# azuxmioy/Render-In-Between

Measured on AMD Instinct MI355X. Metric: rendered frames/sec at 512x512 (generator forward + blend, device-resident), higher is better.
Workload: dtype f32

## Files before the change

render-in-between_amd/csrc/igemm.hip.h:

```cpp
#pragma once
#include <hip/hip_runtime.h>
#include <stdint.h>
#include <type_traits>

namespace rib {

typedef float f32x16 __attribute__((ext_vector_type(16)));
typedef float f32x4 __attribute__((ext_vector_type(4)));
typedef __bf16 bf16x8 __attribute__((ext_vector_type(8)));

__device__ __forceinline__ bf16x8 to_bf16x8(const float4 lo, const float4 hi) {
  bf16x8 r;
  r[0] = (__bf16)lo.x; r[1] = (__bf16)lo.y; r[2] = (__bf16)lo.z; r[3] = (__bf16)lo.w;
  r[4] = (__bf16)hi.x; r[5] = (__bf16)hi.y; r[6] = (__bf16)hi.z; r[7] = (__bf16)hi.w;
  return r;
}

enum { ACT_NONE = 0, ACT_LRELU = 1, ACT_TANH = 2, ACT_SIGMOID = 3 };

__device__ __forceinline__ float blend1(float img, float m, float dain) {
  return __fadd_rn(__fmul_rn(img, m), __fmul_rn(dain, __fsub_rn(1.f, m)));
}

enum { ST_F32 = 0, ST_BF16 = 1, ST_F16 = 2 };
// ... 35 lines not shown
__device__ __forceinline__ float4 lrelu4(float4 v) {
  return make_float4(lrelu(v.x), lrelu(v.y), lrelu(v.z), lrelu(v.w));
}
__device__ __forceinline__ float apply_act(float v, int act) {
  if (act == ACT_LRELU) return lrelu(v);
  if (act == ACT_TANH) return tanhf(v);
  if (act == ACT_SIGMOID) return 1.f / (1.f + __expf(-v));
  return v;
}

struct IgemmParams {
  const float* x;
  int Hin, Win, xC;
  int Cin;
  const float* pro_scale;
  const float* pro_shift;
  int pro_ld;
  int pro_lrelu;
  const float* x2; const float* w2;
  int x2C, Cin2;
  const float* w;
  const float* bias;
  int CoutPad;
  int Hout, Wout;
  int tilesX, tilesY;
  int xcd_chunk;
  float* y;
  int yC, yoff, Cout;
  int y_f32;
  int act;
  const float* res;
  int resC, res_ups;
  float* y_nchw;
  double* stat_part;
  int ksplit;
  float* slab;
  const float* xm;
  int xmC, xm_ups;
  const float* m_scale;
  const float* m_shift;
  int m_ld;
  int C;
  int nsets;
  float* ys0; float* ys1;
  int act0, act1;
  const double* m_part; int m_tiles, m_Cs; float m_inv;
  const float* bl_img; const float* bl_dain; float* bl_fuse; int bl_C;
  int w_mod; unsigned w_stride;
  unsigned b_stride; int pair, pair_yoff;
  const float* zeros;
};

enum { STATS_MAX_PARTIALS = 128 };

__device__ __forceinline__ void stats_from_partials(const double* base, int tiles, int Cs, int c, int t0, int tstep,
                                                    double& a1, double& a2) {
  a1 = 0.0; a2 = 0.0;
  int t = t0;
  for (; t + 3 * tstep < tiles; t += 4 * tstep) {
    const double x0 = base[(size_t)t * 2 * Cs + c], y0 = base[(size_t)t * 2 * Cs + Cs + c];
    const double x1 = base[(size_t)(t + tstep) * 2 * Cs + c], y1 = base[(size_t)(t + tstep) * 2 * Cs + Cs + c];
    const double x2 = base[(size_t)(t + 2 * tstep) * 2 * Cs + c], y2 = base[(size_t)(t + 2 * tstep) * 2 * Cs + Cs + c];
    const double x3 = base[(size_t)(t + 3 * tstep) * 2 * Cs + c], y3 = base[(size_t)(t + 3 * tstep) * 2 * Cs + Cs + c];
    a1 += (x0 + x1) + (x2 + x3);
    a2 += (y0 + y1) + (y2 + y3);
  }
  for (; t < tiles; t += tstep) {
    a1 += base[(size_t)t * 2 * Cs + c];
    a2 += base[(size_t)t * 2 * Cs + Cs + c];
  }
}
__device__ __forceinline__ void scale_shift_of(double s1, double s2, float inv_count, float g, float b, float& sc, float& sh) {
  const double mean = s1 * (double)inv_count;
  double var = s2 * (double)inv_count - mean * mean;
  if (var < 0.0) var = 0.0;
  const float rstd = (float)(1.0 / sqrt(var + 1e-5));
  sc = rstd * g;
  sh = b - (float)mean * sc;
}

enum { PREC_F32 = 0, PREC_BF16 = 1, PREC_F16 = 2 };
template <int FRW, int WM, int WN, int MF, int NF, int BK, int STRIDE, int KS, bool UPS, int KW = 1, int TB = 1, int PREC = 0, int DMA = 0>
struct IgemmGeom {
  static constexpr bool BF16 = PREC != PREC_F32;
  static constexpr int NT = 256 * KW;
  static constexpr int FRH = 32 / FRW;
  static constexpr int TH = FRH * MF * WM;
  static constexpr int TW = FRW;
  static constexpr int PH = UPS ? 4 : 1;
  static constexpr int IH = UPS ? (TH + 2) : ((TH - 1) * STRIDE + KS);
  static constexpr int IW = UPS ? (TW + 2) : ((TW - 1) * STRIDE + KS);
  static constexpr int EPS = BF16 ? 8 : 4;
  static constexpr int KF = BK * 4 / EPS;
  static constexpr int GPR = BK / EPS;
  static constexpr int GPRB = KF / 4;
  static constexpr int CK = KF + 4;
  static constexpr int IWH = (IW + 1) / 2;
  static constexpr int IWP = (STRIDE == 2 && FRW == 8) ? ((IW + 3) / 8 * 8 + 4) : IW;
  static constexpr int BN = NF == 0 ? 16 * WN : 32 * NF * WN;
  static constexpr int AP = (DMA & 2) ? KF : CK;
  static constexpr int BP = (DMA & 1) ? KF : CK;
  static constexpr int SLOTS = KF / 4;
  static constexpr int SWZ_SHIFT = SLOTS >= 16 ? 0 : (SLOTS == 8 ? 1 : (SLOTS == 4 ? 2 : 3));
// ... 193 lines not shown
            const uint32_t w[4] = {__float_as_uint(v.x), __float_as_uint(v.y), __float_as_uint(v.z), __float_as_uint(v.w)};
            float e[8];
#pragma unroll
            for (int k = 0; k < 4; ++k) { e[2 * k] = h16_to_f32<ST>((uint16_t)(w[k] & 0xffffu)); e[2 * k + 1] = h16_to_f32<ST>((uint16_t)(w[k] >> 16)); }
            if (aff) {
              const float sc[8] = {psc[0].x, psc[0].y, psc[0].z, psc[0].w, psc[PV - 1].x, psc[PV - 1].y, psc[PV - 1].z, psc[PV - 1].w};
              const float sh[8] = {psh[0].x, psh[0].y, psh[0].z, psh[0].w, psh[PV - 1].x, psh[PV - 1].y, psh[PV - 1].z, psh[PV - 1].w};
#pragma unroll
              for (int k = 0; k < 8; ++k) e[k] = e[k] * sc[k] + sh[k];
            }
            if (lr) {
#pragma unroll
              for (int k = 0; k < 8; ++k) e[k] = lrelu(e[k]);
            }
            uint32_t o[4];
#pragma unroll
            for (int k = 0; k < 4; ++k) o[k] = (uint32_t)f32_to_h16<ST>(e[2 * k]) | ((uint32_t)f32_to_h16<ST>(e[2 * k + 1]) << 16);
            v = make_float4(__uint_as_float(o[0]), __uint_as_float(o[1]), __uint_as_float(o[2]), __uint_as_float(o[3]));
          }
        } else {
          if (aff) v = make_float4(v.x * psc[0].x + psh[0].x, v.y * psc[0].y + psh[0].y, v.z * psc[0].z + psh[0].z, v.w * psc[0].w + psh[0].w);
          if (lr) v = lrelu4(v);
        }
      }
      if (!inb) v = make_float4(0.f, 0.f, 0.f, 0.f);
      int lpix = pix;
      if constexpr (STRIDE == 2) { const int ly = pix / G::IW, lx = pix % G::IW; lpix = ly * G::IWP + (lx & 1) * G::IWH + (lx >> 1); }
      if (tid + i * NT < total4) *reinterpret_cast<float4*>(sA + lpix * G::CK + ac4 * 4) = v;
    }
  };

  auto consumer_stats = [&]() {
    if constexpr (SPADE) {
      if (p.m_part) {
        constexpr int NCH = G::BN / 2, S = NT / NCH;
        const int j = tid % NCH, sl = tid / NCH;
        const int v = n0 / 2 + j;
        const bool vv = v < p.nsets * p.C;
        const int c = vv ? (v >= p.C ? v - p.C : v) : 0;
        double a1, a2;
        stats_from_partials(p.m_part + (size_t)n * p.m_tiles * 2 * p.m_Cs, p.m_tiles, p.m_Cs, c, sl, S, a1, a2);
        double* red = reinterpret_cast<double*>(smem);
        red[(sl * NCH + j) * 2] = a1; red[(sl * NCH + j) * 2 + 1] = a2;
        __syncthreads();
        if (sl == 0) {
          double t1 = 0.0, t2 = 0.0;
#pragma unroll
          for (int k = 0; k < S; ++k) { t1 += red[(k * NCH + j) * 2]; t2 += red[(k * NCH + j) * 2 + 1]; }
          float sc, sh;
          scale_shift_of(t1, t2, p.m_inv, 1.f, 0.f, sc, sh);
          s_stat[j] = sc; s_stat[NCH + j] = sh;
        }
        __syncthreads();
      }
    }
  };

  auto compute_tap = [&](int dy, int dx, int buf, int ph = 0) {
    if constexpr (N16) {
      const int l15 = lane & 15, lq = lane >> 4;
      const float* sBb = sB + buf * G::SB + l15 * G::CK + lq * 4;
#pragma unroll
      for (int kb = 0; kb < BK / 16; ++kb) {
        float4 a[MF][2];
#pragma unroll
        for (int mf = 0; mf < MF; ++mf)
#pragma unroll
          for (int sub = 0; sub < 2; ++sub) {
            const int r = (wm * MF + mf) * 2 + sub + dy, c = l15 + dx;
            a[mf][sub] = *reinterpret_cast<const float4*>(sA + (r * G::IW + c) * G::CK + lq * 4 + kb * 16);
          }
        const float4 b = *reinterpret_cast<const float4*>(sBb + kb * 16);
#pragma unroll
        for (int t = 0; t < 4; ++t)
#pragma unroll
          for (int mf = 0; mf < MF; ++mf)
#pragma unroll
            for (int sub = 0; sub < 2; ++sub) {
              const float av = t == 0 ? a[mf][sub].x : t == 1 ? a[mf][sub].y : t == 2 ? a[mf][sub].z : a[mf][sub].w;
              const float bw = t == 0 ? b.x : t == 1 ? b.y : t == 2 ? b.z : b.w;
              acc16[mf][sub] = __builtin_amdgcn_mfma_f32_16x16x4f32(av, bw, acc16[mf][sub], 0, 0, 0);
            }
      }
      return;
// ... 340 lines not shown
        for (int mf = 0; mf < MF; ++mf)
#pragma unroll
          for (int nf = 0; nf < NFE; ++nf)
#pragma unroll
            for (int r = 0; r < 16; ++r) acc[mf][nf][r] += rb[((mf * NFE + nf) * 16 + r) * 64];
      }
    }
    if (kw != 0) return;
  }

  if constexpr (N16) {
    const int l15 = lane & 15, lq = lane >> 4;
    const int col = n0 + l15;
    const bool cvalid = col < p.Cout;
    const float bv = p.bias[min(col, p.CoutPad - 1)];
    double s1 = 0.0, s2 = 0.0;
#pragma unroll
    for (int mf = 0; mf < MF; ++mf)
#pragma unroll
      for (int sub = 0; sub < 2; ++sub)
#pragma unroll
        for (int r = 0; r < 4; ++r) {
          const int oy = ty0 + (wm * MF + mf) * 2 + sub;
          const int ox = tx0 + lq * 4 + r;
          const float v = apply_act(acc16[mf][sub][r] + bv, p.act);
          if (cvalid && oy < p.Hout && ox < p.Wout) {
            const size_t pix = ((size_t)n * p.Hout + oy) * p.Wout + ox;
            p.y[pix * p.yC + p.yoff + col] = v;
            if (p.y_nchw) p.y_nchw[(((size_t)n * p.Cout + col) * p.Hout + oy) * p.Wout + ox] = v;
            s1 += (double)v;
            s2 += (double)v * (double)v;
          }
        }
    if (p.stat_part) {
      __syncthreads();
      double* red = reinterpret_cast<double*>(smem);
      double a1 = s1 + __shfl_xor(s1, 16); a1 += __shfl_xor(a1, 32);
      double a2 = s2 + __shfl_xor(s2, 16); a2 += __shfl_xor(a2, 32);
      if (lane < 16) { red[(wm * 16 + l15) * 2] = a1; red[(wm * 16 + l15) * 2 + 1] = a2; }
      __syncthreads();
      if (tid < 16) {
        double b1 = 0.0, b2 = 0.0;
#pragma unroll
        for (int m = 0; m < WM; ++m) { b1 += red[(m * 16 + tid) * 2]; b2 += red[(m * 16 + tid) * 2 + 1]; }
        double* dst = p.stat_part + (((size_t)n * (p.tilesX * p.tilesY) + tile) * 2) * p.CoutPad;
        dst[n0 + tid] = b1;
        dst[p.CoutPad + n0 + tid] = b2;
      }
    }
  } else if (!SPADE && p.slab != nullptr) {
    float* slab = p.slab + ((size_t)split * gridDim.z / p.ksplit + n) * p.Hout * p.Wout * p.CoutPad;
#pragma unroll
    for (int nf = 0; nf < NF; ++nf) {
      const int col = n0 + (wn * NF + nf) * 32 + li;
#pragma unroll
      for (int ph = 0; ph < PH; ++ph)
#pragma unroll
      for (int mf = 0; mf < MF; ++mf) {
#pragma unroll
        for (int r = 0; r < 16; ++r) {
          const int row = (r & 3) + 8 * (r >> 2) + 4 * lh;
          int oy = ty0 + (wm * MF + mf) * G::FRH + row / FRW;
          int ox = tx0 + row % FRW;
          if (UPS) { oy = 2 * oy + (ph >> 1); ox = 2 * ox + (ph & 1); }
          if (col < p.CoutPad && oy < p.Hout && ox < p.Wout)
            slab[((size_t)oy * p.Wout + ox) * p.CoutPad + col] = acc[ph * MF + mf][nf][r];
        }
      }
    }
  } else if (!SPADE) {
    double* red = reinterpret_cast<double*>(smem);
    if (p.stat_part) __syncthreads();
    const float* pbias = p.bias + (p.w_mod ? (size_t)(n % p.w_mod) * p.b_stride : 0);
    const int ny = p.pair ? (n >> 1) : n;
    const int yoff = p.pair ? p.yoff + (n & 1) * p.pair_yoff : p.yoff;
#pragma unroll
    for (int nf = 0; nf < NF; ++nf) {
      float pv = 0.f, d1 = 0.f, d2 = 0.f;
      const int col = n0 + (wn * NF + nf) * 32 + li;
      const bool cvalid = col < p.Cout;
      const float bv = (col < p.CoutPad) ? pbias[col] : 0.f;
#pragma unroll
      for (int ph = 0; ph < PH; ++ph)
#pragma unroll
      for (int mf = 0; mf < MF; ++mf) {
        const int oy0 = ty0 + (__builtin_amdgcn_readfirstlane(wm) * MF + mf) * G::FRH, ox0 = tx0 + 4 * lh;
        const bool full = !UPS && oy0 + G::FRH <= p.Hout && tx0 + FRW <= p.Wout;
        float rv[16];
        if (p.res && full) {
          const int sh = p.res_ups ? 1 : 0;
          const size_t rrow = (size_t)(p.Wout >> sh) * p.resC;
          const size_t rbase = (((size_t)n * (p.Hout >> sh) + (oy0 >> sh)) * (p.Wout >> sh) + (ox0 >> sh)) * p.resC + min(col, p.resC - 1);
#pragma unroll
          for (int r = 0; r < 16; ++r) {
            const int RY = (8 * (r >> 2)) / FRW, RX = (8 * (r >> 2)) % FRW + (r & 3);
            rv[r] = ld_act<ST>(p.res, rbase + (size_t)(RY >> sh) * rrow + (size_t)(RX >> sh) * p.resC);
          }
        } else if (p.res) {
#pragma unroll
          for (int r = 0; r < 16; ++r) {
            const int row = (r & 3) + 8 * (r >> 2) + 4 * lh;
            int oy = ty0 + (wm * MF + mf) * G::FRH + row / FRW;
            int ox = tx0 + row % FRW;
            if (UPS) { oy = 2 * oy + (ph >> 1); ox = 2 * ox + (ph & 1); }
            oy = min(oy, p.Hout - 1); ox = min(ox, p.Wout - 1);
// ... 64 lines not shown
              const size_t nbase = (((size_t)n * p.Cout + col) * p.Hout + oy0) * p.Wout + ox0;
#pragma unroll
              for (int r = 0; r < 16; ++r) {
                const int RY = (8 * (r >> 2)) / FRW, RX = (8 * (r >> 2)) % FRW + (r & 3);
                p.y_nchw[nbase + (size_t)RY * p.Wout + RX] = BF16 ? vf[r] : vv[r];
              }
            }
          }
        } else {
#pragma unroll
        for (int r = 0; r < 16; ++r) {
          const int row = (r & 3) + 8 * (r >> 2) + 4 * lh;
          int oy = ty0 + (wm * MF + mf) * G::FRH + row / FRW;
          int ox = tx0 + row % FRW;
          if (UPS) { oy = 2 * oy + (ph >> 1); ox = 2 * ox + (ph & 1); }
          if (okm & (1u << r)) {
            const size_t yi = (((size_t)ny * p.Hout + oy) * p.Wout + ox) * p.yC + yoff + col;
            if constexpr (BF16) { if (p.y_f32) p.y[yi] = vv[r]; else st_act<ST>(p.y, yi, vv[r]); }
            else p.y[yi] = vv[r];
          }
        }
        if (p.y_nchw) {
#pragma unroll
          for (int r = 0; r < 16; ++r) {
            const int row = (r & 3) + 8 * (r >> 2) + 4 * lh;
            int oy = ty0 + (wm * MF + mf) * G::FRH + row / FRW;
            int ox = tx0 + row % FRW;
            if (UPS) { oy = 2 * oy + (ph >> 1); ox = 2 * ox + (ph & 1); }
            if (okm & (1u << r)) p.y_nchw[(((size_t)n * p.Cout + col) * p.Hout + oy) * p.Wout + ox] = BF16 ? vf[r] : vv[r];
          }
        }
        }
      }
      if (p.stat_part) {
        int cnt = 0;
#pragma unroll
        for (int ph = 0; ph < PH; ++ph)
#pragma unroll
          for (int mf = 0; mf < MF; ++mf) {
            const int oy0 = ty0 + (__builtin_amdgcn_readfirstlane(wm) * MF + mf) * G::FRH;
            if (!UPS && oy0 + G::FRH <= p.Hout && tx0 + FRW <= p.Wout) { cnt += cvalid ? 16 : 0; continue; }
#pragma unroll
            for (int r = 0; r < 16; ++r) {
              const int row = (r & 3) + 8 * (r >> 2) + 4 * lh;
              int oy = ty0 + (wm * MF + mf) * G::FRH + row / FRW;
              int ox = tx0 + row % FRW;
              if (UPS) { oy = 2 * oy + (ph >> 1); ox = 2 * ox + (ph & 1); }
              cnt += (cvalid && oy < p.Hout && ox < p.Wout) ? 1 : 0;
            }
          }
        const double k = (double)cnt, pd = (double)pv;
        const double s1 = k * pd + (double)d1;
        const double s2 = (k * pd + 2.0 * (double)d1) * pd + (double)d2;
        const double a1 = s1 + __shfl_xor(s1, 32);
        const double a2 = s2 + __shfl_xor(s2, 32);
        if (lh == 0) {
          const int c = (wn * NF + nf) * 32 + li;
          red[(wm * G::BN + c) * 2 + 0] = a1;
          red[(wm * G::BN + c) * 2 + 1] = a2;
        }
      }
    }
    if (p.stat_part) {
      __syncthreads();
      for (int c = tid; c < G::BN; c += 256) {
        double a1 = 0.0, a2 = 0.0;
#pragma unroll
        for (int m = 0; m < WM; ++m) { a1 += red[(m * G::BN + c) * 2]; a2 += red[(m * G::BN + c) * 2 + 1]; }
        const int col = n0 + c;
        if (col < p.CoutPad) {
          double* dst = p.stat_part + (((size_t)n * (p.tilesX * p.tilesY) + tile) * 2) * p.CoutPad;
          dst[col] = a1;
          dst[p.CoutPad + col] = a2;
        }
      }
    }
  } else if constexpr (NF == 1) {
    const int hb = li >> 4, c16 = li & 15;
    const int colg = n0 + wn * 32 + c16;
    const int v = (n0 / 2) + wn * 16 + c16;
    const bool vvalid = v < p.nsets * p.C;
    const int set = (vvalid && v >= p.C) ? 1 : 0;
    const int c = v - set * p.C;
    float bg = 0.f, bb = 0.f, sc = 0.f, sh = 0.f;
    if (vvalid) {
      bg = p.bias[colg]; bb = p.bias[colg + 16];
      if (p.m_part) { sc = s_stat[v - n0 / 2]; sh = s_stat[G::BN / 2 + v - n0 / 2]; }
      else { sc = p.m_scale[(size_t)n * p.m_ld + c]; sh = p.m_shift[(size_t)n * p.m_ld + c]; }
    }
    float* yout = set ? p.ys1 : p.ys0;
    const int act = set ? p.act1 : p.act0;
    const int Hm = p.xm_ups ? p.Hout / 2 : p.Hout, Wm = p.xm_ups ? p.Wout / 2 : p.Wout;
#pragma unroll
    for (int mf = 0; mf < MF; ++mf) {
      const int oy0 = ty0 + (__builtin_amdgcn_readfirstlane(wm) * MF + mf) * G::FRH;
      const bool full = oy0 + G::FRH <= p.Hout && tx0 + FRW <= p.Wout;
      const int oyl = oy0 + (16 * hb) / FRW, oxl = tx0 + 4 * lh;
      const int s = p.xm_ups ? 1 : 0;
      const size_t xrow = (size_t)Wm * p.xmC, yrow = (size_t)p.Wout * p.C;
      const size_t xbase = (((size_t)n * Hm + (oyl >> s)) * Wm + (oxl >> s)) * p.xmC + (vvalid ? c : 0);
      const size_t ybase = (((size_t)n * p.Hout + oyl) * p.Wout + oxl) * p.C + c;
      float xr[8];
#pragma unroll
      for (int k = 0; k < 8; ++k) {
        if (full) {
          const int RY = (8 * (k >> 2)) / FRW, RX = (8 * (k >> 2)) % FRW + (k & 3);
          xr[k] = ld_act<ST>(p.xm, xbase + (size_t)(RY >> s) * xrow + (size_t)(RX >> s) * p.xmC);
        } else {
          const int r = hb * 8 + k;
          const int row = (r & 3) + 8 * (r >> 2) + 4 * lh;
          const int oy = min(ty0 + (wm * MF + mf) * G::FRH + row / FRW, p.Hout - 1);
          const int ox = min(tx0 + row % FRW, p.Wout - 1);
          const int sy = p.xm_ups ? (oy >> 1) : oy, sx = p.xm_ups ? (ox >> 1) : ox;
          xr[k] = ld_act<ST>(p.xm, (((size_t)n * Hm + sy) * Wm + sx) * p.xmC + (vvalid ? c : 0));
        }
      }
#pragma unroll
      for (int k = 0; k < 8; ++k) {
        const float lo = acc[mf][0][k], hi = acc[mf][0][8 + k];
        const float olo = __shfl_xor(lo, 16), ohi = __shfl_xor(hi, 16);
        const float gamma = (hb ? ohi : lo) + bg;
        const float beta = (hb ? hi : olo) + bb;
        float o = (xr[k] * sc + sh) * (1.f + gamma) + beta;
        o = apply_act(o, act);
        if (full) {
          const int RY = (8 * (k >> 2)) / FRW, RX = (8 * (k >> 2)) % FRW + (k & 3);
          if (vvalid) st_act<ST>(yout, ybase + (size_t)RY * yrow + (size_t)RX * p.C, o);
        } else {
          const int r = hb * 8 + k;
          const int row = (r & 3) + 8 * (r >> 2) + 4 * lh;
          const int oy = ty0 + (wm * MF + mf) * G::FRH + row / FRW;
          const int ox = tx0 + row % FRW;
          if (vvalid && oy < p.Hout && ox < p.Wout) st_act<ST>(yout, (((size_t)n * p.Hout + oy) * p.Wout + ox) * p.C + c, o);
        }
      }
    }
  } else {
#pragma unroll
    for (int q = 0; q < NF / 2; ++q) {
      const int colg = n0 + (wn * NF + 2 * q) * 32 + li;
      const int v = (n0 / 2) + (wn * NF / 2 + q) * 32 + li;
      const bool vvalid = v < p.nsets * p.C;
      const int set = (vvalid && v >= p.C) ? 1 : 0;
      const int c = v - set * p.C;
      float bg = 0.f, bb = 0.f, sc = 0.f, sh = 0.f;
      if (vvalid) {
        bg = p.bias[colg]; bb = p.bias[colg + 32];
        if (p.m_part) { sc = s_stat[v - n0 / 2]; sh = s_stat[G::BN / 2 + v - n0 / 2]; }
        else { sc = p.m_scale[(size_t)n * p.m_ld + c]; sh = p.m_shift[(size_t)n * p.m_ld + c]; }
      }
      float* yout = set ? p.ys1 : p.ys0;
      const int act = set ? p.act1 : p.act0;
      const int Hm = p.xm_ups ? p.Hout / 2 : p.Hout, Wm = p.xm_ups ? p.Wout / 2 : p.Wout;
#pragma unroll
      for (int mf = 0; mf < MF; ++mf) {
        const int oy0 = ty0 + (__builtin_amdgcn_readfirstlane(wm) * MF + mf) * G::FRH, ox0 = tx0 + 4 * lh;
        const bool full = oy0 + G::FRH <= p.Hout && tx0 + FRW <= p.Wout;
        float xr[16];
        if (full) {
          const int s = p.xm_ups ? 1 : 0;
          const size_t xrow = (size_t)Wm * p.xmC;
          const size_t xbase = (((size_t)n * Hm + (oy0 >> s)) * Wm + (ox0 >> s)) * p.xmC + (vvalid ? c : 0);
#pragma unroll
          for (int r = 0; r < 16; ++r) {
            const int RY = (8 * (r >> 2)) / FRW, RX = (8 * (r >> 2)) % FRW + (r & 3);
            xr[r] = ld_act<ST>(p.xm, xbase + (size_t)(RY >> s) * xrow + (size_t)(RX >> s) * p.xmC);
          }
          if (vvalid) {
            const size_t yrow = (size_t)p.Wout * p.C;
            const size_t ybase = (((size_t)n * p.Hout + oy0) * p.Wout + ox0) * p.C + c;
#pragma unroll
            for (int r = 0; r < 16; ++r) {
              const int RY = (8 * (r >> 2)) / FRW, RX = (8 * (r >> 2)) % FRW + (r & 3);
              const float gamma = acc[mf][2 * q][r] + bg;
              const float beta = acc[mf][2 * q + 1][r] + bb;
              float o = (xr[r] * sc + sh) * (1.f + gamma) + beta;
              o = apply_act(o, act);
              st_act<ST>(yout, ybase + (size_t)RY * yrow + (size_t)RX * p.C, o);
            }
          }
        } else {
// ... 30 lines not shown
```

render-in-between_amd/csrc/kernels.hip.h:

```cpp
#pragma once
#include "igemm.hip.h"

namespace rib {

struct GemmDmaParams {
  const float* A; const float* B; float* C;
  int M, N, K, lda, ldc;
  size_t sA, sB, sC;
  int modB;
};

typedef uint32_t u32x4 __attribute__((ext_vector_type(4)));
__device__ __forceinline__ void split3_bf16(const float4 p, const float4 q, bf16x8& hi, bf16x8& mid, bf16x8& lo) {
  const float x[8] = {p.x, p.y, p.z, p.w, q.x, q.y, q.z, q.w};
  u32x4 h, m, l;
#pragma unroll
  for (int i = 0; i < 4; ++i) {
    const uint32_t u0 = __float_as_uint(x[2 * i]), u1 = __float_as_uint(x[2 * i + 1]);
    h[i] = __builtin_amdgcn_perm(u1, u0, 0x07060302u);
    const float r0 = x[2 * i] - __uint_as_float(u0 & 0xffff0000u), r1 = x[2 * i + 1] - __uint_as_float(u1 & 0xffff0000u);
    const uint32_t v0 = __float_as_uint(r0), v1 = __float_as_uint(r1);
    m[i] = __builtin_amdgcn_perm(v1, v0, 0x07060302u);
    const float s0 = r0 - __uint_as_float(v0 & 0xffff0000u), s1 = r1 - __uint_as_float(v1 & 0xffff0000u);
    l[i] = __builtin_amdgcn_perm(__float_as_uint(s1), __float_as_uint(s0), 0x07060302u);
// ... 85 lines not shown
        const int rb = (wn * NF + nf) * 32 + li;
        b[nf] = *reinterpret_cast<const float4*>(sB + rb * BK + (slot ^ ((rb >> 1) & 7)) * 4);
      }
#pragma unroll
      for (int nf = 0; nf < NF; ++nf) {
        if constexpr (ST == ST_F32) {
          acc[nf] = __builtin_amdgcn_mfma_f32_32x32x2f32(a.x, b[nf].x, acc[nf], 0, 0, 0);
          acc[nf] = __builtin_amdgcn_mfma_f32_32x32x2f32(a.y, b[nf].y, acc[nf], 0, 0, 0);
          acc[nf] = __builtin_amdgcn_mfma_f32_32x32x2f32(a.z, b[nf].z, acc[nf], 0, 0, 0);
          acc[nf] = __builtin_amdgcn_mfma_f32_32x32x2f32(a.w, b[nf].w, acc[nf], 0, 0, 0);
        } else if constexpr (ST == ST_F16) {
          acc[nf] = __builtin_amdgcn_mfma_f32_32x32x16_f16(*reinterpret_cast<const f16x8*>(&a), *reinterpret_cast<const f16x8*>(&b[nf]), acc[nf], 0, 0, 0);
        } else {
          acc[nf] = __builtin_amdgcn_mfma_f32_32x32x16_bf16(*reinterpret_cast<const bf16x8*>(&a), *reinterpret_cast<const bf16x8*>(&b[nf]), acc[nf], 0, 0, 0);
        }
      }
    }
  }
  float* C = p.C + (size_t)z * p.sC;
#pragma unroll
  for (int nf = 0; nf < NF; ++nf) {
    const int col = n0 + (wn * NF + nf) * 32 + li;
#pragma unroll
    for (int r = 0; r < 16; ++r) {
      const int row = m0 + wm * 32 + (r & 3) + 8 * (r >> 2) + 4 * lh;
      float v = acc[nf][r];
      if constexpr (X3 == 2) v += acc_s[nf][r];
      if (row < p.M && col < p.N) C[(size_t)row * p.ldc + col] = v;
    }
  }
}

struct FinalizeParams {
  const double* part;
  int tiles, Cs, C;
  const float* gamma;
  const float* beta;
  float* scale;
  float* shift;
  int ld, off;
  float inv_count;
  float eps;
  int g_stride, pair_merge, pair_off;
};

template <int CH>
__global__ __launch_bounds__(1024) void k_stats_finalize(const FinalizeParams p) {
  static_assert(CH == 16 || CH == 4, "16 channels x 64 slices or 4 channels x 256 slices");
  constexpr int SL = 1024 / CH;
  __shared__ double red[2][16][CH];
  const int cl = threadIdx.x % CH, sl = threadIdx.x / CH;
  const int c = blockIdx.x * CH + cl;
  const int n = blockIdx.y;
  double a1 = 0.0, a2 = 0.0;
  if (c < p.Cs) stats_from_partials(p.part + (size_t)n * p.tiles * 2 * p.Cs, p.tiles, p.Cs, c, sl, SL, a1, a2);
#pragma unroll
  for (int off = CH; off < 64; off <<= 1) { a1 += __shfl_xor(a1, off); a2 += __shfl_xor(a2, off); }
  if ((threadIdx.x & 63) < CH) { red[0][threadIdx.x >> 6][cl] = a1; red[1][threadIdx.x >> 6][cl] = a2; }
  __syncthreads();
  if (sl == 0) {
    double t1 = 0.0, t2 = 0.0;
#pragma unroll
    for (int w = 0; w < 16; ++w) { t1 += red[0][w][cl]; t2 += red[1][w][cl]; }
    red[0][0][cl] = t1; red[1][0][cl] = t2;
  }
  if (sl == 0 && c < p.C) {
    const double s1 = red[0][0][cl], s2 = red[1][0][cl];
    const double mean = s1 * (double)p.inv_count;
    double var = s2 * (double)p.inv_count - mean * mean;
    if (var < 0.0) var = 0.0;
    const float rstd = (float)(1.0 / sqrt(var + (double)p.eps));
    const int gs = (n & 1) * p.g_stride;
    const float g = p.gamma ? p.gamma[gs + c] : 1.f;
    const float b = p.beta ? p.beta[gs + c] : 0.f;
    const float sc = rstd * g;
    const size_t at = p.pair_merge ? (size_t)(n >> 1) * p.ld + p.off + (n & 1) * p.pair_off + c : (size_t)n * p.ld + p.off + c;
    p.scale[at] = sc;
    p.shift[at] = b - (float)mean * sc;
  }
}

struct SplitEpiParams {
  const float* slab; int ksplit; int B;
  const float* bias; int CoutPad;
  float* y; int yC, yoff, Cout;
  int act;
  const float* res; int resC, res_ups;
  double* stat_part; int blocks;
  int Hout, Wout;
};

template <int ST>
__global__ __launch_bounds__(256) void k_splitk_epilogue(const SplitEpiParams p) {
  __shared__ __attribute__((aligned(16))) double red[2][256][4];
  const int c4n = p.CoutPad / 4;
  const int slots = 256 / c4n;
  const int c4 = threadIdx.x % c4n, slot = threadIdx.x / c4n;
  const int n = blockIdx.y;
  const int npix = p.Hout * p.Wout;
  const int ppb = slots * 4;
  const size_t sstride = (size_t)p.B * npix * p.CoutPad;
  const float4 bv = *reinterpret_cast<const float4*>(p.bias + c4 * 4);
  double s1[4] = {0.0, 0.0, 0.0, 0.0}, s2[4] = {0.0, 0.0, 0.0, 0.0};
  float4 acc4[4];
  {
    float4 v[4][4];
#pragma unroll
    for (int k = 0; k < 4; ++k) {
      const int pix = blockIdx.x * ppb + k * slots + slot;
      const float* src = p.slab + ((size_t)n * npix + (pix < npix ? pix : 0)) * p.CoutPad + c4 * 4;
#pragma unroll
      for (int s = 0; s < 4; ++s) v[k][s] = s < p.ksplit ? *reinterpret_cast<const float4*>(src + s * sstride) : make_float4(0.f, 0.f, 0.f, 0.f);
    }
#pragma unroll
    for (int k = 0; k < 4; ++k) {
      float4 a = v[k][0];
#pragma unroll
      for (int s = 1; s < 4; ++s)
        if (s < p.ksplit) { a.x += v[k][s].x; a.y += v[k][s].y; a.z += v[k][s].z; a.w += v[k][s].w; }
      acc4[k] = a;
    }
// ... 20 lines not shown
      const int oy = pix / p.Wout, ox = pix % p.Wout;
      const size_t rpix = p.res_ups ? ((size_t)n * (p.Hout >> 1) + (oy >> 1)) * (p.Wout >> 1) + (ox >> 1) : (size_t)n * npix + pix;
#pragma unroll
      for (int e = 0; e < 4; ++e) rres[k][e] = ld_act<ST>(p.res, rpix * p.resC + min(c4 * 4 + e, p.resC - 1));
    }
  }
  float vals[4][4];
#pragma unroll
  for (int k = 0; k < 4; ++k) {
    const int pix = blockIdx.x * ppb + k * slots + slot;
    const float4 a = acc4[k];
    const float v[4] = {a.x + bv.x, a.y + bv.y, a.z + bv.z, a.w + bv.w};
#pragma unroll
    for (int e = 0; e < 4; ++e) {
      float t = v[e];
      if (p.res) t += rres[k][e];
      t = apply_act(t, p.act);
      if constexpr (ST != ST_F32) t = round16<ST>(t);
      vals[k][e] = (pix < npix && c4 * 4 + e < p.Cout) ? t : 0.f;
    }
#pragma unroll
    for (int e = 0; e < 4; ++e) { s1[e] += (double)vals[k][e]; s2[e] += (double)vals[k][e] * (double)vals[k][e]; }
  }
#pragma unroll
  for (int k = 0; k < 4; ++k) {
    const int pix = blockIdx.x * ppb + k * slots + slot;
    if (pix < npix) {
      const size_t opix = (size_t)n * npix + pix;
#pragma unroll
      for (int e = 0; e < 4; ++e)
        if (c4 * 4 + e < p.Cout) st_act<ST>(p.y, opix * p.yC + p.yoff + c4 * 4 + e, vals[k][e]);
    }
  }
  if (p.stat_part) {
#pragma unroll
    for (int e = 0; e < 4; ++e) { red[0][threadIdx.x][e] = s1[e]; red[1][threadIdx.x][e] = s2[e]; }
    __syncthreads();
    for (int c = threadIdx.x; c < p.CoutPad; c += 256) {
      const int g = c / 4, e = c % 4;
      double a1 = 0.0, a2 = 0.0;
      for (int s = 0; s < slots; ++s) { a1 += red[0][s * c4n + g][e]; a2 += red[1][s * c4n + g][e]; }
      double* dst = p.stat_part + (((size_t)n * p.blocks + blockIdx.x) * 2) * p.CoutPad;
      dst[c] = a1;
      dst[p.CoutPad + c] = a2;
    }
  }
}

struct StatSrc {
  const double* part;
  int tiles, Cs;
  float inv_count;
  const float* gamma;
  const float* beta;
};

__device__ __forceinline__ void block_stats_64(const StatSrc& s, int n, int c0, int nch, double* red ,
                                               float* s_sc, float* s_sh) {
  const int j = threadIdx.x & 63, q = threadIdx.x >> 6;
  double a1 = 0.0, a2 = 0.0;
  if (j < nch) stats_from_partials(s.part + (size_t)n * s.tiles * 2 * s.Cs, s.tiles, s.Cs, c0 + j, q, 4, a1, a2);
  red[(q * 64 + j) * 2] = a1; red[(q * 64 + j) * 2 + 1] = a2;
  __syncthreads();
  if (q == 0 && j < nch) {
    double t1 = 0.0, t2 = 0.0;
#pragma unroll
    for (int k = 0; k < 4; ++k) { t1 += red[(k * 64 + j) * 2]; t2 += red[(k * 64 + j) * 2 + 1]; }
    float sc, sh;
    scale_shift_of(t1, t2, s.inv_count, s.gamma ? s.gamma[c0 + j] : 1.f, s.beta ? s.beta[c0 + j] : 0.f, sc, sh);
    s_sc[j] = sc; s_sh[j] = sh;
  }
  __syncthreads();
}

enum { WSRC_PLAIN = 0, WSRC_SPADE = 1, WSRC_JOIN = 2 };
struct WinoInParams {
  const float* x; int H, W, xC, Cin;
  const float* pro_scale; const float* pro_shift; int pro_ld, pro_lrelu;
  StatSrc st;
  float* v; int tilesY, tilesX;
  int nslices, ublocks;
  int x_ups; const float* slab; int slab_ld, col0; const float* sbias;
  const float* x2; const float* xres; float* o; const float* pro2_scale; const float* pro2_shift; StatSrc st2;
};

__device__ __forceinline__ float spade_mod1(float x, float sc, float sh, float g, float bg, float b, float bb) {
  return fmaf(fmaf(x, sc, sh), 1.f + (g + bg), b + bb);
}

template <int MODE> struct WinoConsts { float4 sc, sh, bg, bb, sc2, sh2; bool aff; };
template <int MODE> struct WinoRaw { float4 a, b, c; };

template <int MODE>
__device__ __forceinline__ void wino_in_consts(const WinoInParams& p, int n, int slice, int c4, bool cok, double* red, float* s_sc,
                                               float* s_sh, WinoConsts<MODE>& k) {
  k.sc = make_float4(1.f, 1.f, 1.f, 1.f); k.sh = make_float4(0.f, 0.f, 0.f, 0.f);
  k.aff = false;
  const int l = (threadIdx.x & 15) * 4;
  if (p.st.part) {
    block_stats_64(p.st, n, slice * 64, min(64, p.Cin - slice * 64), red, s_sc, s_sh);
    k.sc = make_float4(s_sc[l], s_sc[l + 1], s_sc[l + 2], s_sc[l + 3]);
    k.sh = make_float4(s_sh[l], s_sh[l + 1], s_sh[l + 2], s_sh[l + 3]);
    k.aff = true;
  } else if (p.pro_scale && cok) {
    k.sc = *reinterpret_cast<const float4*>(p.pro_scale + (size_t)n * p.pro_ld + c4 * 4);
    k.sh = *reinterpret_cast<const float4*>(p.pro_shift + (size_t)n * p.pro_ld + c4 * 4);
    k.aff = true;
  }
  if constexpr (MODE == WSRC_SPADE) {
    const int v = c4 * 4, colg = (v / 32) * 64 + (v % 32);
    k.bg = cok ? *reinterpret_cast<const float4*>(p.sbias + colg) : k.sh;
    k.bb = cok ? *reinterpret_cast<const float4*>(p.sbias + colg + 32) : k.sh;
  }
  if constexpr (MODE == WSRC_JOIN) {
    k.sc2 = make_float4(1.f, 1.f, 1.f, 1.f); k.sh2 = make_float4(0.f, 0.f, 0.f, 0.f);
    if (p.x2) {
      if (p.st2.part) {
        __syncthreads();
        block_stats_64(p.st2, n, slice * 64, min(64, p.Cin - slice * 64), red, s_sc, s_sh);
        k.sc2 = make_float4(s_sc[l], s_sc[l + 1], s_sc[l + 2], s_sc[l + 3]);
        k.sh2 = make_float4(s_sh[l], s_sh[l + 1], s_sh[l + 2], s_sh[l + 3]);
      } else if (cok) {
        k.sc2 = *reinterpret_cast<const float4*>(p.pro2_scale + (size_t)n * p.pro_ld + c4 * 4);
        k.sh2 = *reinterpret_cast<const float4*>(p.pro2_shift + (size_t)n * p.pro_ld + c4 * 4);
      }
    }
  }
}

template <int MODE>
__device__ __forceinline__ void wino_fetch(const WinoInParams& p, int n, int cy, int cx, int c4, WinoRaw<MODE>& r) {
  if constexpr (MODE == WSRC_SPADE) {
    const int Hs = p.x_ups ? p.H >> 1 : p.H, Ws = p.x_ups ? p.W >> 1 : p.W;
    const int sy = p.x_ups ? cy >> 1 : cy, sx = p.x_ups ? cx >> 1 : cx;
    r.a = *reinterpret_cast<const float4*>(p.x + (((size_t)n * Hs + sy) * Ws + sx) * p.xC + c4 * 4);
    const int v = c4 * 4, colg = (v / 32) * 64 + (v % 32);
    const float* sl = p.slab + (((size_t)n * p.H + cy) * p.W + cx) * p.slab_ld + p.col0 + colg;
    r.b = *reinterpret_cast<const float4*>(sl);
    r.c = *reinterpret_cast<const float4*>(sl + 32);
  } else {
    const size_t e = (((size_t)n * p.H + cy) * p.W + cx) * p.xC + c4 * 4;
    r.a = *reinterpret_cast<const float4*>(p.x + e);
    if constexpr (MODE == WSRC_JOIN) r.b = *reinterpret_cast<const float4*>((p.x2 ? p.x2 : p.xres) + e);
  }
}

template <int MODE>
__device__ __forceinline__ float4 wino_value(const WinoInParams& p, const WinoConsts<MODE>& k, const WinoRaw<MODE>& r) {
  float4 w = r.a;
  if constexpr (MODE == WSRC_SPADE) {
    w = make_float4(spade_mod1(r.a.x, k.sc.x, k.sh.x, r.b.x, k.bg.x, r.c.x, k.bb.x), spade_mod1(r.a.y, k.sc.y, k.sh.y, r.b.y, k.bg.y, r.c.y, k.bb.y),
                    spade_mod1(r.a.z, k.sc.z, k.sh.z, r.b.z, k.bg.z, r.c.z, k.bb.z), spade_mod1(r.a.w, k.sc.w, k.sh.w, r.b.w, k.bg.w, r.c.w, k.bb.w));
// ... 40 lines not shown
      }
    float4 t[4];
#pragma unroll
    for (int q = 0; q < 4; ++q) {
      float4 v[2];
#pragma unroll
      for (int a = 0; a < 2; ++a) {
        const int iy = 2 * ty - 1 + (a ? ib : ia), ix = 2 * tx - 1 + q;
        const bool inb = iy >= 0 && iy < p.H && ix >= 0 && ix < p.W;
        float4 w = wino_value<MODE>(p, kc, d[a][q]);
        if constexpr (MODE == WSRC_JOIN) {
          if (r == 1 && (q == 1 || q == 2) && inb) *reinterpret_cast<float4*>(p.o + (((size_t)n * p.H + iy) * p.W + ix) * p.xC + c4 * 4) = w;
        }
        if (!inb) w = make_float4(0.f, 0.f, 0.f, 0.f);
        v[a] = w;
      }
      t[q] = make_float4(v[0].x + sg * v[1].x, v[0].y + sg * v[1].y, v[0].z + sg * v[1].z, v[0].w + sg * v[1].w);
    }
    const size_t plane = (size_t)ntiles * p.Cin;
    float* vb = p.v + (size_t)n * 16 * plane + (size_t)tile * p.Cin + c4 * 4;
    *reinterpret_cast<float4*>(vb + (size_t)(r * 4 + 0) * plane) = RIB_F4_SUB(t[0], t[2]);
    *reinterpret_cast<float4*>(vb + (size_t)(r * 4 + 1) * plane) = RIB_F4_ADD(t[1], t[2]);
    *reinterpret_cast<float4*>(vb + (size_t)(r * 4 + 2) * plane) = RIB_F4_SUB(t[2], t[1]);
    *reinterpret_cast<float4*>(vb + (size_t)(r * 4 + 3) * plane) = RIB_F4_SUB(t[1], t[3]);
  }
}

struct WinoOutParams {
  const float* m; int tilesY, tilesX, CoutPad;
  const float* bias;
  float* y; int yC, yoff, Cout, Hout, Wout;
  int act;
  const float* res; int resC;
  double* stat_part;
  int nslices, ublocks;
};

__device__ __forceinline__ void wino_out_partials(double (*red)[256][4], const double s1[4], const double s2[4], double* stat_part,
                                                  int n, int ublocks, int ub, int slice, int CoutPad) {
#pragma unroll
  for (int e = 0; e < 4; ++e) { red[0][threadIdx.x][e] = s1[e]; red[1][threadIdx.x][e] = s2[e]; }
  __syncthreads();
  if (threadIdx.x < 64) {
    const int c = slice * 64 + threadIdx.x;
    if (c < CoutPad) {
      const int g = threadIdx.x >> 2, e = threadIdx.x & 3;
      double a1 = 0.0, a2 = 0.0;
#pragma unroll
      for (int s = 0; s < 16; ++s) { a1 += red[0][s * 16 + g][e]; a2 += red[1][s * 16 + g][e]; }
      double* dst = stat_part + (((size_t)n * ublocks + ub) * 2) * CoutPad;
      dst[c] = a1;
      dst[CoutPad + c] = a2;
    }
  }
}

__global__ __launch_bounds__(256) void k_wino_out(const WinoOutParams p) {
  __shared__ __attribute__((aligned(16))) double red[2][256][4];
  const int c4n = p.CoutPad / 4;
  const int slice = blockIdx.x % p.nslices, ub = blockIdx.x / p.nslices;
  const int c4 = slice * 16 + (threadIdx.x & 15);
  const int n = blockIdx.y;
  const int ntiles = p.tilesY * p.tilesX;
  double s1[4] = {0.0, 0.0, 0.0, 0.0}, s2[4] = {0.0, 0.0, 0.0, 0.0};
  if (c4 < c4n) {
    const float4 bv = *reinterpret_cast<const float4*>(p.bias + c4 * 4);
    const size_t plane = (size_t)ntiles * p.CoutPad;
    for (int u = ub * 16 + (threadIdx.x >> 4); u < ntiles * 2; u += p.ublocks * 16) {
      const int r = u & 1, tile = u >> 1;
      const float* mb = p.m + (size_t)n * 16 * plane + (size_t)tile * p.CoutPad + c4 * 4;
      float4 mm[3][4];
#pragma unroll
      for (int a = 0; a < 3; ++a)
#pragma unroll
        for (int q = 0; q < 4; ++q) mm[a][q] = *reinterpret_cast<const float4*>(mb + (size_t)((r + a) * 4 + q) * plane);
      const float sg = r ? -1.f : 1.f;
      float4 uu[4];
#pragma unroll
      for (int q = 0; q < 4; ++q)
        uu[q] = make_float4(mm[0][q].x + sg * (mm[1][q].x + mm[2][q].x), mm[0][q].y + sg * (mm[1][q].y + mm[2][q].y),
                            mm[0][q].z + sg * (mm[1][q].z + mm[2][q].z), mm[0][q].w + sg * (mm[1][q].w + mm[2][q].w));
      float4 yv[2];
      yv[0] = RIB_F4_ADD(RIB_F4_ADD(uu[0], uu[1]), uu[2]);
      yv[1] = RIB_F4_SUB(RIB_F4_SUB(uu[1], uu[2]), uu[3]);
      const int ty = tile / p.tilesX, tx = tile % p.tilesX;
      const int oy = 2 * ty + r;
      float rr[2][4];
#pragma unroll
      for (int q = 0; q < 2; ++q) {
        const int cy = min(oy, p.Hout - 1), cx = min(2 * tx + q, p.Wout - 1);
#pragma unroll
        for (int e = 0; e < 4; ++e)
          rr[q][e] = p.res ? p.res[(((size_t)n * p.Hout + cy) * p.Wout + cx) * p.resC + min(c4 * 4 + e, p.resC - 1)] : 0.f;
      }
#pragma unroll
      for (int q = 0; q < 2; ++q) {
        const int ox = 2 * tx + q;
        const bool inb = oy < p.Hout && ox < p.Wout;
        const float v4[4] = {yv[q].x + bv.x, yv[q].y + bv.y, yv[q].z + bv.z, yv[q].w + bv.w};
#pragma unroll
        for (int e = 0; e < 4; ++e) {
          float t = apply_act(v4[e] + rr[q][e], p.act);
          const bool ok = inb && c4 * 4 + e < p.Cout;
          if (ok) p.y[(((size_t)n * p.Hout + oy) * p.Wout + ox) * p.yC + p.yoff + c4 * 4 + e] = t;
          t = ok ? t : 0.f;
          s1[e] += (double)t; s2[e] += (double)t * (double)t;
        }
      }
    }
  }
  if (p.stat_part) wino_out_partials(red, s1, s2, p.stat_part, n, p.ublocks, ub, slice, p.CoutPad);
}

__device__ __constant__ float kWino4BT[6][6] = {
    {81.f / 64, 0.f, -45.f / 16, 0.f, 1.f, 0.f},        {0.f, -27.f / 16, -9.f / 4, 3.f / 4, 1.f, 0.f},
    {0.f, 27.f / 16, -9.f / 4, -3.f / 4, 1.f, 0.f},     {0.f, -27.f / 32, -9.f / 16, 3.f / 2, 1.f, 0.f},
    {0.f, 27.f / 32, -9.f / 16, -3.f / 2, 1.f, 0.f},    {0.f, 81.f / 64, 0.f, -45.f / 16, 0.f, 1.f}};
__device__ __constant__ float kWino4AT[4][6] = {
    {1.f, 1.f, 1.f, 1.f, 1.f, 0.f},                      {0.f, 3.f / 4, -3.f / 4, 3.f / 2, -3.f / 2, 0.f},
    {0.f, 9.f / 16, 9.f / 16, 9.f / 4, 9.f / 4, 0.f},    {0.f, 27.f / 64, -27.f / 64, 27.f / 8, -27.f / 8, 1.f}};

__device__ __forceinline__ float4 f4_fma(float a, float4 x, float4 acc) {
  return make_float4(fmaf(a, x.x, acc.x), fmaf(a, x.y, acc.y), fmaf(a, x.z, acc.z), fmaf(a, x.w, acc.w));
}
__device__ __forceinline__ float4 f4_scale(float a, float4 x) { return make_float4(a * x.x, a * x.y, a * x.z, a * x.w); }

template <int MODE>
__global__ __launch_bounds__(256) void k_wino4_in(const WinoInParams p) {
  __shared__ double red[4 * 64 * 2];
  __shared__ float s_sc[64], s_sh[64];
  const int c4n = p.Cin / 4;
  const int n = blockIdx.y;
  const int slice = blockIdx.x % p.nslices, ub = blockIdx.x / p.nslices;
  const int c4 = slice * 16 + (threadIdx.x & 15);
  const bool cok = c4 < c4n;
  const int ntiles = p.tilesY * p.tilesX;
  WinoConsts<MODE> kc;
  wino_in_consts<MODE>(p, n, slice, c4, cok, red, s_sc, s_sh, kc);
  if (!cok) return;
  for (int u = ub * 16 + (threadIdx.x >> 4); u < ntiles * 6; u += p.ublocks * 16) {
    const int r = u % 6, tile = u / 6;
    const int ty = tile / p.tilesX, tx = tile % p.tilesX;
    const int a0 = r == 0 ? 0 : 1, da = (r == 0 || r == 5) ? 2 : 1, na = (r == 0 || r == 5) ? 3 : 4;
    float4 t[6];
// ... 93 lines not shown
      const float4 s34 = RIB_F4_ADD(u[3], u[4]);
      const float4 d34 = RIB_F4_SUB(u[3], u[4]);
      float4 yv[4];
      yv[0] = make_float4(u[0].x + s12.x + s34.x, u[0].y + s12.y + s34.y, u[0].z + s12.z + s34.z, u[0].w + s12.w + s34.w);
      yv[1] = f4_fma(3.f / 4, d12, f4_scale(3.f / 2, d34));
      yv[2] = f4_fma(9.f / 16, s12, f4_scale(9.f / 4, s34));
      yv[3] = f4_fma(27.f / 64, d12, f4_fma(27.f / 8, d34, u[5]));
      const int ty = tile / p.tilesX, tx = tile % p.tilesX;
      const int oy = 4 * ty + r;
      float rr[4][4];
#pragma unroll
      for (int q = 0; q < 4; ++q) {
        const int cy = min(oy, p.Hout - 1), cx = min(4 * tx + q, p.Wout - 1);
#pragma unroll
        for (int e = 0; e < 4; ++e)
          rr[q][e] = p.res ? p.res[(((size_t)n * p.Hout + cy) * p.Wout + cx) * p.resC + min(c4 * 4 + e, p.resC - 1)] : 0.f;
      }
#pragma unroll
      for (int q = 0; q < 4; ++q) {
        const int ox = 4 * tx + q;
        const bool inb = oy < p.Hout && ox < p.Wout;
        const float v4[4] = {yv[q].x + bv.x, yv[q].y + bv.y, yv[q].z + bv.z, yv[q].w + bv.w};
#pragma unroll
        for (int e = 0; e < 4; ++e) {
          float t = apply_act(v4[e] + rr[q][e], p.act);
          const bool ok = inb && c4 * 4 + e < p.Cout;
          if (ok) p.y[(((size_t)n * p.Hout + oy) * p.Wout + ox) * p.yC + p.yoff + c4 * 4 + e] = t;
          t = ok ? t : 0.f;
          s1[e] += (double)t; s2[e] += (double)t * (double)t;
        }
      }
    }
  }
  if (p.stat_part) wino_out_partials(red, s1, s2, p.stat_part, n, p.ublocks, ub, slice, p.CoutPad);
}
#undef RIB_F4_SUB
#undef RIB_F4_ADD

struct ModulateParams {
  const float* slab; int ksplit, B, slab_ld, col0;
  const float* bias;
  const float* xm; int xmC, xm_ups;
  const float* m_scale; const float* m_shift; int m_ld;
  StatSrc st;
  int C, nsets;
  float* ys0; float* ys1; int act0, act1;
  int Hout, Wout;
  int nslices, pblocks;
};

template <int ST>
__global__ __launch_bounds__(256) void k_spade_modulate(const ModulateParams p) {
  __shared__ double red[4 * 64 * 2];
  __shared__ float s_sc[64], s_sh[64];
  const int v4n = p.nsets * p.C / 4;
  const int n = blockIdx.y;
  const int slice = blockIdx.x % p.nslices, pb = blockIdx.x / p.nslices;
  const int v4 = slice * 16 + (threadIdx.x & 15);
  const int npix = p.Hout * p.Wout;
  const size_t sstride = (size_t)p.B * npix * p.slab_ld;
  const int Hm = p.xm_ups ? p.Hout / 2 : p.Hout, Wm = p.xm_ups ? p.Wout / 2 : p.Wout;
  const int v = v4 * 4;
  const int set = v >= p.C ? 1 : 0;
  const int c = v - set * p.C;
  float4 sc, sh;
  if (p.st.part) {
    const int v0 = slice * 64, c0 = v0 >= p.C ? v0 - p.C : v0;
    block_stats_64(p.st, n, c0, min(64, p.C - c0), red, s_sc, s_sh);
    const int l = (threadIdx.x & 15) * 4;
    sc = make_float4(s_sc[l], s_sc[l + 1], s_sc[l + 2], s_sc[l + 3]);
    sh = make_float4(s_sh[l], s_sh[l + 1], s_sh[l + 2], s_sh[l + 3]);
  }
  if (v4 >= v4n) return;
  if (!p.st.part) {
    sc = *reinterpret_cast<const float4*>(p.m_scale + (size_t)n * p.m_ld + c);
    sh = *reinterpret_cast<const float4*>(p.m_shift + (size_t)n * p.m_ld + c);
  }
  const int colg = (v / 32) * 64 + (v % 32);
  const float4 bg = *reinterpret_cast<const float4*>(p.bias + colg);
  const float4 bb = *reinterpret_cast<const float4*>(p.bias + colg + 32);
  const int act = set ? p.act1 : p.act0;
  float* yout = set ? p.ys1 : p.ys0;
  const int pstep = p.pblocks * 16;
  for (int pix0 = pb * 16 + (threadIdx.x >> 4); pix0 < npix; pix0 += 4 * pstep) {
    float4 g[4], b[4], x[4];
#pragma unroll
    for (int k = 0; k < 4; ++k) {
      const int pix = min(pix0 + k * pstep, npix - 1);
      const float* src = p.slab + ((size_t)n * npix + pix) * p.slab_ld + p.col0 + colg;
      g[k] = *reinterpret_cast<const float4*>(src);
      b[k] = *reinterpret_cast<const float4*>(src + 32);
      for (int s = 1; s < p.ksplit; ++s) {
        const float4 g2 = *reinterpret_cast<const float4*>(src + s * sstride);
        const float4 b2 = *reinterpret_cast<const float4*>(src + s * sstride + 32);
        g[k].x += g2.x; g[k].y += g2.y; g[k].z += g2.z; g[k].w += g2.w;
        b[k].x += b2.x; b[k].y += b2.y; b[k].z += b2.z; b[k].w += b2.w;
      }
      const int oy = pix / p.Wout, ox = pix % p.Wout;
      const int sy = p.xm_ups ? (oy >> 1) : oy, sx = p.xm_ups ? (ox >> 1) : ox;
      x[k] = ld_act4<ST>(p.xm, (((size_t)n * Hm + sy) * Wm + sx) * p.xmC + c);
    }
#pragma unroll
    for (int k = 0; k < 4; ++k) {
      const int pix = pix0 + k * pstep;
      if (pix >= npix) break;
      float4 o;
      o.x = apply_act(spade_mod1(x[k].x, sc.x, sh.x, g[k].x, bg.x, b[k].x, bb.x), act);
      o.y = apply_act(spade_mod1(x[k].y, sc.y, sh.y, g[k].y, bg.y, b[k].y, bb.y), act);
      o.z = apply_act(spade_mod1(x[k].z, sc.z, sh.z, g[k].z, bg.z, b[k].z, bb.z), act);
      o.w = apply_act(spade_mod1(x[k].w, sc.w, sh.w, g[k].w, bg.w, b[k].w, bb.w), act);
      st_act4<ST>(yout, ((size_t)n * npix + pix) * p.C + c, o);
    }
  }
}

struct PoolParams {
  const float* x; float* y;
  int H, W, C;
  double* stat_part;
  int blocks;
};

template <int ST>
__global__ __launch_bounds__(256) void k_avgpool(const PoolParams p) {
  __shared__ __attribute__((aligned(16))) double red[2][256][4];
  const int c4n = p.C / 4;
  const int slots = 256 / c4n;
  const int c4 = threadIdx.x % c4n, slot = threadIdx.x / c4n;
  const int Ho = p.H / 2, Wo = p.W / 2;
  const int n = blockIdx.y;
  const int npix = Ho * Wo;
  const int ppb = slots * 4;
  double s1[4] = {0.0, 0.0, 0.0, 0.0}, s2[4] = {0.0, 0.0, 0.0, 0.0};
  const size_t xn = (size_t)n * p.H * p.W * p.C;
  for (int k = 0; k < 4; ++k) {
    const int pix = blockIdx.x * ppb + k * slots + slot;
    if (pix < npix && slot < slots) {
      const int oy = pix / Wo, ox = pix % Wo;
      float4 v[9]; float m[9];
#pragma unroll
      for (int t = 0; t < 9; ++t) {
        const int iy = oy * 2 - 1 + t / 3, ix = ox * 2 - 1 + t % 3;
        m[t] = (iy >= 0 && iy < p.H && ix >= 0 && ix < p.W) ? 1.f : 0.f;
        const int cy = min(max(iy, 0), p.H - 1), cx = min(max(ix, 0), p.W - 1);
        v[t] = ld_act4<ST>(p.x, xn + ((size_t)cy * p.W + cx) * p.C + c4 * 4);
      }
      float4 a = make_float4(0.f, 0.f, 0.f, 0.f);
#pragma unroll
      for (int t = 0; t < 9; ++t)
        if (m[t] != 0.f) { a.x += v[t].x; a.y += v[t].y; a.z += v[t].z; a.w += v[t].w; }
      const float inv9 = 1.f / 9.f;
      a.x *= inv9; a.y *= inv9; a.z *= inv9; a.w *= inv9;
      if constexpr (ST != ST_F32) a = make_float4(round16<ST>(a.x), round16<ST>(a.y), round16<ST>(a.z), round16<ST>(a.w));
      st_act4<ST>(p.y, ((size_t)n * npix + pix) * p.C + c4 * 4, a);
      const float av[4] = {a.x, a.y, a.z, a.w};
#pragma unroll
      for (int e = 0; e < 4; ++e) { s1[e] += (double)av[e]; s2[e] += (double)av[e] * (double)av[e]; }
    }
  }
#pragma unroll
  for (int e = 0; e < 4; ++e) { red[0][threadIdx.x][e] = s1[e]; red[1][threadIdx.x][e] = s2[e]; }
  __syncthreads();
  for (int c = threadIdx.x; c < p.C; c += 256) {
    const int g = c / 4, e = c % 4;
    double a1 = 0.0, a2 = 0.0;
    for (int s = 0; s < slots; ++s) { a1 += red[0][s * c4n + g][e]; a2 += red[1][s * c4n + g][e]; }
    double* dst = p.stat_part + (((size_t)n * p.blocks + blockIdx.x) * 2) * p.C;
    dst[c] = a1;
    dst[p.C + c] = a2;
  }
}

struct InAddParams {
  const float* t1; const float* sc1; const float* sh1;
  const float* ts; const float* scs; const float* shs;
  const float* xres;
  float* out;
  int C, HW;
  int ld;
  StatSrc st1, sts;
  int nslices, pblocks;
};

template <int ST>
__global__ __launch_bounds__(256) void k_in_add(const InAddParams p) {
  __shared__ double red[4 * 64 * 2];
  __shared__ float s_sc[2][64], s_sh[2][64];
  const int c4n = p.C / 4;
  const int n = blockIdx.y;
  const int slice = blockIdx.x % p.nslices, pb = blockIdx.x / p.nslices;
  const int c4 = slice * 16 + (threadIdx.x & 15);
  const int nch = min(64, p.C - slice * 64);
  if (p.st1.part) block_stats_64(p.st1, n, slice * 64, nch, red, s_sc[0], s_sh[0]);
  if (p.ts && p.sts.part) block_stats_64(p.sts, n, slice * 64, nch, red, s_sc[1], s_sh[1]);
  if (c4 >= c4n) return;
  const int l = (threadIdx.x & 15) * 4;
  float4 s, t, s2 = make_float4(0.f, 0.f, 0.f, 0.f), t2 = s2;
  if (p.st1.part) { s = make_float4(s_sc[0][l], s_sc[0][l + 1], s_sc[0][l + 2], s_sc[0][l + 3]); t = make_float4(s_sh[0][l], s_sh[0][l + 1], s_sh[0][l + 2], s_sh[0][l + 3]); }
  else { s = *reinterpret_cast<const float4*>(p.sc1 + (size_t)n * p.ld + c4 * 4); t = *reinterpret_cast<const float4*>(p.sh1 + (size_t)n * p.ld + c4 * 4); }
  if (p.ts) {
    if (p.sts.part) { s2 = make_float4(s_sc[1][l], s_sc[1][l + 1], s_sc[1][l + 2], s_sc[1][l + 3]); t2 = make_float4(s_sh[1][l], s_sh[1][l + 1], s_sh[1][l + 2], s_sh[1][l + 3]); }
    else { s2 = *reinterpret_cast<const float4*>(p.scs + (size_t)n * p.ld + c4 * 4); t2 = *reinterpret_cast<const float4*>(p.shs + (size_t)n * p.ld + c4 * 4); }
  }
  const float* second = p.ts ? p.ts : p.xres;
  if (!p.ts) { s2 = make_float4(1.f, 1.f, 1.f, 1.f); t2 = make_float4(0.f, 0.f, 0.f, 0.f); }
  const int pstep = p.pblocks * 16;
  for (int pix0 = pb * 16 + (threadIdx.x >> 4); pix0 < p.HW; pix0 += 4 * pstep) {
    float4 a[4], b[4];
#pragma unroll
    for (int k = 0; k < 4; ++k) {
      const size_t e = ((size_t)n * p.HW + min(pix0 + k * pstep, p.HW - 1)) * p.C + c4 * 4;
      a[k] = ld_act4<ST>(p.t1, e);
      b[k] = ld_act4<ST>(second, e);
    }
#pragma unroll
    for (int k = 0; k < 4; ++k) {
      const int pix = pix0 + k * pstep;
      if (pix >= p.HW) break;
      float4 o = make_float4(a[k].x * s.x + t.x, a[k].y * s.y + t.y, a[k].z * s.z + t.z, a[k].w * s.w + t.w);
      if (p.ts) { o.x += b[k].x * s2.x + t2.x; o.y += b[k].y * s2.y + t2.y; o.z += b[k].z * s2.z + t2.z; o.w += b[k].w * s2.w + t2.w; }
      else { o.x += b[k].x; o.y += b[k].y; o.z += b[k].z; o.w += b[k].w; }
      st_act4<ST>(p.out, ((size_t)n * p.HW + pix) * p.C + c4 * 4, o);
    }
  }
}

template <int CO, int ST = 0>
__global__ __launch_bounds__(256) void k_conv_small(const IgemmParams p) {
  extern __shared__ __attribute__((aligned(16))) float smem_dyn[];
  const int Cin = p.Cin, CK = Cin + 4, C4 = Cin / 4;
  float* sA = smem_dyn;
  float* sW = smem_dyn + 18 * 18 * CK;
  const int tid = threadIdx.x;
  const int n = blockIdx.z;
// ... 169 lines not shown
  }
  for (int co = CO; co < p.Cout && p.y; ++co) {
    if (ST != ST_F32 && !p.y_f32) st_act<ST>(p.y, pix * p.yC + p.yoff + co, apply_act(0.f, p.act)); else p.y[pix * p.yC + p.yoff + co] = apply_act(0.f, p.act);
  }
  if constexpr (CO == 1) {
    if (p.bl_fuse) {
      const float m = o[0];
      const size_t hw = (size_t)p.Hout * p.Wout, at = (size_t)oy * p.Wout + ox;
      for (int c = 0; c < p.bl_C; ++c) {
        const size_t i = ((size_t)n * p.bl_C + c) * hw + at;
        p.bl_fuse[i] = blend1(p.bl_img[i], m, p.bl_dain[i]);
      }
    }
  }
}

struct Gather6Params { const float4* src[6]; float4* dst[6]; unsigned n4[6]; };

__global__ __launch_bounds__(256) void k_gather6(const Gather6Params p) {
  const int r = blockIdx.y;
  const float4* s = p.src[r];
  float4* d = p.dst[r];
  const unsigned n = p.n4[r];
  for (unsigned i = blockIdx.x * 256 + threadIdx.x; i < n; i += gridDim.x * 256) d[i] = s[i];
}

struct LowcParams {
  const float* s0; const float* s1; const float* s2; int c0, c1, c2;
  int H, W;
  const float* w;
  const float* bias;
  float* y; int yC, yoff, Cout;
  int act;
  double* stat_part; int CoutPad;
  int tilesX, tilesY;
};

template <int CE, int NCOL, int ST, int TW = 32>
__global__ __launch_bounds__(256) void k_conv_lowc(const LowcParams p) {
  constexpr bool N16 = NCOL == 16;
  static_assert(NCOL == 16 || NCOL == 32 || NCOL == 64, "16-, 32- or 64-column layers");
  static_assert(CE % (N16 ? 4 : 2) == 0, "channel count rounded up to the k-group of one MFMA");
  static_assert(TW == 32 || TW == 16, "8x32 or 8x16 pixel tiles");
  constexpr int TH = 8, IH = TH + 2, IW = TW + 2;
  constexpr int MF = TW / 16;
  constexpr int CP = CE + 1;
  constexpr int KG = N16 ? 4 : 2;
  constexpr int S = 9 * CE / KG;
  constexpr int NF = N16 ? 1 : NCOL / 32;
  __shared__ __attribute__((aligned(16))) float sA[IH * IW * CP];
  __shared__ __attribute__((aligned(16))) double red[4][NCOL][2];
  const int tid = threadIdx.x, lane = tid & 63, wave = tid >> 6;
  const int n = blockIdx.y;
  const int tile = blockIdx.x;
  const int ty0 = (tile / p.tilesX) * TH, tx0 = (tile % p.tilesX) * TW;
  const int ctot = p.c0 + p.c1 + p.c2;
  const size_t HW = (size_t)p.H * p.W;
  {
    constexpr int TOT = CE * IH * IW, NIT = (TOT + 255) / 256;
    float v[NIT];
#pragma unroll
    for (int it = 0; it < NIT; ++it) {
      const int i = tid + it * 256;
      const int c = i / (IH * IW), rem = i - c * (IH * IW);
      const int y = rem / IW, x = rem - y * IW;
      const int gy = ty0 - 1 + y, gx = tx0 - 1 + x;
      v[it] = 0.f;
      if (i < TOT && c < ctot && gy >= 0 && gy < p.H && gx >= 0 && gx < p.W) {
        const float* src; int cc, cn;
        if (c < p.c0) { src = p.s0; cc = c; cn = p.c0; }
        else if (c < p.c0 + p.c1) { src = p.s1; cc = c - p.c0; cn = p.c1; }
        else { src = p.s2; cc = c - p.c0 - p.c1; cn = p.c2; }
        v[it] = src[((size_t)n * cn + cc) * HW + (size_t)gy * p.W + gx];
      }
    }
#pragma unroll
    for (int it = 0; it < NIT; ++it) {
      const int i = tid + it * 256;
      const int c = i / (IH * IW), rem = i - c * (IH * IW);
      const int y = rem / IW, x = rem - y * IW;
      if (i < TOT) sA[(y * IW + x) * CP + c] = v[it];
    }
  }
  constexpr int HV = (!N16 && S * NF > 64) ? 2 : 1;
  constexpr int SH = (S + HV - 1) / HV;
  float bw[SH][NF];
  const float* pw = N16 ? p.w + (lane >> 4) * 16 + (lane & 15) : p.w + (lane >> 5) * NCOL + (lane & 31);
  auto load_b = [&](int h) {
#pragma unroll
// ... 26 lines not shown
          const int off = ((tap / 3) * IW + (tap % 3)) * CP + c;
#pragma unroll
          for (int mf = 0; mf < MF; ++mf) {
            const float a = pa[off + mf * IW * CP];
#pragma unroll
            for (int nf = 0; nf < NF; ++nf) {
              acc[mf][nf] = __builtin_amdgcn_mfma_f32_32x32x2f32(a, bw[sl][nf], acc[mf][nf], 0, 0, 0);
            }
          }
        }
      }
    }
#pragma unroll
    for (int nf = 0; nf < NF; ++nf) {
      const int col = nf * 32 + li;
      const float bv = p.bias[col];
      const bool cok = col < p.Cout;
      double c1 = 0.0, c2 = 0.0;
#pragma unroll
      for (int mf = 0; mf < MF; ++mf) {
#pragma unroll
        for (int r = 0; r < 16; ++r) {
          const int m = (r & 3) + 8 * (r >> 2) + 4 * lh;
          const int oy = ty0 + wave * 2 + (TW == 32 ? mf : (m >> 4));
          const int ox = tx0 + (TW == 32 ? m : (m & 15));
          float v = apply_act(acc[mf][nf][r] + bv, p.act);
          if (ST != ST_F32) v = round16<ST>(v);
          const bool ok = cok && oy < p.H && ox < p.W;
          if (ok) st_act<ST>(p.y, ((size_t)n * HW + (size_t)oy * p.W + ox) * p.yC + p.yoff + col, v);
          v = ok ? v : 0.f;
          c1 += (double)v; c2 += (double)v * (double)v;
        }
      }
      if (p.stat_part) {
        c1 += __shfl_xor(c1, 32); c2 += __shfl_xor(c2, 32);
        if (lh == 0) { red[wave][col][0] = c1; red[wave][col][1] = c2; }
      }
    }
  } else {
    const int l15 = lane & 15, lq = lane >> 4;
    constexpr int NFR = TW / 8;
    f32x4 acc[NFR];
#pragma unroll
    for (int f = 0; f < NFR; ++f)
#pragma unroll
      for (int r = 0; r < 4; ++r) acc[f][r] = 0.f;
    const float* pa = sA + ((wave * 2) * IW + l15) * CP + lq;
#pragma unroll
    for (int s = 0; s < S; ++s) {
      const int tap = (4 * s) / CE, c = (4 * s) % CE;
      const int off = ((tap / 3) * IW + (tap % 3)) * CP + c;
#pragma unroll
      for (int f = 0; f < NFR; ++f) {
        const float a = pa[off + (TW == 32 ? ((f >> 1) * IW + (f & 1) * 16) : f * IW) * CP];
        acc[f] = __builtin_amdgcn_mfma_f32_16x16x4f32(a, bw[s][0], acc[f], 0, 0, 0);
      }
    }
    const int col = l15;
    const float bv = p.bias[col];
    const bool cok = col < p.Cout;
#pragma unroll
    for (int f = 0; f < NFR; ++f) {
      const int oy = ty0 + wave * 2 + (TW == 32 ? (f >> 1) : f);
#pragma unroll
      for (int r = 0; r < 4; ++r) {
        const int ox = tx0 + (TW == 32 ? (f & 1) * 16 : 0) + lq * 4 + r;
        float v = apply_act(acc[f][r] + bv, p.act);
        if (ST != ST_F32) v = round16<ST>(v);
        const bool ok = cok && oy < p.H && ox < p.W;
        if (ok) st_act<ST>(p.y, ((size_t)n * HW + (size_t)oy * p.W + ox) * p.yC + p.yoff + col, v);
        v = ok ? v : 0.f;
        s1 += (double)v; s2 += (double)v * (double)v;
      }
    }
    if (p.stat_part) {
      s1 += __shfl_xor(s1, 16); s2 += __shfl_xor(s2, 16);
      s1 += __shfl_xor(s1, 32); s2 += __shfl_xor(s2, 32);
      if (lq == 0) { red[wave][col][0] = s1; red[wave][col][1] = s2; }
    }
  }
  if (p.stat_part) {
    __syncthreads();
    for (int c = tid; c < p.CoutPad; c += 256) {
      double a1 = 0.0, a2 = 0.0;
      if (c < NCOL) {
#pragma unroll
        for (int w = 0; w < 4; ++w) { a1 += red[w][c][0]; a2 += red[w][c][1]; }
      }
      {
        double* dst = p.stat_part + (((size_t)n * (p.tilesX * p.tilesY) + tile) * 2) * p.CoutPad;
        dst[c] = a1;
        dst[p.CoutPad + c] = a2;
      }
    }
  }
}

struct PackParams {
  const float* s0; const float* s1; const float* s2;
  int c0, c1, c2;
  float* dst; int dC;
  int HW;
};

template <int ST>
__global__ __launch_bounds__(256) void k_pack(const PackParams p) {
  __shared__ float tile[64][33];
  const int n = blockIdx.y;
  const int pix0 = blockIdx.x * 64;
  const int lp = threadIdx.x & 63, slice = threadIdx.x >> 6;
  const int ctot = p.c0 + p.c1 + p.c2;
  const int pix = pix0 + lp;
  for (int j = slice; j < p.dC; j += 4) {
    float t = 0.f;
    if (pix < p.HW && j < ctot) {
      if (j < p.c0) t = p.s0[((size_t)n * p.c0 + j) * p.HW + pix];
      else if (j < p.c0 + p.c1) t = p.s1[((size_t)n * p.c1 + (j - p.c0)) * p.HW + pix];
      else t = p.s2[((size_t)n * p.c2 + (j - p.c0 - p.c1)) * p.HW + pix];
    }
    tile[lp][j] = t;
  }
  __syncthreads();
  const int c4n = p.dC / 4;
  for (int idx = threadIdx.x; idx < 64 * c4n; idx += 256) {
    const int q = idx / c4n, g = idx % c4n;
    if (pix0 + q < p.HW)
// ... 133 lines not shown
```

render-in-between_amd/csrc/rib.hip:

```cpp
#include "kernels.hip.h"
#include "raster.hip.h"
#include "quality.hip.h"
#include <hip/hip_ext.h>
#include "../../include/rib.h"

#include <algorithm>
#include <array>
#include <climits>
#include <cmath>
#include <cstdarg>
#include <cstdio>
#include <cstdlib>
#include <cstring>
#include <map>
#include <memory>
#include <string>
#include <vector>


#include "variants.hip.h"
#define RIB_V(sec, ...) RIB_I_V(RIB_F_EXTERN, __VA_ARGS__)
#define RIB_VK(sec, ...) RIB_I_VK(RIB_F_EXTERN, __VA_ARGS__)
#define RIB_VT(sec, ...) RIB_I_VT(RIB_F_EXTERN, __VA_ARGS__)
#define RIB_VTK(sec, ...) RIB_I_VTK(RIB_F_EXTERN, __VA_ARGS__)
// ... 345 lines not shown
      if (S > nchunks || (S > 1 && (!allow_split || v.NF == 0))) break;
      const long wgs = tiles * ntiles * B * S;
      const int chunks = (nchunks + S - 1) / S;
      const int taps = ups ? 16 : ks * ks;
      const double mfma_tap = v.NF == 0 ? (BK / 16) * v.MF * 8 * 32.0
                                        : (v.BF16 != PREC_F32 ? (BK / 16) * v.MF * v.NF * 32.0 : (BK / 8) * v.MF * v.NF * 4 * 64.0);
      const double ovh_wg = (chunks * (std::max(1, taps / v.TB) * 350.0 + (ks == 1 && v.TB == 2 ? 300.0 : 600.0)) + 7000.0) / v.KW + (v.KW - 1) * 1500.0;
      const double mfma_wg = (double)chunks * taps * mfma_tap;
      const double t_lat = std::ceil((double)wgs / (256.0 * occ)) * (mfma_wg + ovh_wg);
      const double t_cu = std::ceil((double)wgs / 256.0) * (mfma_wg + ovh_wg / occ);
      double t = std::max(t_lat, t_cu);
      if (S > 1) t += 6000.0 + (double)(S + 1) * B * Hout * Wout * pad32(ncols) * 4.0 / 1667.0;
      if (t < best.cycles) { best.cycles = t; best.v = &v; best.ksplit = S; }
    }
  }
  return best;
}

const Variant* pick_gemm_dma(int prec, long Z, int M, int N, int K) {
  static const bool off = getenv("RIB_NO_DMA") != nullptr;
  if (off || K % (prec == PREC_F32 ? 32 : 64) != 0) return nullptr;
  const Variant* best = nullptr; long best_area = 0, best_wgs = 0;
  for (int i = 0; i < kNumVariants; ++i) {
    const Variant& v = kVariants[i];
    if (!v.dma() || v.BF16 != prec) continue;
    const long wgs = Z * ((M + v.BM() - 1) / v.BM()) * ((N + v.BN() - 1) / v.BN());
    const long area = (long)v.BM() * v.BN();
    const bool full = wgs >= 512, bfull = best_wgs >= 512;
    if (!best || (full && (!bfull || area > best_area)) || (!full && !bfull && wgs > best_wgs)) { best = &v; best_area = area; best_wgs = wgs; }
  }
  return best;
}

enum OpKind { OP_PACK, OP_IGEMM, OP_FINALIZE, OP_POOL, OP_INADD, OP_SPLITEPI, OP_MODULATE, OP_WINO_IN, OP_WINO_OUT, OP_LOWC, OP_GEMM };

enum PtrSpace { PS_NULL = 0, PS_WS, PS_WEIGHT, PS_USER, PS_WINO };
enum UserSlot { U_LABEL = 0, U_FAKE, U_PREV, U_IMG, U_MASK, U_FUSE, U_COUNT };
struct PRef {
  PtrSpace sp = PS_NULL;
  size_t off = 0;
};


struct Op {
  OpKind kind;
  int kclass;
  std::string name;
  const Variant* var = nullptr;
  std::string for_op;
  bool label_only = false;
  int small_co = 0;
  bool head = false;
  bool fuse_blend = false;
  IgemmParams ip;
  PRef x, pro_scale, pro_shift, w, bias, y, res, y_nchw, stat, xm, m_scale, m_shift, ys0, ys1, slab, x2, w2;
  PRef m_part;
  PRef st_part[2], st_gamma[2], st_beta[2];
  SplitEpiParams sp; PRef s_slab, s_bias, s_y, s_res, s_stat;
  ModulateParams mp; PRef m_slab, m_bias, m_xm, m_sc, m_sh, m_ys0, m_ys1;
  dim3 grid;
  double flops = 0;
  FinalizeParams fp; PRef f_part, f_gamma, f_beta, f_scale, f_shift;
  PoolParams pp; PRef p_x, p_y, p_stat;
  InAddParams ap; PRef a_t1, a_sc1, a_sh1, a_ts, a_scs, a_shs, a_x, a_out;
  PackParams kp; PRef k_s0, k_s1, k_s2, k_dst;
  LowcParams lc; PRef lc_s0, lc_s1, lc_s2, lc_w, lc_bias, lc_y, lc_stat; int lowc_ce = 0, lowc_ncol = 0, lowc_tw = 32;
  WinoInParams wi; PRef wi_x, wi_sc, wi_sh, wi_v, wi_slab, wi_sbias, wi_x2, wi_xres, wi_o, wi_sc2, wi_sh2; int wi_mode = 0;
  WinoOutParams wo; PRef wo_m, wo_bias, wo_y, wo_res, wo_stat;
  GemmDmaParams gp; PRef g_a, g_b, g_c;
  bool wino = false;
  int wino_m = 0;
};

struct PendingStats {
  Op fin;
  bool pushed = false;
  size_t part_off = 0; int tiles = 0, Cs = 0; float inv_count = 0.f;
  bool affine = false; size_t g_off = 0, be_off = 0;
};

struct Tap { std::string name; size_t off; int Cp, C, H, W; };

struct LazySrc;
struct Act {
  size_t off = 0;
  int Cp = 0, C = 0, H = 0, W = 0;
  bool virt = false; int usrc[3] = {0, 0, 0}, uc[3] = {0, 0, 0};
  std::shared_ptr<LazySrc> lazy;
};
struct PendingStats;
struct Norm {
  size_t sc = 0, sh = 0; int ld = 0;
  bool valid = false;
  std::shared_ptr<PendingStats> pend;
};

struct LazySrc {
  int mode = 0;
  std::string name;
  Act x; Norm nx;
  bool x_ups = false, lrelu = false;
  size_t slab_off = 0; int slab_ld = 0, col0 = 0; size_t sbias_off = 0;
  bool has2 = false; Act x2; Norm n2; Act xres; Act o;
};

struct LabelSlots { size_t x0 = 0, x0_b = 0, nx_sc = 0, nx_sh = 0, nx_b = 0, cat = 0, cat_b = 0, ncat_sc = 0, ncat_sh = 0, ncat_b = 0; };

struct Plan {
  bool labels_only = false;
  LabelSlots ls;
// ... 312 lines not shown
}

struct FusionPolicy {
  bool consumer_stats = !getenv("RIB_NO_CONSUMER_STATS");
  bool head_conv = !getenv("RIB_NO_HEADCONV");
  bool small_conv = !getenv("RIB_NO_SMALLCONV");
  long wino_max_px = getenv("RIB_WINO_MAX_PX") ? atol(getenv("RIB_WINO_MAX_PX")) : 16384;
  int wino_force = getenv("RIB_WINO_M") ? atoi(getenv("RIB_WINO_M")) : 0;
  bool split_k = !getenv("RIB_NO_SPLITK");
  bool n16 = !getenv("RIB_NO_N16");
  int lowc_tw = getenv("RIB_LOWC_TW") ? (atoi(getenv("RIB_LOWC_TW")) == 16 ? 16 : 32) : 0;
  long cond_gemm_max_px = getenv("RIB_COND_GEMM_MAX_PX") ? atol(getenv("RIB_COND_GEMM_MAX_PX")) : 4096;
  bool unfused_spade = !getenv("RIB_NO_UNFUSED_SPADE");
  bool lazy_sources = !getenv("RIB_NO_LAZY");
  bool fuse_shortcut = !getenv("RIB_NO_FUSE_SHORTCUT");
  bool ws_reuse = !getenv("RIB_NO_WS_REUSE");
  bool pair_mask_encoders = !getenv("RIB_NO_PAIR");
};

struct Builder {
  rib_handle* h;
  Plan* P;
  int B;
  const FusionPolicy pol;
  size_t ws = 0;
  std::string error;
  bool mark_label = false;
  bool pair_mask = false;
  bool defer_stats = true;
  void materialize(const Norm& n, const std::string& consumer = std::string()) {
    if (n.pend && !n.pend->pushed) { n.pend->pushed = true; n.pend->fin.for_op = consumer; push(n.pend->fin); }
  }
  static bool has_partials(const Norm& n) { return n.pend && !n.pend->pushed; }
  void finalize_or_defer(Op& f, Norm* out, bool now, size_t part_off, int tiles, int Cs, float inv_count, bool affine, size_t g_off, size_t be_off) {
    if (now || !pol.consumer_stats || !defer_stats || mark_label || tiles > STATS_MAX_PARTIALS) { push(f); return; }
    auto ps = std::make_shared<PendingStats>();
    ps->fin = f; ps->part_off = part_off; ps->tiles = tiles; ps->Cs = Cs; ps->inv_count = inv_count;
    ps->affine = affine; ps->g_off = g_off; ps->be_off = be_off;
    out->pend = ps;
  }
  bool take_partials(const Norm& n, StatSrc& st, Op& op, int slot) {
    if (!has_partials(n) || n.pend->tiles > STATS_MAX_PARTIALS) return false;
    const PendingStats& ps = *n.pend;
    memset(&st, 0, sizeof st);
    st.tiles = ps.tiles; st.Cs = ps.Cs; st.inv_count = ps.inv_count;
    op.st_part[slot] = WS(ps.part_off);
    if (ps.affine) { op.st_gamma[slot] = WT(ps.g_off); op.st_beta[slot] = WT(ps.be_off); }
    return true;
  }
  struct LevelSlab { size_t off = 0; int ld = 0; };
  std::map<int, LevelSlab> level_slab;
  int tuneB = 0;
  int TB_() const { return tuneB > 0 ? tuneB : B; }
  void push(Op op) {
    op.label_only = mark_label;
    P->ops.push_back(op);
  }

  struct AllocRec { size_t voff, bytes, phys; int first, last; };
  std::vector<AllocRec> allocs;
  size_t alloc(size_t bytes) {
    size_t o = ws; ws += align256(bytes);
    allocs.push_back(AllocRec{o, align256(bytes), o, INT_MAX, -1});
    return o;
  }
  Act act(int C, int H, int W) {
    Act a; a.C = C; a.Cp = h->padc(C); a.H = H; a.W = W;
    a.off = alloc((size_t)B * H * W * a.Cp * h->esz());
    return a;
  }
  Norm norm(int Cp, int images = 0) {
    Norm n; n.ld = Cp; n.valid = true;
    n.sc = alloc((size_t)(images ? images : B) * Cp * sizeof(float));
    n.sh = alloc((size_t)(images ? images : B) * Cp * sizeof(float));
    return n;
  }
  Act act_n(int images, int C, int H, int W) {
    Act a; a.C = C; a.Cp = h->padc(C); a.H = H; a.W = W;
    a.off = alloc((size_t)images * H * W * a.Cp * h->esz());
    return a;
  }
  Act virt(int C, int H, int W, int s0, int c0, int s1 = 0, int c1 = 0, int s2 = 0, int c2 = 0) {
    Act a; a.virt = true; a.C = C; a.Cp = 0; a.H = H; a.W = W;
    a.usrc[0] = s0; a.uc[0] = c0; a.usrc[1] = s1; a.uc[1] = c1; a.usrc[2] = s2; a.uc[2] = c2;
    return a;
  }
  bool lowc_serves(std::initializer_list<const char*> names) {
    for (const char* nm : names) {
      auto it = h->conv_index.find(nm);
      if (it == h->conv_index.end() || !h->convs[it->second].wl_off) return false;
    }
    return true;
  }
  bool head_without_nhwc(const ConvDef& c) {
    return c.cout <= 3 && c.ks == 3 && c.stride == 1 && (c.cinp == 16 || c.cinp == 32) && pol.small_conv && pol.head_conv;
  }
  static PRef WS(size_t off) { PRef r; r.sp = PS_WS; r.off = off; return r; }
// ... 105 lines not shown
    } else if (a.y_none) {
      op.y = PRef(); p.yC = 0; p.yoff = 0; p.Cout = a.cout_store >= 0 ? a.cout_store : c.cout;
    } else {
      op.y = WS(a.out.off); p.yC = a.out.Cp; p.yoff = a.yoff;
      p.Cout = a.cout_store >= 0 ? a.cout_store : h->padc(c.cout);
      if (a.out.H != Hout || a.out.W != Wout) { error = fmt("%s: output size mismatch", opname.c_str()); return false; }
    }
    if (a.pair) {
      const bool w16p = h->mc16();
      p.w_mod = 2;
      p.w_stride = (unsigned)(w16p ? 2 * (a.pair->w16_off - c.w16_off) : a.pair->w_off - c.w_off);
      p.b_stride = (unsigned)(a.pair->b_off - c.b_off);
      p.pair = a.pair_merge ? 1 : 0; p.pair_yoff = a.pair_yoff;
    }
    if (a.res) { op.res = WS(a.res->off); p.resC = a.res->Cp; p.res_ups = a.res_ups ? 1 : 0; }
    op.y_nchw = a.y_nchw;
    if (a.y_none && !(small && c.cout <= 3 && (c.cinp == 16 || c.cinp == 32) && pol.head_conv && a.y_nchw.sp != PS_NULL)) {
      error = opname + ": only the head kernel can run without an NHWC destination"; return false;
    }
    if (small) {
      op.small_co = c.cout;
      op.head = c.cout <= 3 && (c.cinp == 16 || c.cinp == 32) && pol.head_conv;
      op.fuse_blend = op.head && c.cout == 1 && a.y_user.sp == PS_USER && a.y_user.off == (size_t)U_MASK;
      p.bl_C = h->g.c.image_nc;
      p.ksplit = 1;
      p.tilesX = (Wout + 15) / 16; p.tilesY = (Hout + 15) / 16; p.xcd_chunk = xcd_chunk_of(p.tilesX * p.tilesY);
      op.grid = dim3(p.tilesX * p.tilesY, 1, B);
      op.flops = 2.0 * c.cin * c.ks * c.ks * c.cout * (double)Hout * Wout * B;
      P->flops[RIB_KC_IGEMM] += op.flops;
      push(op);
      return true;
    }
    int tiles = p.tilesX * p.tilesY;
    size_t part_off = 0;
    op.grid = dim3(tiles, v->NF == 0 ? 1 : (c.coutp + v->BN() - 1) / v->BN(), nB * S);
    op.flops = 2.0 * c.cin * c.ks * c.ks * c.cout * (double)Hout * Wout * nB + aux_flops;
    P->flops[RIB_KC_IGEMM] += op.flops;
    if (a.pair && (S != 1 || v->NF == 0)) { error = opname + ": a paired launch cannot split K or use the 16-column path"; return false; }
    if (S == 1) {
      if (a.want_stats) { part_off = alloc((size_t)nB * tiles * 2 * c.coutp * sizeof(double)); op.stat = WS(part_off); }
      push(op);
    } else {
      const size_t slab_off = alloc((size_t)S * B * Hout * Wout * c.coutp * sizeof(float));
      op.slab = WS(slab_off);
      Op e; e.kind = OP_SPLITEPI; e.kclass = RIB_KC_CONVAUX; e.name = opname + ".splitk_sum";
      memset(&e.sp, 0, sizeof e.sp);
      e.sp.ksplit = S; e.sp.B = B; e.sp.CoutPad = c.coutp; e.sp.yC = p.yC; e.sp.yoff = p.yoff; e.sp.Cout = p.Cout;
      e.sp.act = p.act; e.sp.resC = p.resC; e.sp.res_ups = p.res_ups; e.sp.Hout = Hout; e.sp.Wout = Wout;
      const int slots = 256 / (c.coutp / 4), ppb = slots * 4;
      const int blocks = (Hout * Wout + ppb - 1) / ppb;
      e.sp.blocks = blocks;
      e.s_slab = WS(slab_off); e.s_bias = op.bias; e.s_y = op.y; e.s_res = op.res;
      if (a.want_stats) { part_off = alloc((size_t)B * blocks * 2 * c.coutp * sizeof(double)); e.s_stat = WS(part_off); }
      e.grid = dim3(blocks, B, 1);
      tiles = blocks;
      op.y = PRef(); op.res = PRef();
      push(op);
      push(e);
    }
    if (a.want_stats) {
      Op f; f.kind = OP_FINALIZE; f.kclass = RIB_KC_STATS; f.name = opname + ".stats";
      memset(&f.fp, 0, sizeof f.fp);
      f.fp.tiles = tiles; f.fp.Cs = c.coutp; f.fp.C = h->padc(c.cout);
      f.fp.ld = a.stats_out->ld; f.fp.off = (int)a.stats_choff;
      f.fp.inv_count = 1.0f / ((float)Hout * (float)Wout); f.fp.eps = 1e-5f;
      f.f_part = WS(part_off);
      if (a.affine) { f.f_gamma = WT(c.g_off); f.f_beta = WT(c.be_off); }
      f.f_scale = WS(a.stats_out->sc); f.f_shift = WS(a.stats_out->sh);
      f.grid = dim3(c.coutp / 16, nB, 1);
      if (a.pair) { f.fp.g_stride = a.affine ? (int)(a.pair->g_off - c.g_off) : 0; f.fp.pair_merge = a.pair_merge ? 1 : 0; f.fp.pair_off = a.pair_yoff; }
      finalize_or_defer(f, a.stats_out, a.stats_choff != 0 || a.stats_now || a.pair != nullptr, part_off, tiles, c.coutp, f.fp.inv_count, a.affine, c.g_off, c.be_off);
    }
    return true;
  }

  bool conv_lowc(const ConvArgs& a, const std::string& opname) {
    const ConvDef& c = *a.cd;
    const int H = a.in.H, W = a.in.W;
    if (!c.wl_off || c.ks != 3 || c.stride != 1 || a.ups || a.pro || a.res || a.aux || a.y_nchw.sp != PS_NULL || a.y_user.sp != PS_NULL ||
        a.in.uc[0] + a.in.uc[1] + a.in.uc[2] != c.cin) { error = opname + ": not a layer k_conv_lowc can run"; return false; }
    if (a.out.H != H || a.out.W != W) { error = fmt("%s: output size mismatch", opname.c_str()); return false; }
    Op op; op.kind = OP_LOWC; op.kclass = RIB_KC_IGEMM; op.name = opname; op.lowc_ce = c.lowc_ce; op.lowc_ncol = c.lowc_ncol;
    memset(&op.lc, 0, sizeof op.lc);
    LowcParams& p = op.lc;
    p.c0 = a.in.uc[0]; p.c1 = a.in.uc[1]; p.c2 = a.in.uc[2];
    p.H = H; p.W = W; p.yC = a.out.Cp; p.yoff = a.yoff; p.Cout = a.cout_store >= 0 ? a.cout_store : h->padc(c.cout);
    p.act = a.act; p.CoutPad = c.coutp;
    const int tw = pol.lowc_tw ? pol.lowc_tw : ((c.lowc_ncol == 64 && !a.want_stats) ? 16 : 32);
    op.lowc_tw = tw;
    p.tilesX = (W + tw - 1) / tw; p.tilesY = (H + 7) / 8;
    if (p.Cout > c.lowc_ncol || c.cout > c.lowc_ncol) { error = opname + ": more output columns than the k_conv_lowc instantiation has"; return false; }
    op.lc_s0 = US(a.in.usrc[0]); if (p.c1) op.lc_s1 = US(a.in.usrc[1]); if (p.c2) op.lc_s2 = US(a.in.usrc[2]);
    op.lc_w = WT(c.wl_off); op.lc_bias = WT(c.b_off); op.lc_y = WS(a.out.off);
    const int tiles = p.tilesX * p.tilesY;
    size_t part_off = 0;
    if (a.want_stats) { part_off = alloc((size_t)B * tiles * 2 * c.coutp * sizeof(double)); op.lc_stat = WS(part_off); }
    op.grid = dim3(tiles, B, 1);
    op.flops = 2.0 * c.cin * 9.0 * c.cout * (double)H * W * B;
    P->flops[RIB_KC_IGEMM] += op.flops;
    push(op);
    if (a.want_stats) {
      Op f; f.kind = OP_FINALIZE; f.kclass = RIB_KC_STATS; f.name = opname + ".stats";
      memset(&f.fp, 0, sizeof f.fp);
      f.fp.tiles = tiles; f.fp.Cs = c.coutp; f.fp.C = h->padc(c.cout);
      f.fp.ld = a.stats_out->ld; f.fp.off = (int)a.stats_choff;
      f.fp.inv_count = 1.0f / ((float)H * (float)W); f.fp.eps = 1e-5f;
      f.f_part = WS(part_off);
      if (a.affine) { f.f_gamma = WT(c.g_off); f.f_beta = WT(c.be_off); }
      f.f_scale = WS(a.stats_out->sc); f.f_shift = WS(a.stats_out->sh);
      f.grid = dim3(c.coutp / 16, B, 1);
      finalize_or_defer(f, a.stats_out, a.stats_choff != 0 || a.stats_now, part_off, tiles, c.coutp, f.fp.inv_count, a.affine, c.g_off, c.be_off);
    }
    return true;
  }

  bool conv_wino(const ConvArgs& a, const std::string& opname, int Hout, int Wout) {
    const ConvDef& c = *a.cd;
    const int wino_force = pol.wino_force;
    const int wm = wino_force == 2 || wino_force == 4 ? wino_force : ((long)TB_() * ((Hout + 3) / 4) * ((Wout + 3) / 4) >= 256 ? 4 : 2);
    const int NP = (wm + 2) * (wm + 2);
    const int tilesY = (Hout + wm - 1) / wm, tilesX = (Wout + wm - 1) / wm, ntiles = tilesY * tilesX;
    const std::string gname = opname + (wm == 2 ? ".wino" : ".wino4");
    const size_t v_off = alloc((size_t)B * NP * ntiles * c.cinp * sizeof(float));
    const size_t m_off = alloc((size_t)B * NP * ntiles * c.coutp * sizeof(float));
    {
      Op op; op.kind = OP_WINO_IN; op.kclass = RIB_KC_CONVAUX; op.name = opname + ".wino_in"; op.for_op = gname; op.wino_m = wm;
      memset(&op.wi, 0, sizeof op.wi);
      op.wi.H = a.in.H; op.wi.W = a.in.W; op.wi.xC = a.in.Cp; op.wi.Cin = c.cinp; op.wi.tilesY = tilesY; op.wi.tilesX = tilesX;
      op.wi.pro_lrelu = a.pro_lrelu ? 1 : 0;
      op.wi_x = WS(a.in.off); op.wi_v = WS(v_off);
      if (a.in.lazy) {
        const LazySrc& L = *a.in.lazy;
        if (a.pro || a.pro_lrelu) { error = gname + ": a lazy input carries its own prologue"; return false; }
        op.wi_mode = L.mode;
        op.wi_x = WS(L.x.off); op.wi.xC = L.x.Cp;
        op.wi.pro_ld = L.nx.ld;
        if (!take_partials(L.nx, op.wi.st, op, 0)) { materialize(L.nx, gname); op.wi_sc = WS(L.nx.sc); op.wi_sh = WS(L.nx.sh); }
        if (L.mode == WSRC_SPADE) {
          op.wi.x_ups = L.x_ups ? 1 : 0; op.wi.pro_lrelu = L.lrelu ? 1 : 0;
          op.wi_slab = WS(L.slab_off); op.wi.slab_ld = L.slab_ld; op.wi.col0 = L.col0; op.wi_sbias = WT(L.sbias_off);
        } else {
          if (L.has2) {
            op.wi_x2 = WS(L.x2.off);
            if (L.n2.ld != L.nx.ld) { error = gname + ": join operands with different statistics rows"; return false; }
            if (!take_partials(L.n2, op.wi.st2, op, 1)) { materialize(L.n2, gname); op.wi_sc2 = WS(L.n2.sc); op.wi_sh2 = WS(L.n2.sh); }
          } else op.wi_xres = WS(L.xres.off);
          op.wi_o = WS(L.o.off);
        }
      } else if (a.pro && !(a.pro_choff == 0 && take_partials(*a.pro, op.wi.st, op, 0))) {
        materialize(*a.pro, gname);
        op.wi.pro_ld = a.pro->ld;
        op.wi_sc = WS(a.pro->sc + a.pro_choff * sizeof(float)); op.wi_sh = WS(a.pro->sh + a.pro_choff * sizeof(float));
      }
      const int nsl = (c.cinp + 63) / 64, units = ntiles * (wm + 2);
      op.wi.nslices = nsl; op.wi.ublocks = std::max(1, std::min((units + 15) / 16, (op.wi.st.tiles > 0 ? 512 : 4096) / nsl));
      op.grid = dim3(op.wi.ublocks * nsl, B, 1);
      push(op);
    }
    {
      Choice ch;
      ch.v = pick_gemm_dma(h->prec(), (long)TB_() * NP, ntiles, c.coutp, c.cinp);
      if (!ch.v) ch = choose_variant(h->prec(), 1, 1, false, false, c.coutp, TB_() * NP, tilesY, tilesX, c.cinp, false, 0, false);
      auto it = h->choices.find(fmt("%d,%d,%d|%s", TB_(), P->H, P->W, gname.c_str()));
      if (it != h->choices.end()) {
        const Variant& tv = kVariants[it->second.first];
        if (tv.BF16 != h->prec() || tv.KS != 1 || tv.STRIDE != 1 || tv.UPS || tv.SPADE || tv.NF == 0 || c.cinp % tv.BK != 0 || it->second.second != 1) {
          error = fmt("%s: tuned choice (variant %d, ksplit %d) does not fit this layer", gname.c_str(), it->second.first, it->second.second); return false;
        }
        ch.v = &tv; ch.ksplit = 1;
      }
      const Variant* v = ch.v;
      if (!v) { error = gname + ": no 1x1 kernel variant"; return false; }
      const int set = ensure_wino_set(h, (int)(&c - h->convs.data()), wm);
      if (set < 0) { error = gname + ": " + h->err; return false; }
      Op op; op.kind = OP_IGEMM; op.kclass = RIB_KC_IGEMM; op.name = gname; op.var = v; op.wino = true; op.wino_m = wm;
      op.flops = 2.0 * c.cin * 9.0 * c.cout * (double)Hout * Wout * B;
      if (v->dma()) {
        op.kind = OP_GEMM;
        GemmDmaParams& g = op.gp;
        memset(&g, 0, sizeof g);
        g.M = ntiles; g.N = c.coutp; g.K = c.cinp; g.lda = c.cinp; g.ldc = c.coutp;
        g.sA = (size_t)ntiles * c.cinp; g.sB = (size_t)c.coutp * c.cinp; g.sC = (size_t)ntiles * c.coutp; g.modB = NP;
        op.g_a = WS(v_off); op.g_b = PRef(); op.g_b.sp = PS_WINO; op.g_b.off = (size_t)set; op.g_c = WS(m_off);
        op.grid = dim3((ntiles + v->BM() - 1) / v->BM(), (c.coutp + v->BN() - 1) / v->BN(), B * NP);
        P->flops[RIB_KC_IGEMM] += op.flops;
        push(op);
      } else {
      IgemmParams& p = op.ip;
      memset(&p, 0, sizeof p);
      p.Hin = tilesY; p.Win = tilesX; p.xC = c.cinp; p.Cin = c.cinp; p.CoutPad = c.coutp; p.Hout = tilesY; p.Wout = tilesX;
      p.tilesX = (tilesX + v->TW() - 1) / v->TW(); p.tilesY = (tilesY + v->TH() - 1) / v->TH(); p.xcd_chunk = xcd_chunk_of(p.tilesX * p.tilesY);
      p.act = ACT_NONE; p.ksplit = 1; p.yC = c.coutp; p.yoff = 0; p.Cout = c.coutp;
      p.w_mod = NP; p.w_stride = (unsigned)((size_t)c.coutp * c.cinp);
      op.x = WS(v_off); op.w = PRef(); op.w.sp = PS_WINO; op.w.off = (size_t)set; op.bias = WT(c.zero_off); op.y = WS(m_off);
      op.grid = dim3(p.tilesX * p.tilesY, (c.coutp + v->BN() - 1) / v->BN(), B * NP);
      P->flops[RIB_KC_IGEMM] += op.flops;
      push(op);
      }
    }
    {
      Op op; op.kind = OP_WINO_OUT; op.kclass = RIB_KC_CONVAUX; op.name = opname + ".wino_out"; op.for_op = gname; op.wino_m = wm;
      memset(&op.wo, 0, sizeof op.wo);
      const int nsl = (c.coutp + 63) / 64, units = ntiles * wm;
      const int blocks = std::max(1, std::min((units + 15) / 16, (int)STATS_MAX_PARTIALS));
      op.wo.tilesY = tilesY; op.wo.tilesX = tilesX; op.wo.CoutPad = c.coutp; op.wo.ublocks = blocks; op.wo.nslices = nsl;
      op.wo.yC = a.out.Cp; op.wo.yoff = a.yoff; op.wo.Cout = a.cout_store >= 0 ? a.cout_store : h->padc(c.cout);
      op.wo.Hout = Hout; op.wo.Wout = Wout; op.wo.act = a.act;
      if (a.out.H != Hout || a.out.W != Wout) { error = fmt("%s: output size mismatch", opname.c_str()); return false; }
      op.wo_m = WS(m_off); op.wo_bias = WT(c.b_off); op.wo_y = WS(a.out.off);
      if (a.res) { op.wo_res = WS(a.res->off); op.wo.resC = a.res->Cp; }
      size_t part_off = 0;
      if (a.want_stats) { part_off = alloc((size_t)B * blocks * 2 * c.coutp * sizeof(double)); op.wo_stat = WS(part_off); }
      op.grid = dim3(blocks * nsl, B, 1);
      push(op);
      if (a.want_stats) {
        Op f; f.kind = OP_FINALIZE; f.kclass = RIB_KC_STATS; f.name = opname + ".stats";
        memset(&f.fp, 0, sizeof f.fp);
        f.fp.tiles = blocks; f.fp.Cs = c.coutp; f.fp.C = h->padc(c.cout);
        f.fp.ld = a.stats_out->ld; f.fp.off = (int)a.stats_choff;
        f.fp.inv_count = 1.0f / ((float)Hout * (float)Wout); f.fp.eps = 1e-5f;
        f.f_part = WS(part_off);
        if (a.affine) { f.f_gamma = WT(c.g_off); f.f_beta = WT(c.be_off); }
        f.f_scale = WS(a.stats_out->sc); f.f_shift = WS(a.stats_out->sh);
        f.grid = dim3(c.coutp / 16, B, 1);
        finalize_or_defer(f, a.stats_out, a.stats_choff != 0 || a.stats_now, part_off, blocks, c.coutp, f.fp.inv_count, a.affine, c.g_off, c.be_off);
      }
    }
    return true;
  }

  bool cond_level_gemm(int level, const Act& cond) {
    const long max_px = pol.cond_gemm_max_px;
    const auto it = h->level_groups.find(level);
    if (it == h->level_groups.end() || it->second.size() < 2 || (long)TB_() * cond.H * cond.W > max_px) return true;
    int N = 0; double fl = 0.0;
    for (int gi : it->second) {
      const SpadeGroup& sg = h->spades[gi];
      if (sg.col0 != N || h->padc(sg.cond) != cond.Cp) { error = fmt("cond level %d: SPADE group %s does not continue the level's filter matrix", level, sg.key.c_str()); return false; }
      N += sg.npad;
      fl += 2.0 * sg.cond * 2.0 * sg.nsets * sg.C * (double)cond.H * cond.W * B;
    }
    const SpadeGroup& first = h->spades[it->second[0]];
    const std::string name = fmt("cond_%d.gammabeta", level);
    Choice ch;
    ch.v = pick_gemm_dma(h->prec(), TB_(), cond.H * cond.W, N, cond.Cp);
    if (!ch.v) ch = choose_variant(h->prec(), 1, 1, false, false, N, TB_(), cond.H, cond.W, cond.Cp, false);
    {
      auto ct = h->choices.find(fmt("%d,%d,%d|%s", TB_(), P->H, P->W, name.c_str()));
      if (ct != h->choices.end()) {
        const Variant& tv = kVariants[ct->second.first];
        if (tv.BF16 != h->prec() || tv.KS != 1 || tv.STRIDE != 1 || tv.UPS || tv.SPADE || tv.NF == 0 || cond.Cp % tv.BK != 0 || ct->second.second != 1) {
          error = fmt("%s: tuned choice (variant %d, ksplit %d) does not fit this launch", name.c_str(), ct->second.first, ct->second.second); return false;
        }
        ch.v = &tv; ch.ksplit = 1;
      }
    }
    const Variant* v = ch.v;
    if (!v) { error = name + ": no 1x1 kernel variant"; return false; }
// ... 76 lines not shown
      *ys0 = act(sg.C, Hout, Wout);
      if (sg.nsets == 2) *ys1 = act(sg.C, Hout, Wout);
      int S = 1, slab_ld = 0, col0 = 0;
      size_t slab_off = 0;
      if (from_level) {
        slab_off = lvl->second.off; slab_ld = lvl->second.ld; col0 = sg.col0;
      } else {
        const Variant* cv = uf.v; S = uf.ksplit;
        slab_off = alloc((size_t)S * B * Hout * Wout * sg.npad * sizeof(float)); slab_ld = sg.npad;
        Op op; op.kind = OP_IGEMM; op.kclass = RIB_KC_SPADE; op.name = key + ".spade"; op.var = cv;
        IgemmParams& p = op.ip;
        memset(&p, 0, sizeof p);
        p.Hin = cond.H; p.Win = cond.W; p.xC = cond.Cp; p.Cin = cond.Cp;
        p.CoutPad = sg.npad; p.Hout = Hout; p.Wout = Wout; p.ksplit = S;
        p.tilesX = (Wout + cv->TW() - 1) / cv->TW(); p.tilesY = (Hout + cv->TH() - 1) / cv->TH(); p.xcd_chunk = xcd_chunk_of(p.tilesX * p.tilesY);
        op.x = WS(cond.off); op.w = WT(h->mc16() ? sg.w16_off : sg.w_off); op.bias = WT(sg.b_off); op.slab = WS(slab_off);
        op.grid = dim3(p.tilesX * p.tilesY, (sg.npad + cv->BN() - 1) / cv->BN(), B * S);
        op.flops = 2.0 * sg.cond * 2.0 * sg.nsets * sg.C * (double)Hout * Wout * B;
        P->flops[RIB_KC_SPADE] += op.flops;
        push(op);
      }
      Op mo; mo.kind = OP_MODULATE; mo.kclass = RIB_KC_ELTWISE; mo.name = key + ".spade.modulate";
      memset(&mo.mp, 0, sizeof mo.mp);
      mo.mp.ksplit = S; mo.mp.B = B; mo.mp.slab_ld = slab_ld; mo.mp.col0 = col0; mo.mp.xmC = x.Cp; mo.mp.xm_ups = x_ups ? 1 : 0;
      mo.mp.m_ld = nx.ld; mo.mp.C = sg.Cp; mo.mp.nsets = sg.nsets; mo.mp.act0 = act0 ? ACT_LRELU : ACT_NONE; mo.mp.act1 = ACT_NONE;
      mo.mp.Hout = Hout; mo.mp.Wout = Wout;
      mo.m_slab = WS(slab_off); mo.m_bias = WT(sg.b_off); mo.m_xm = WS(x.off);
      if (!(sg.Cp % 64 == 0 && nx.pend && !nx.pend->affine && sg.Cp <= nx.pend->Cs && take_partials(nx, mo.mp.st, mo, 0))) {
        materialize(nx, key + ".spade");
        mo.m_sc = WS(nx.sc); mo.m_sh = WS(nx.sh);
      }
      mo.m_ys0 = WS(ys0->off); if (sg.nsets == 2) mo.m_ys1 = WS(ys1->off);
      const int nsl = (sg.nsets * sg.Cp + 63) / 64;
      mo.mp.nslices = nsl; mo.mp.pblocks = std::max(1, std::min((Hout * Wout + 15) / 16, (mo.mp.st.tiles > 0 ? 384 : 2048) / nsl));
      mo.grid = dim3(mo.mp.pblocks * nsl, B, 1);
      push(mo);
      return true;
    }
    *ys0 = act(sg.C, Hout, Wout);
    if (sg.nsets == 2) *ys1 = act(sg.C, Hout, Wout);
    Op op; op.kind = OP_IGEMM; op.kclass = RIB_KC_SPADE; op.name = key + ".spade"; op.var = v;
    IgemmParams& p = op.ip;
    memset(&p, 0, sizeof p);
    p.Hin = cond.H; p.Win = cond.W; p.xC = cond.Cp; p.Cin = cond.Cp;
    const bool one_frag = v->NF == 1;
    const int ncols = one_frag ? 32 : sg.npad;
    p.CoutPad = ncols; p.Hout = Hout; p.Wout = Wout;
    p.tilesX = (Wout + v->TW() - 1) / v->TW(); p.tilesY = (Hout + v->TH() - 1) / v->TH(); p.xcd_chunk = xcd_chunk_of(p.tilesX * p.tilesY);
    p.ksplit = 1;
    p.xmC = x.Cp; p.xm_ups = x_ups ? 1 : 0; p.m_ld = nx.ld; p.C = sg.Cp; p.nsets = sg.nsets;
    p.act0 = act0 ? ACT_LRELU : ACT_NONE; p.act1 = ACT_NONE;
    op.x = WS(cond.off); op.w = WT(h->mc16() ? sg.w16_off : sg.w_off); op.bias = WT(sg.b_off);
    if (one_frag) { op.w = WT(sg.w1_off); op.bias = WT(sg.b1_off); }
    op.xm = WS(x.off);
    if (has_partials(nx) && !nx.pend->affine && sg.Cp <= nx.pend->Cs) {
      const PendingStats& ps = *nx.pend;
      op.m_part = WS(ps.part_off); p.m_tiles = ps.tiles; p.m_Cs = ps.Cs; p.m_inv = ps.inv_count;
    } else {
      materialize(nx, key + ".spade");
      op.m_scale = WS(nx.sc); op.m_shift = WS(nx.sh);
    }
    op.ys0 = WS(ys0->off); if (sg.nsets == 2) op.ys1 = WS(ys1->off);
    op.grid = dim3(p.tilesX * p.tilesY, (ncols + v->BN() - 1) / v->BN(), B);
    op.flops = 2.0 * sg.cond * 2.0 * sg.nsets * sg.C * (double)Hout * Wout * B;
    P->flops[RIB_KC_SPADE] += op.flops;
    push(op);
    return true;
  }

  bool spade_block(const std::string& name, const Act& x, bool x_ups, const Norm& nx, const Act& cond,
                   Act* out, Norm* nout) {
    const ConvDef& c0 = conv_of(h, name + ".conv_block_0");
    const ConvDef& c1 = conv_of(h, name + ".conv_block_1");
    const bool learned = h->conv_index.count(name + ".conv_block_s") > 0;
    const int Hout = x_ups ? x.H * 2 : x.H, Wout = x_ups ? x.W * 2 : x.W;
    Act ys0, ys1;
    Act hbuf = act(c0.cout, Hout, Wout);
    Norm nh = norm(hbuf.Cp);
    { ConvArgs a; a.cd = &c0; a.out = hbuf; a.want_stats = true; a.stats_out = &nh;
      if (!spade(name + ".0", cond, x, x_ups, nx, &ys0, &ys1, true, runs_wino(a, Hout, Wout))) return false;
      if (!ys0.lazy) tap(name + ".ys0", ys0);
      a.in = ys0;
      if (!conv(a, name + ".conv_block_0")) return false; }
    tap(name + ".h", hbuf);
    Act y1, dummy;
    {
      ConvArgs t; t.cd = &c1; t.res = &x; t.res_ups = !learned && x_ups;
      const bool lazy1 = !learned && runs_wino(t, Hout, Wout);
      if (!spade(name + ".1", cond, hbuf, false, nh, &y1, &dummy, true, lazy1)) return false;
    }
// ... 53 lines not shown
      cur = act_n(2, c0.cout, L.H, L.W); ncur = norm(h->padc(c0.cout), 2);
      const size_t img_bytes = (size_t)L.H * L.W * cur.Cp * h->esz();
      for (int b = 0; b < 2; ++b) {
        const ConvDef& cd = conv_of(h, m + "." + branches[b] + ".0");
        Act o = cur; o.off += b * img_bytes;
        Norm no = ncur; no.sc += (size_t)b * ncur.ld * sizeof(float); no.sh += (size_t)b * ncur.ld * sizeof(float);
        ConvArgs a; a.cd = &cd; a.in = *inputs[b]; a.out = o; a.want_stats = true; a.stats_out = &no; a.affine = true; a.stats_now = true;
        if (!conv(a, cd.name)) return false;
        tap(std::string("mask.") + (b == 0 ? "lbl_0" : "img_0") + ".raw", o);
      }
    }
    for (int i = 1; i <= c.mask_down; ++i) {
      const ConvDef& cl = conv_of(h, m + ".down_lbl." + std::to_string(i));
      const ConvDef& ci = conv_of(h, m + ".down_img." + std::to_string(i));
      const bool lastl = (i == c.mask_down);
      Act o = lastl ? CAT : act_n(2, cl.cout, cur.H / 2, cur.W / 2);
      Norm no = lastl ? ncat : norm(h->padc(cl.cout), 2);
      ConvArgs a; a.cd = &cl; a.pair = &ci; a.in = cur; a.out = o; a.pro = &ncur; a.pro_lrelu = true;
      if (lastl) { a.pair_merge = true; a.pair_yoff = chm; }
      a.want_stats = true; a.stats_out = &no; a.affine = true; a.no_split = true;
      a.choice_names = {m + ".down_pair." + std::to_string(i), m + ".down_img." + std::to_string(i)};
      if (!conv(a, m + ".down_pair." + std::to_string(i))) return false;
      if (!lastl) {
        const size_t img_bytes = (size_t)o.H * o.W * o.Cp * h->esz();
        Act ol = o, oi = o; oi.off += img_bytes;
        tap("mask.lbl_" + std::to_string(i) + ".raw", ol);
        tap("mask.img_" + std::to_string(i) + ".raw", oi);
      }
      cur = o; ncur = no;
    }
    return true;
  }

  template <typename F> static void for_each_pref(Op& op, F f) {
    PRef* all[] = {&op.x, &op.pro_scale, &op.pro_shift, &op.w, &op.bias, &op.y, &op.res, &op.y_nchw, &op.stat, &op.xm, &op.m_scale,
                   &op.m_shift, &op.ys0, &op.ys1, &op.slab, &op.x2, &op.w2, &op.m_part,
                   &op.s_slab, &op.s_bias, &op.s_y, &op.s_res, &op.s_stat, &op.m_slab, &op.m_bias, &op.m_xm, &op.m_sc, &op.m_sh,
                   &op.m_ys0, &op.m_ys1, &op.f_part, &op.f_gamma, &op.f_beta, &op.f_scale, &op.f_shift, &op.p_x, &op.p_y, &op.p_stat,
                   &op.a_t1, &op.a_sc1, &op.a_sh1, &op.a_ts, &op.a_scs, &op.a_shs, &op.a_x, &op.a_out, &op.k_s0, &op.k_s1, &op.k_s2, &op.k_dst,
                   &op.wi_x, &op.wi_sc, &op.wi_sh, &op.wi_v, &op.wi_slab, &op.wi_x2, &op.wi_xres, &op.wi_o, &op.wi_sc2, &op.wi_sh2, &op.wo_m, &op.wo_bias, &op.wo_y, &op.wo_res, &op.wo_stat,
                   &op.lc_s0, &op.lc_s1, &op.lc_s2, &op.lc_w, &op.lc_bias, &op.lc_y, &op.lc_stat, &op.st_part[0], &op.st_part[1], &op.g_a, &op.g_c};
    for (PRef* r : all) if (r->sp == PS_WS) f(*r);
  }
  AllocRec* alloc_of(size_t voff) {
    size_t lo = 0, hi = allocs.size();
    while (lo + 1 < hi) { const size_t mid = (lo + hi) / 2; if (allocs[mid].voff <= voff) lo = mid; else hi = mid; }
    return (!allocs.empty() && voff >= allocs[lo].voff && voff < allocs[lo].voff + allocs[lo].bytes) ? &allocs[lo] : nullptr;
  }
  bool assign_physical() {
    const bool reuse = pol.ws_reuse && !P->labels_only;
    if (!reuse) { P->ws_bytes = ws; return true; }
    bool bad = false;
    for (size_t i = 0; i < P->ops.size(); ++i)
      for_each_pref(P->ops[i], [&](PRef& r) {
        AllocRec* a = alloc_of(r.off);
        if (!a) { bad = true; return; }
        a->first = std::min(a->first, (int)i); a->last = std::max(a->last, (int)i);
      });
    if (bad) { error = "workspace reference outside every allocation"; return false; }
    const LabelSlots& l = P->ls;
    for (size_t off : {l.x0, l.nx_sc, l.nx_sh, l.cat, l.ncat_sc, l.ncat_sh})
      if (AllocRec* a = alloc_of(off)) a->first = -1;
    if (h->keep_taps)
      for (const Tap& t : P->taps)
        if (AllocRec* a = alloc_of(t.off)) a->last = INT_MAX;
    std::vector<int> order;
    for (size_t i = 0; i < allocs.size(); ++i) if (allocs[i].last >= 0 || allocs[i].first == -1) order.push_back((int)i);
    std::sort(order.begin(), order.end(), [&](int a, int b) { return allocs[a].bytes != allocs[b].bytes ? allocs[a].bytes > allocs[b].bytes : a < b; });
    std::vector<int> placed;
    size_t top = 0;
    for (int i : order) {
      AllocRec& a = allocs[i];
      std::vector<std::pair<size_t, size_t>> busy;
      for (int j : placed) {
        const AllocRec& b = allocs[j];
// ... 21 lines not shown
    l.x0 = x.off; l.x0_b = (size_t)B * x.H * x.W * x.Cp * h->esz();
    l.nx_sc = nx.sc; l.nx_sh = nx.sh; l.nx_b = (size_t)B * nx.ld * sizeof(float);
    l.cat = CAT.off; l.cat_b = (size_t)B * CAT.H * CAT.W * CAT.Cp * h->esz();
    l.ncat_sc = ncat.sc; l.ncat_sh = ncat.sh; l.ncat_b = (size_t)B * ncat.ld * sizeof(float);
  }

  bool build_labels() {
    const Cfg& g = h->g;
    const rib_config& c = g.c;
    const int H = P->H, W = P->W;
    P->labels_only = true;
    defer_stats = false;
    const bool vL = lowc_serves({"down_first", "flow_network_temp.down_lbl.0"});
    Act L = vL ? virt(c.label_nc, H, W, U_LABEL, c.label_nc) : act(c.label_nc, H, W);
    if (!vL && L.Cp > 32) { error = "input channel counts above 32 are not supported by the pack kernel"; return false; }
    if (!vL) {
      Op op; op.kind = OP_PACK; op.kclass = RIB_KC_PACK; op.name = "pack.label";
      memset(&op.kp, 0, sizeof op.kp);
      op.kp.c0 = c.label_nc; op.kp.c1 = 0; op.kp.c2 = 0; op.kp.dC = L.Cp; op.kp.HW = H * W;
      op.k_s0 = US(U_LABEL); op.k_dst = WS(L.off);
      op.grid = dim3((H * W + 63) / 64, B, 1);
      push(op);
    }
    const int chm = g.mask_nf(c.mask_down);
    if (h->padc(chm) != chm) { error = "mask network width must be a multiple of 8 (16 with bf16 storage)"; return false; }
    Act CAT = act(2 * chm, H >> c.mask_down, W >> c.mask_down);
    Norm ncat = norm(CAT.Cp);
    if (!mask_branch(0, L, CAT, ncat, chm)) return false;
    const ConvDef& df = conv_of(h, "down_first");
    Act x = act(df.cout, H, W); Norm nx = norm(x.Cp);
    ConvArgs a; a.cd = &df; a.in = L; a.out = x; a.want_stats = true; a.stats_out = &nx;
    if (!conv(a, "down_first")) return false;
    record_label_slots(x, nx, CAT, ncat);
    return assign_physical();
  }

  struct Frame {
    Act L;
    Act Ein;
    Act I9;
    std::vector<Act> cond;
    Act CAT; Norm ncat;
    int chm = 0, Hm = 0, Wm = 0;
  };

  bool plan_boundary(Frame& F) {
    const Cfg& g = h->g;
    const rib_config& c = g.c;
    const int H = P->H, W = P->W;
    const bool vL = lowc_serves({"down_first", "flow_network_temp.down_lbl.0"});
    const bool vE = lowc_serves({"ref_embedding.conv_first"});
    const bool vI = lowc_serves({"flow_network_temp.down_img.0"}) && head_without_nhwc(conv_of(h, "conv_img"));
    F.L = vL ? virt(c.label_nc, H, W, U_LABEL, c.label_nc) : act(c.label_nc, H, W);
    F.Ein = vE ? virt(c.image_nc * 2, H, W, U_FAKE, c.image_nc, U_PREV, c.image_nc) : act(c.image_nc * 2, H, W);
    F.I9 = vI ? virt(c.image_nc * 3, H, W, U_PREV, c.image_nc, U_FAKE, c.image_nc, U_IMG, c.image_nc) : act(c.image_nc * 3, H, W);
    auto pack = [&](const std::string& nm, const Act& dst, int s0, int c0, int s1, int c1) {
      Op op; op.kind = OP_PACK; op.kclass = RIB_KC_PACK; op.name = nm;
      memset(&op.kp, 0, sizeof op.kp);
      op.kp.c0 = c0; op.kp.c1 = c1; op.kp.c2 = 0; op.kp.dC = dst.Cp; op.kp.HW = H * W;
      op.k_s0 = US(s0); if (c1) op.k_s1 = US(s1);
      op.k_dst = WS(dst.off);
      op.grid = dim3((H * W + 63) / 64, B, 1);
      push(op);
    };
    if (F.L.Cp > 32 || F.Ein.Cp > 32 || F.I9.Cp > 32) { error = "input channel counts above 32 are not supported by the pack kernel"; return false; }
    mark_label = true;
    if (!vL) pack("pack.label", F.L, U_LABEL, c.label_nc, 0, 0);
// ... 46 lines not shown
      mark_label = false;
    }

    return true;
  }

  bool plan_trunk(Frame& F) {
    const Cfg& g = h->g;
    const rib_config& c = g.c;
    const int H = P->H, W = P->W;
    const int D = c.num_down_img;
    const std::vector<Act>& cond = F.cond;
    Act x; Norm nx;
    {
      const ConvDef& df = conv_of(h, "down_first");
      x = act(df.cout, H, W); nx = norm(x.Cp);
      ConvArgs a; a.cd = &df; a.in = F.L; a.out = x; a.want_stats = true; a.stats_out = &nx;
      mark_label = true;
      if (!conv(a, "down_first")) return false;
      mark_label = false;
      tap("down_first", x);
    }
    record_label_slots(x, nx, F.CAT, F.ncat);
    for (int i = 0; i <= D; ++i) {
      Act out; Norm nout;
      const bool last = (i == D);
      if (!spade_block("down_" + std::to_string(i), x, false, nx, cond[std::min(c.emb_down, i)], &out, last ? &nout : nullptr)) return false;
      if (!last) {
        if (out.Cp % 4 != 0 || 256 % (out.Cp / 4) != 0) { error = "avgpool: unsupported channel count"; return false; }
        Act pooled = act(out.C, out.H / 2, out.W / 2);
        Norm np = norm(pooled.Cp);
        const int slots = 256 / (out.Cp / 4), ppb = slots * 4;
        const int blocks = (pooled.H * pooled.W + ppb - 1) / ppb;
        const size_t part = alloc((size_t)B * blocks * 2 * out.Cp * sizeof(double));
        Op op; op.kind = OP_POOL; op.kclass = RIB_KC_POOL; op.name = "down_" + std::to_string(i) + ".pool";
        memset(&op.pp, 0, sizeof op.pp);
        op.pp.H = out.H; op.pp.W = out.W; op.pp.C = out.Cp; op.pp.blocks = blocks;
        op.p_x = WS(out.off); op.p_y = WS(pooled.off); op.p_stat = WS(part);
        op.grid = dim3(blocks, B, 1);
        push(op);
        Op f; f.kind = OP_FINALIZE; f.kclass = RIB_KC_STATS; f.name = op.name + ".stats";
        memset(&f.fp, 0, sizeof f.fp);
        f.fp.tiles = blocks; f.fp.Cs = out.Cp; f.fp.C = out.Cp; f.fp.ld = np.ld; f.fp.off = 0;
        f.fp.inv_count = 1.0f / ((float)pooled.H * (float)pooled.W); f.fp.eps = 1e-5f;
        f.f_part = WS(part); f.f_scale = WS(np.sc); f.f_shift = WS(np.sh);
        f.grid = dim3((out.Cp + 15) / 16, B, 1);
        finalize_or_defer(f, &np, false, part, blocks, out.Cp, f.fp.inv_count, false, 0, 0);
        x = pooled; nx = np;
      } else { x = out; nx = nout; }
    }
    const int jres = std::min(c.emb_down, D + 1);
    for (int i = 0; i < g.num_res_blocks(); ++i) {
      Act out; Norm nout;
      if (!spade_block("res_" + std::to_string(i), x, false, nx, cond[jres], &out, &nout)) return false;
      x = out; nx = nout;
    }
    bool ups = false;
    for (int i = D; i >= 0; --i) {
      Act out; Norm nout;
      if (!spade_block("up_" + std::to_string(i), x, ups, nx, cond[std::min(i, c.emb_down)], &out, i != 0 ? &nout : nullptr)) return false;
      x = out; nx = nout; ups = true;
    }
    {
      const ConvDef& ci = conv_of(h, "conv_img");
      ConvArgs a; a.cd = &ci; a.in = x; a.pro_lrelu = true; a.out = F.I9; a.yoff = c.image_nc * 2;
      a.cout_store = c.image_nc; a.act = ACT_TANH; a.y_nchw = US(U_IMG);
      a.y_none = F.I9.virt;
      if (!conv(a, "conv_img")) return false;
    }

    return true;
  }

  bool plan_mask_net(Frame& F) {
    const Cfg& g = h->g;
    const rib_config& c = g.c;
    const int H = P->H, W = P->W;
    const std::string m = "flow_network_temp";
    const int chm = F.chm, Hm = F.Hm, Wm = F.Wm;
    const Act& CAT = F.CAT; const Norm& ncat = F.ncat;
// ... 19 lines not shown
      if (learned) {
        const ConvDef& cs = conv_of(h, bn + ".conv_block_s");
        ts = act(cs.cout, Hm, Wm); ns = norm(ts.Cp);
        ConvArgs a; a.cd = &cs; a.in = xin; a.out = ts; if (first) { a.pro = &ncat; a.pro_lrelu = true; }
        a.want_stats = true; a.stats_out = &ns; a.affine = true;
        if (!conv(a, cs.name)) return false;
      } else if (first) { error = "mask res block 0 must have a learned shortcut"; return false; }
      Act o = act(c1.cout, Hm, Wm);
      {
        const bool no_lazy = !pol.lazy_sources;
        ConvArgs t;
        if (i + 1 < c.mask_res_blocks) t.cd = &conv_of(h, m + ".res_flow." + std::to_string(i + 1) + ".conv_block_0");
        if (t.cd && !no_lazy && h->prec() == PREC_F32 && runs_wino(t, Hm, Wm) && t.cd->cinp == o.Cp && n1.ld == o.Cp) {
          auto L = std::make_shared<LazySrc>();
          L->mode = WSRC_JOIN; L->name = bn + ".join"; L->x = t1; L->nx = n1; L->o = o;
          if (learned) { L->has2 = true; L->x2 = ts; L->n2 = ns; } else L->xres = xin_stored;
          Act y = o; y.lazy = L;
          tap("mask.res_" + std::to_string(i), o);
          r = y; first = false;
          continue;
        }
      }
      Op op; op.kind = OP_INADD; op.kclass = RIB_KC_ELTWISE; op.name = bn + ".join";
      memset(&op.ap, 0, sizeof op.ap);
      op.ap.C = o.Cp; op.ap.HW = Hm * Wm; op.ap.ld = n1.ld;
      op.a_t1 = WS(t1.off);
      if (!take_partials(n1, op.ap.st1, op, 0)) { materialize(n1); op.a_sc1 = WS(n1.sc); op.a_sh1 = WS(n1.sh); }
      if (learned) {
        op.a_ts = WS(ts.off);
        if (!take_partials(ns, op.ap.sts, op, 1)) { materialize(ns); op.a_scs = WS(ns.sc); op.a_shs = WS(ns.sh); }
      } else op.a_x = WS(xin_stored.off);
      op.a_out = WS(o.off);
      const int nsl = (o.Cp + 63) / 64;
      op.ap.nslices = nsl; op.ap.pblocks = std::max(1, std::min((Hm * Wm + 15) / 16, ((op.ap.st1.tiles > 0 || op.ap.sts.tiles > 0) ? 384 : 2048) / nsl));
      op.grid = dim3(op.ap.pblocks * nsl, B, 1);
      push(op);
      tap("mask.res_" + std::to_string(i), o);
      r = o; first = false;
    }
    Act cur = r; Norm ncur; bool have = false;
    for (int j = 0; j < c.mask_down; ++j) {
      const ConvDef& cd = conv_of(h, m + ".up_flow." + std::to_string(2 * j + 1));
      Act o = act(cd.cout, cur.H * 2, cur.W * 2); Norm no = norm(o.Cp);
      ConvArgs a; a.cd = &cd; a.in = cur; a.ups = true; a.out = o;
      if (have) { a.pro = &ncur; a.pro_lrelu = true; }
      a.want_stats = true; a.stats_out = &no; a.affine = true;
      if (!conv(a, cd.name)) return false;
      tap("mask.up_" + std::to_string(j) + ".raw", o);
      cur = o; ncur = no; have = true;
    }
    {
      const ConvDef& cm = conv_of(h, m + ".conv_mask.0");
      ConvArgs a; a.cd = &cm; a.in = cur; if (have) { a.pro = &ncur; a.pro_lrelu = true; }
      a.act = ACT_SIGMOID; a.y_user = US(U_MASK);
      if (!conv(a, cm.name)) return false;
    }
    return true;
  }

  bool build() {
    Frame F;
    return plan_boundary(F) && plan_embedder(F) && plan_mask_label_branch(F) && plan_trunk(F) && plan_mask_net(F) && assign_physical();
  }
};

enum { PLAN_LABELS = 1, PLAN_UNPAIRED = 2 };
inline bool plan_pairs(int B, int flags) {
  return FusionPolicy().pair_mask_encoders && B == 1 && !(flags & (PLAN_LABELS | PLAN_UNPAIRED));
}
Plan* get_plan(rib_handle* h, int B, int H, int W, int flags = 0, int tuneB = 0) {
  const bool labels_only = (flags & PLAN_LABELS) != 0;
  if (!labels_only && !plan_pairs(B, 0)) flags &= ~PLAN_UNPAIRED;
  if (h->plan_batch > 0) tuneB = h->plan_batch;
  if (tuneB == B) tuneB = 0;
  const std::array<int, 5> key = {flags & 3, tuneB, B, H, W};
  auto it = h->plans.find(key);
  if (it != h->plans.end()) return it->second.get();
  const int mult = 1 << std::max(h->g.c.num_down_img, h->g.c.mask_down);
  if (B < 1 || H < mult || W < mult || H % mult || W % mult) {
    h->err = fmt("unsupported shape B=%d H=%d W=%d: H and W must be positive multiples of %d (SURVEY F5)", B, H, W, mult);
    return nullptr;
  }
  {
    const rib_config& c = h->g.c;
    const size_t widest = (size_t)std::max(std::max(c.emb_filters, c.mask_filters * 2), std::max(c.num_filters * 2, 32));
    if ((size_t)H * W * widest >= (1ull << 31)) {
      h->err = fmt("unsupported shape H=%d W=%d: a full-resolution activation exceeds 2^31 elements", H, W);
      return nullptr;
    }
  }
  std::unique_ptr<Plan> P(new Plan());
  P->B = B; P->H = H; P->W = W;
  Builder b; b.h = h; b.P = P.get(); b.B = B; b.tuneB = tuneB; b.pair_mask = plan_pairs(B, flags);
  if (!(labels_only ? b.build_labels() : b.build())) { h->err = "plan: " + b.error; return nullptr; }
  Plan* raw = P.get();
// ... 30 lines not shown
template <int CO> void launch_small_t(int bf16, dim3 grid, size_t lds, hipStream_t st, const IgemmParams& p) {
  if (bf16 == PREC_BF16) RIB_KLAUNCH((k_conv_small<CO, ST_BF16>), grid, dim3(256), lds, st, p);
  else if (bf16 == PREC_F16) RIB_KLAUNCH((k_conv_small<CO, ST_F16>), grid, dim3(256), lds, st, p);
  else RIB_KLAUNCH((k_conv_small<CO, ST_F32>), grid, dim3(256), lds, st, p);
}
void launch_head(int co, int cin, int bf16, dim3 grid, hipStream_t st, const IgemmParams& p) {
  if (cin == 16) { if (co == 1) launch_head_t<1, 16>(bf16, grid, st, p); else if (co == 2) launch_head_t<2, 16>(bf16, grid, st, p); else launch_head_t<3, 16>(bf16, grid, st, p); }
  else { if (co == 1) launch_head_t<1, 32>(bf16, grid, st, p); else if (co == 2) launch_head_t<2, 32>(bf16, grid, st, p); else launch_head_t<3, 32>(bf16, grid, st, p); }
}

int run_plan(rib_handle* h, Plan* P, const Resolver& R, hipStream_t st, bool skip_label_ops = false) {
  const int bf16 = h->prec();
  for (Op& op : P->ops) {
    if (skip_label_ops && op.label_only) continue;
    g_prof_pair = ProfPair();
    if (h->profiling && h->prof_kernels) {
      ProfPair pp;
      HIP_TRY(h, hipEventCreate(&pp.start));
      HIP_TRY(h, hipEventCreate(&pp.stop));
      h->prof_kernel_events.push_back({op.kclass, pp.start, pp.stop});
      g_prof_pair = pp;
    } else if (h->profiling) {
      hipEvent_t e0 = nullptr;
      HIP_TRY(h, hipEventCreate(&e0));
      HIP_TRY(h, hipEventRecord(e0, st));
      h->prof_events.push_back({op.kclass, e0});
    }
    switch (op.kind) {
      case OP_IGEMM: {
        IgemmParams p = op.ip;
        p.x = R.get<const float>(op.x); p.pro_scale = R.get<const float>(op.pro_scale); p.pro_shift = R.get<const float>(op.pro_shift);
        p.w = R.get<const float>(op.w); p.bias = R.get<const float>(op.bias);
        p.y = R.get<float>(op.y); p.res = R.get<const float>(op.res); p.y_nchw = R.get<float>(op.y_nchw);
        p.stat_part = R.get<double>(op.stat); p.slab = R.get<float>(op.slab);
        p.x2 = R.get<const float>(op.x2); p.w2 = R.get<const float>(op.w2);
        p.xm = R.get<const float>(op.xm); p.m_scale = R.get<const float>(op.m_scale); p.m_shift = R.get<const float>(op.m_shift);
        p.ys0 = R.get<float>(op.ys0); p.ys1 = R.get<float>(op.ys1);
        p.m_part = R.get<const double>(op.m_part);
        p.zeros = R.blob + h->zero_off;
        if (op.small_co > 0 && op.head) {
          if (op.fuse_blend && R.user[U_FUSE]) {
            p.bl_img = reinterpret_cast<const float*>(R.user[U_IMG]); p.bl_dain = reinterpret_cast<const float*>(R.user[U_FAKE]);
            p.bl_fuse = reinterpret_cast<float*>(const_cast<void*>(R.user[U_FUSE]));
          }
          launch_head(op.small_co, p.Cin, bf16, op.grid, st, p);
        } else if (op.small_co > 0) {
          const size_t lds = ((size_t)18 * 18 * (p.Cin + 4) + (size_t)op.small_co * 9 * p.Cin) * sizeof(float);
          switch (op.small_co) {
            case 1: launch_small_t<1>(bf16, op.grid, lds, st, p); break;
            case 2: launch_small_t<2>(bf16, op.grid, lds, st, p); break;
            case 3: launch_small_t<3>(bf16, op.grid, lds, st, p); break;
            default: launch_small_t<4>(bf16, op.grid, lds, st, p); break;
          }
        } else
        RIB_KLAUNCH(pick_igemm_fn(op.var, p), op.grid, dim3(256 * op.var->KW), 0, st, p);
      } break;
      case OP_GEMM: {
        GemmDmaParams p = op.gp;
        p.A = R.get<const float>(op.g_a); p.B = R.get<const float>(op.g_b); p.C = R.get<float>(op.g_c);
        RIB_KLAUNCH(h->products == RIB_PRODUCTS_BF16X3 && op.var->gfn_x3 ? op.var->gfn_x3 : op.var->gfn, op.grid, dim3(256), 0, st, p);
      } break;
      case OP_FINALIZE: {
        FinalizeParams p = op.fp;
        p.part = R.get<const double>(op.f_part); p.gamma = R.get<const float>(op.f_gamma); p.beta = R.get<const float>(op.f_beta);
        p.scale = R.get<float>(op.f_scale); p.shift = R.get<float>(op.f_shift);
        if (p.tiles > 512) RIB_KLAUNCH(k_stats_finalize<4>, dim3((p.Cs + 3) / 4, op.grid.y, op.grid.z), dim3(1024), 0, st, p);
        else RIB_KLAUNCH(k_stats_finalize<16>, op.grid, dim3(1024), 0, st, p);
      } break;
      case OP_MODULATE: {
        ModulateParams p = op.mp;
        p.slab = R.get<const float>(op.m_slab); p.bias = R.get<const float>(op.m_bias); p.xm = R.get<const float>(op.m_xm);
        p.m_scale = R.get<const float>(op.m_sc); p.m_shift = R.get<const float>(op.m_sh);
        p.st.part = R.get<const double>(op.st_part[0]); p.st.gamma = R.get<const float>(op.st_gamma[0]); p.st.beta = R.get<const float>(op.st_beta[0]);
        p.ys0 = R.get<float>(op.m_ys0); p.ys1 = R.get<float>(op.m_ys1);
        RIB_LAUNCH_ST(bf16, k_spade_modulate, op.grid, dim3(256), 0, st, p);
      } break;
      case OP_SPLITEPI: {
        SplitEpiParams p = op.sp;
        p.slab = R.get<const float>(op.s_slab); p.bias = R.get<const float>(op.s_bias); p.y = R.get<float>(op.s_y);
        p.res = R.get<const float>(op.s_res); p.stat_part = R.get<double>(op.s_stat);
        RIB_LAUNCH_ST(bf16, k_splitk_epilogue, op.grid, dim3(256), 0, st, p);
      } break;
      case OP_POOL: {
        PoolParams p = op.pp;
        p.x = R.get<const float>(op.p_x); p.y = R.get<float>(op.p_y); p.stat_part = R.get<double>(op.p_stat);
        RIB_LAUNCH_ST(bf16, k_avgpool, op.grid, dim3(256), 0, st, p);
      } break;
      case OP_INADD: {
        InAddParams p = op.ap;
        p.t1 = R.get<const float>(op.a_t1); p.sc1 = R.get<const float>(op.a_sc1); p.sh1 = R.get<const float>(op.a_sh1);
        p.ts = R.get<const float>(op.a_ts); p.scs = R.get<const float>(op.a_scs); p.shs = R.get<const float>(op.a_shs);
        p.xres = R.get<const float>(op.a_x); p.out = R.get<float>(op.a_out);
        p.st1.part = R.get<const double>(op.st_part[0]); p.st1.gamma = R.get<const float>(op.st_gamma[0]); p.st1.beta = R.get<const float>(op.st_beta[0]);
        p.sts.part = R.get<const double>(op.st_part[1]); p.sts.gamma = R.get<const float>(op.st_gamma[1]); p.sts.beta = R.get<const float>(op.st_beta[1]);
        RIB_LAUNCH_ST(bf16, k_in_add, op.grid, dim3(256), 0, st, p);
      } break;
      case OP_WINO_IN: {
        WinoInParams p = op.wi;
        p.x = R.get<const float>(op.wi_x); p.pro_scale = R.get<const float>(op.wi_sc); p.pro_shift = R.get<const float>(op.wi_sh);
        p.v = R.get<float>(op.wi_v);
        p.st.part = R.get<const double>(op.st_part[0]); p.st.gamma = R.get<const float>(op.st_gamma[0]); p.st.beta = R.get<const float>(op.st_beta[0]);
        p.slab = R.get<const float>(op.wi_slab); p.sbias = R.get<const float>(op.wi_sbias);
        p.x2 = R.get<const float>(op.wi_x2); p.xres = R.get<const float>(op.wi_xres); p.o = R.get<float>(op.wi_o);
        p.pro2_scale = R.get<const float>(op.wi_sc2); p.pro2_shift = R.get<const float>(op.wi_sh2);
        p.st2.part = R.get<const double>(op.st_part[1]); p.st2.gamma = R.get<const float>(op.st_gamma[1]); p.st2.beta = R.get<const float>(op.st_beta[1]);
        if (op.wino_m == 4) {
          if (op.wi_mode == WSRC_SPADE) RIB_KLAUNCH(k_wino4_in<WSRC_SPADE>, op.grid, dim3(256), 0, st, p);
          else if (op.wi_mode == WSRC_JOIN) RIB_KLAUNCH(k_wino4_in<WSRC_JOIN>, op.grid, dim3(256), 0, st, p);
          else RIB_KLAUNCH(k_wino4_in<WSRC_PLAIN>, op.grid, dim3(256), 0, st, p);
        } else {
          if (op.wi_mode == WSRC_SPADE) RIB_KLAUNCH(k_wino_in<WSRC_SPADE>, op.grid, dim3(256), 0, st, p);
          else if (op.wi_mode == WSRC_JOIN) RIB_KLAUNCH(k_wino_in<WSRC_JOIN>, op.grid, dim3(256), 0, st, p);
          else RIB_KLAUNCH(k_wino_in<WSRC_PLAIN>, op.grid, dim3(256), 0, st, p);
        }
      } break;
      case OP_WINO_OUT: {
        WinoOutParams p = op.wo;
        p.m = R.get<const float>(op.wo_m); p.bias = R.get<const float>(op.wo_bias); p.y = R.get<float>(op.wo_y);
        p.res = R.get<const float>(op.wo_res); p.stat_part = R.get<double>(op.wo_stat);
        if (op.wino_m == 4) RIB_KLAUNCH(k_wino4_out, op.grid, dim3(256), 0, st, p);
        else RIB_KLAUNCH(k_wino_out, op.grid, dim3(256), 0, st, p);
      } break;
      case OP_LOWC: {
        LowcParams p = op.lc;
        p.s0 = R.get<const float>(op.lc_s0); p.s1 = R.get<const float>(op.lc_s1); p.s2 = R.get<const float>(op.lc_s2);
        p.w = R.get<const float>(op.lc_w); p.bias = R.get<const float>(op.lc_bias); p.y = R.get<float>(op.lc_y);
        p.stat_part = R.get<double>(op.lc_stat);
        launch_lowc(op.lowc_ce, op.lowc_ncol, op.lowc_tw, op.grid, st, p);
      } break;
      case OP_PACK: {
        PackParams p = op.kp;
        p.s0 = R.get<const float>(op.k_s0); p.s1 = R.get<const float>(op.k_s1); p.s2 = R.get<const float>(op.k_s2);
        p.dst = R.get<float>(op.k_dst);
        RIB_LAUNCH_ST(bf16, k_pack, op.grid, dim3(256), 0, st, p);
      } break;
    }
  }
  g_prof_pair = ProfPair();
  if (h->profiling && !h->prof_kernels) {
    hipEvent_t e1 = nullptr;
    HIP_TRY(h, hipEventCreate(&e1));
    HIP_TRY(h, hipEventRecord(e1, st));
    h->prof_events.push_back({-1, e1});
  }
  HIP_TRY(h, hipGetLastError());
  return RIB_OK;
}

int check_ready(rib_handle* h) {
  if (!h) return RIB_ERR_INVALID;
  if (!h->weights_ready) return fail(h, RIB_ERR_STATE, "weights not loaded: call rib_finalize_weights() or rib_import_weights() first");
  return RIB_OK;
}

}

extern "C" {

int rib_create(const rib_config* cfg, int device, rib_handle** out) {
  if (!cfg || !out) { g_create_error = "rib_create: null argument"; return RIB_ERR_INVALID; }
// ... 762 lines not shown
    case OP_GEMM: {
      const GemmDmaParams& g = op.gp;
      const double Z = op.grid.z;
      return Z * g.M * (double)g.K * e + (g.modB ? (double)g.modB : 1.0) * g.N * (double)g.K * e + Z * g.M * (double)g.N * 4.0;
    }
    case OP_LOWC: {
      const LowcParams& l = op.lc;
      return Bn * l.H * l.W * (double)(l.c0 + l.c1 + l.c2) * 4.0 + Bn * l.H * l.W * (double)l.Cout * e + 9.0 * (l.c0 + l.c1 + l.c2) * l.Cout * 4.0;
    }
    case OP_POOL: return Bn * op.pp.H * op.pp.W * (double)op.pp.C * e * 1.25;
    case OP_INADD: return Bn * op.ap.HW * (double)op.ap.C * e * 3.0;
    case OP_SPLITEPI: {
      const SplitEpiParams& q = op.sp;
      return (double)q.ksplit * q.B * q.Hout * q.Wout * q.CoutPad * 4.0 + (double)q.B * q.Hout * q.Wout * q.Cout * e * (q.res ? 2.0 : 1.0);
    }
    case OP_MODULATE: {
      const ModulateParams& m = op.mp;
      const double px = (double)m.B * m.Hout * m.Wout;
      return px * 2.0 * m.C * m.nsets * 4.0 * m.ksplit + px * m.C * e / (m.xm_ups ? 4.0 : 1.0) + px * m.C * e * m.nsets;
    }
    case OP_WINO_IN: {
      const WinoInParams& w = op.wi;
      const int T = op.wino_m + 2;
      double b = Bn * w.H * w.W * (double)w.Cin * e / (w.x_ups ? 4.0 : 1.0) + Bn * w.tilesY * w.tilesX * (double)T * T * w.Cin * e;
      if (op.wi_mode != 0 && w.slab) b += Bn * w.H * w.W * 2.0 * w.Cin * 4.0;
      if (w.x2 || w.xres) b += Bn * w.H * w.W * (double)w.Cin * e * 2.0;
      return b;
    }
    case OP_WINO_OUT: {
      const WinoOutParams& w = op.wo;
      const int T = op.wino_m + 2;
      return Bn * w.tilesY * w.tilesX * (double)T * T * w.CoutPad * 4.0 + Bn * w.Hout * w.Wout * (double)w.Cout * e * (w.res ? 2.0 : 1.0);
    }
    case OP_FINALIZE: return Bn * op.fp.tiles * 2.0 * op.fp.Cs * 8.0;
    default: return 0.0;
  }
}

int rib_debug_launch_info(rib_handle* h, int B, int H, int W, int idx, char* buf, size_t buflen) {
  if (!h || !buf) return RIB_ERR_INVALID;
  Plan* P = get_plan(h, B, H, W);
  if (!P || idx < 0 || idx >= (int)P->ops.size()) return RIB_ERR_INVALID;
  const Op& op = P->ops[idx];
  const int rc = launch_info_head(op, buf, buflen);
  const size_t n = strlen(buf);
  if (n + 24 < buflen) snprintf(buf + n, buflen - n, "|%.0f", op_algorithmic_bytes(h, P, op));
  return rc;
}

const char* rib_build_info(void) {
  static const std::string info = [] {
#define RIB_X(s) rib_stamp_section_##s,
    const char* sh[RIB_NSECTIONS] = {RIB_FOR_SECTIONS(RIB_X)};
#undef RIB_X
    std::string s = std::string("librib stamp=") + (kLibStamp + sizeof("rib-stamp lib ") - 1) + " shards=";
    bool ok = true;
    for (int i = 0; i < RIB_NSECTIONS; ++i) {
      const char* hash = strrchr(sh[i], ' ');
      hash = hash ? hash + 1 : "?";
      ok = ok && strcmp(hash, RIB_SHARD_STAMP) == 0;
      s += std::string(i ? "," : "") + hash;
    }
    s += fmt(" consistent=%d variants=%d compiler=%s", ok ? 1 : 0, kNumVariants, __VERSION__);
    return s;
  }();
  return info.c_str();
}
// ... 127 lines not shown
```

Measured before the change: 393.7.

## Replace per-tile stats partials with deterministic fixed-point atomic accumulators

Normalization statistics are now accumulated in a per-channel arena of multi-limb 64-bit integers via atomic adds, instead of per-tile double partials reduced later. Because integer addition is order-independent, the sums stay deterministic. Finalize and the consumer kernels then decode the sums directly rather than reducing over all tiles, which shrinks the finalize kernels and cuts partial-buffer traffic. In exchange it adds zeroing ops, 14 atomics per channel per block, and encode/decode arithmetic.

```diff
diff --git a/render-in-between_amd/csrc/igemm.hip.h b/render-in-between_amd/csrc/igemm.hip.h
--- a/render-in-between_amd/csrc/igemm.hip.h
+++ b/render-in-between_amd/csrc/igemm.hip.h
@@ -91,7 +91,7 @@
   const float* res;
   int resC, res_ups;
   float* y_nchw;
-  double* stat_part;
+  long long* stat_acc;
   int ksplit;
   float* slab;
   const float* xm;
@@ -103,7 +103,7 @@
   int nsets;
   float* ys0; float* ys1;
   int act0, act1;
-  const double* m_part; int m_tiles, m_Cs; float m_inv;
+  const long long* m_acc; int m_Cs; float m_inv;
   const float* bl_img; const float* bl_dain; float* bl_fuse; int bl_C;
   int w_mod; unsigned w_stride;
   unsigned b_stride; int pair, pair_yoff;
@@ -112,22 +112,44 @@
 
 enum { STATS_MAX_PARTIALS = 128 };
 
-__device__ __forceinline__ void stats_from_partials(const double* base, int tiles, int Cs, int c, int t0, int tstep,
-                                                    double& a1, double& a2) {
-  a1 = 0.0; a2 = 0.0;
-  int t = t0;
-  for (; t + 3 * tstep < tiles; t += 4 * tstep) {
-    const double x0 = base[(size_t)t * 2 * Cs + c], y0 = base[(size_t)t * 2 * Cs + Cs + c];
-    const double x1 = base[(size_t)(t + tstep) * 2 * Cs + c], y1 = base[(size_t)(t + tstep) * 2 * Cs + Cs + c];
-    const double x2 = base[(size_t)(t + 2 * tstep) * 2 * Cs + c], y2 = base[(size_t)(t + 2 * tstep) * 2 * Cs + Cs + c];
-    const double x3 = base[(size_t)(t + 3 * tstep) * 2 * Cs + c], y3 = base[(size_t)(t + 3 * tstep) * 2 * Cs + Cs + c];
-    a1 += (x0 + x1) + (x2 + x3);
-    a2 += (y0 + y1) + (y2 + y3);
+enum { STATS_LIMBS = 7, STATS_ROWS = 2 * STATS_LIMBS };
+enum { STATS_MAX_TILES = 1 << 14 };
+constexpr double STATS_MAX_ABS = 0x1p302;
+__host__ __device__ __forceinline__ void stats_encode(double v, long long limb[STATS_LIMBS]) {
+  double a = fabs(v);
+  a = a < STATS_MAX_ABS ? a : STATS_MAX_ABS;
+#pragma unroll
+  for (int k = STATS_LIMBS - 1; k > 0; --k) {
+    const double u = ldexp(1.0, 48 * k - 32);
+    const double q = floor(a / u);
+    limb[k] = (long long)q;
+    a -= q * u;
   }
-  for (; t < tiles; t += tstep) {
-    a1 += base[(size_t)t * 2 * Cs + c];
-    a2 += base[(size_t)t * 2 * Cs + Cs + c];
-  }
+  limb[0] = (long long)rint(a * 0x1p32);
+  if (v < 0.0)
+    for (int k = 0; k < STATS_LIMBS; ++k) limb[k] = -limb[k];
+}
+__host__ __device__ __forceinline__ double stats_decode(const long long limb[STATS_LIMBS]) {
+  double d = (double)limb[STATS_LIMBS - 1];
+#pragma unroll
+  for (int k = STATS_LIMBS - 2; k >= 0; --k) d = d * 0x1p48 + (double)limb[k];
+  return d * 0x1p-32;
+}
+__device__ __forceinline__ void stats_acc_add(long long* acc, int ld, int c, double s1, double s2) {
+  long long l[2][STATS_LIMBS];
+  stats_encode(s1, l[0]);
+  stats_encode(s2, l[1]);
+  unsigned long long* a = reinterpret_cast<unsigned long long*>(acc) + c;
+#pragma unroll
+  for (int r = 0; r < STATS_ROWS; ++r)
+    __hip_atomic_fetch_add(a + (size_t)r * ld, (unsigned long long)l[r / STATS_LIMBS][r % STATS_LIMBS], __ATOMIC_RELAXED, __HIP_MEMORY_SCOPE_AGENT);
+}
+__device__ __forceinline__ void stats_of_acc(const long long* acc, int ld, int c, double& s1, double& s2) {
+  long long l[2][STATS_LIMBS];
+#pragma unroll
+  for (int r = 0; r < STATS_ROWS; ++r) l[r / STATS_LIMBS][r % STATS_LIMBS] = acc[(size_t)r * ld + c];
+  s1 = stats_decode(l[0]);
+  s2 = stats_decode(l[1]);
 }
 __device__ __forceinline__ void scale_shift_of(double s1, double s2, float inv_count, float g, float b, float& sc, float& sh) {
   const double mean = s1 * (double)inv_count;
@@ -387,24 +409,16 @@
 
   auto consumer_stats = [&]() {
     if constexpr (SPADE) {
-      if (p.m_part) {
-        constexpr int NCH = G::BN / 2, S = NT / NCH;
-        const int j = tid % NCH, sl = tid / NCH;
-        const int v = n0 / 2 + j;
-        const bool vv = v < p.nsets * p.C;
-        const int c = vv ? (v >= p.C ? v - p.C : v) : 0;
-        double a1, a2;
-        stats_from_partials(p.m_part + (size_t)n * p.m_tiles * 2 * p.m_Cs, p.m_tiles, p.m_Cs, c, sl, S, a1, a2);
-        double* red = reinterpret_cast<double*>(smem);
-        red[(sl * NCH + j) * 2] = a1; red[(sl * NCH + j) * 2 + 1] = a2;
-        __syncthreads();
-        if (sl == 0) {
-          double t1 = 0.0, t2 = 0.0;
-#pragma unroll
-          for (int k = 0; k < S; ++k) { t1 += red[(k * NCH + j) * 2]; t2 += red[(k * NCH + j) * 2 + 1]; }
+      if (p.m_acc) {
+        constexpr int NCH = G::BN / 2;
+        if (tid < NCH) {
+          const int v = n0 / 2 + tid;
+          const int c = v < p.nsets * p.C ? (v >= p.C ? v - p.C : v) : 0;
+          double t1, t2;
+          stats_of_acc(p.m_acc + (size_t)n * STATS_ROWS * p.m_Cs, p.m_Cs, c, t1, t2);
           float sc, sh;
           scale_shift_of(t1, t2, p.m_inv, 1.f, 0.f, sc, sh);
-          s_stat[j] = sc; s_stat[NCH + j] = sh;
+          s_stat[tid] = sc; s_stat[NCH + tid] = sh;
         }
         __syncthreads();
       }
@@ -811,7 +825,7 @@
             s2 += (double)v * (double)v;
           }
         }
-    if (p.stat_part) {
+    if (p.stat_acc) {
       __syncthreads();
       double* red = reinterpret_cast<double*>(smem);
       double a1 = s1 + __shfl_xor(s1, 16); a1 += __shfl_xor(a1, 32);
@@ -822,9 +836,7 @@
         double b1 = 0.0, b2 = 0.0;
 #pragma unroll
         for (int m = 0; m < WM; ++m) { b1 += red[(m * 16 + tid) * 2]; b2 += red[(m * 16 + tid) * 2 + 1]; }
-        double* dst = p.stat_part + (((size_t)n * (p.tilesX * p.tilesY) + tile) * 2) * p.CoutPad;
-        dst[n0 + tid] = b1;
-        dst[p.CoutPad + n0 + tid] = b2;
+        stats_acc_add(p.stat_acc + (size_t)n * STATS_ROWS * p.CoutPad, p.CoutPad, n0 + tid, b1, b2);
       }
     }
   } else if (!SPADE && p.slab != nullptr) {
@@ -849,7 +861,7 @@
     }
   } else if (!SPADE) {
     double* red = reinterpret_cast<double*>(smem);
-    if (p.stat_part) __syncthreads();
+    if (p.stat_acc) __syncthreads();
     const float* pbias = p.bias + (p.w_mod ? (size_t)(n % p.w_mod) * p.b_stride : 0);
     const int ny = p.pair ? (n >> 1) : n;
     const int yoff = p.pair ? p.yoff + (n & 1) * p.pair_yoff : p.yoff;
@@ -980,7 +992,7 @@
         }
         }
       }
-      if (p.stat_part) {
+      if (p.stat_acc) {
         int cnt = 0;
 #pragma unroll
         for (int ph = 0; ph < PH; ++ph)
@@ -1009,7 +1021,7 @@
         }
       }
     }
-    if (p.stat_part) {
+    if (p.stat_acc) {
       __syncthreads();
       for (int c = tid; c < G::BN; c += 256) {
         double a1 = 0.0, a2 = 0.0;
@@ -1017,9 +1029,7 @@
         for (int m = 0; m < WM; ++m) { a1 += red[(m * G::BN + c) * 2]; a2 += red[(m * G::BN + c) * 2 + 1]; }
         const int col = n0 + c;
         if (col < p.CoutPad) {
-          double* dst = p.stat_part + (((size_t)n * (p.tilesX * p.tilesY) + tile) * 2) * p.CoutPad;
-          dst[col] = a1;
-          dst[p.CoutPad + col] = a2;
+          stats_acc_add(p.stat_acc + (size_t)n * STATS_ROWS * p.CoutPad, p.CoutPad, col, a1, a2);
         }
       }
     }
@@ -1033,7 +1043,7 @@
     float bg = 0.f, bb = 0.f, sc = 0.f, sh = 0.f;
     if (vvalid) {
       bg = p.bias[colg]; bb = p.bias[colg + 16];
-      if (p.m_part) { sc = s_stat[v - n0 / 2]; sh = s_stat[G::BN / 2 + v - n0 / 2]; }
+      if (p.m_acc) { sc = s_stat[v - n0 / 2]; sh = s_stat[G::BN / 2 + v - n0 / 2]; }
       else { sc = p.m_scale[(size_t)n * p.m_ld + c]; sh = p.m_shift[(size_t)n * p.m_ld + c]; }
     }
     float* yout = set ? p.ys1 : p.ys0;
@@ -1094,7 +1104,7 @@
       float bg = 0.f, bb = 0.f, sc = 0.f, sh = 0.f;
       if (vvalid) {
         bg = p.bias[colg]; bb = p.bias[colg + 32];
-        if (p.m_part) { sc = s_stat[v - n0 / 2]; sh = s_stat[G::BN / 2 + v - n0 / 2]; }
+        if (p.m_acc) { sc = s_stat[v - n0 / 2]; sh = s_stat[G::BN / 2 + v - n0 / 2]; }
         else { sc = p.m_scale[(size_t)n * p.m_ld + c]; sh = p.m_shift[(size_t)n * p.m_ld + c]; }
       }
       float* yout = set ? p.ys1 : p.ys0;
diff --git a/render-in-between_amd/csrc/kernels.hip.h b/render-in-between_amd/csrc/kernels.hip.h
--- a/render-in-between_amd/csrc/kernels.hip.h
+++ b/render-in-between_amd/csrc/kernels.hip.h
@@ -141,8 +141,8 @@
 }
 
 struct FinalizeParams {
-  const double* part;
-  int tiles, Cs, C;
+  const long long* acc;
+  int Cs, C;
   const float* gamma;
   const float* beta;
   float* scale;
@@ -153,40 +153,27 @@
   int g_stride, pair_merge, pair_off;
 };
 
-template <int CH>
-__global__ __launch_bounds__(1024) void k_stats_finalize(const FinalizeParams p) {
-  static_assert(CH == 16 || CH == 4, "16 channels x 64 slices or 4 channels x 256 slices");
-  constexpr int SL = 1024 / CH;
-  __shared__ double red[2][16][CH];
-  const int cl = threadIdx.x % CH, sl = threadIdx.x / CH;
-  const int c = blockIdx.x * CH + cl;
+__global__ __launch_bounds__(64) void k_stats_finalize(const FinalizeParams p) {
+  const int c = blockIdx.x * 64 + threadIdx.x;
   const int n = blockIdx.y;
-  double a1 = 0.0, a2 = 0.0;
-  if (c < p.Cs) stats_from_partials(p.part + (size_t)n * p.tiles * 2 * p.Cs, p.tiles, p.Cs, c, sl, SL, a1, a2);
-#pragma unroll
-  for (int off = CH; off < 64; off <<= 1) { a1 += __shfl_xor(a1, off); a2 += __shfl_xor(a2, off); }
-  if ((threadIdx.x & 63) < CH) { red[0][threadIdx.x >> 6][cl] = a1; red[1][threadIdx.x >> 6][cl] = a2; }
-  __syncthreads();
-  if (sl == 0) {
-    double t1 = 0.0, t2 = 0.0;
-#pragma unroll
-    for (int w = 0; w < 16; ++w) { t1 += red[0][w][cl]; t2 += red[1][w][cl]; }
-    red[0][0][cl] = t1; red[1][0][cl] = t2;
-  }
-  if (sl == 0 && c < p.C) {
-    const double s1 = red[0][0][cl], s2 = red[1][0][cl];
-    const double mean = s1 * (double)p.inv_count;
-    double var = s2 * (double)p.inv_count - mean * mean;
-    if (var < 0.0) var = 0.0;
-    const float rstd = (float)(1.0 / sqrt(var + (double)p.eps));
-    const int gs = (n & 1) * p.g_stride;
-    const float g = p.gamma ? p.gamma[gs + c] : 1.f;
-    const float b = p.beta ? p.beta[gs + c] : 0.f;
-    const float sc = rstd * g;
-    const size_t at = p.pair_merge ? (size_t)(n >> 1) * p.ld + p.off + (n & 1) * p.pair_off + c : (size_t)n * p.ld + p.off + c;
-    p.scale[at] = sc;
-    p.shift[at] = b - (float)mean * sc;
-  }
+  if (c >= p.C) return;
+  double s1, s2;
+  stats_of_acc(p.acc + (size_t)n * STATS_ROWS * p.Cs, p.Cs, c, s1, s2);
+  const double mean = s1 * (double)p.inv_count;
+  double var = s2 * (double)p.inv_count - mean * mean;
+  if (var < 0.0) var = 0.0;
+  const float rstd = (float)(1.0 / sqrt(var + (double)p.eps));
+  const int gs = (n & 1) * p.g_stride;
+  const float g = p.gamma ? p.gamma[gs + c] : 1.f;
+  const float b = p.beta ? p.beta[gs + c] : 0.f;
+  const float sc = rstd * g;
+  const size_t at = p.pair_merge ? (size_t)(n >> 1) * p.ld + p.off + (n & 1) * p.pair_off + c : (size_t)n * p.ld + p.off + c;
+  p.scale[at] = sc;
+  p.shift[at] = b - (float)mean * sc;
+}
+
+__global__ __launch_bounds__(256) void k_stats_zero(long long* acc, int n) {
+  for (int i = blockIdx.x * 256 + threadIdx.x; i < n; i += gridDim.x * 256) acc[i] = 0;
 }
 
 struct SplitEpiParams {
@@ -195,7 +182,7 @@
   float* y; int yC, yoff, Cout;
   int act;
   const float* res; int resC, res_ups;
-  double* stat_part; int blocks;
+  long long* stat_acc; int blocks;
   int Hout, Wout;
 };
 
@@ -282,7 +269,7 @@
         if (c4 * 4 + e < p.Cout) st_act<ST>(p.y, opix * p.yC + p.yoff + c4 * 4 + e, vals[k][e]);
     }
   }
-  if (p.stat_part) {
+  if (p.stat_acc) {
 #pragma unroll
     for (int e = 0; e < 4; ++e) { red[0][threadIdx.x][e] = s1[e]; red[1][threadIdx.x][e] = s2[e]; }
     __syncthreads();
@@ -290,32 +277,24 @@
       const int g = c / 4, e = c % 4;
       double a1 = 0.0, a2 = 0.0;
       for (int s = 0; s < slots; ++s) { a1 += red[0][s * c4n + g][e]; a2 += red[1][s * c4n + g][e]; }
-      double* dst = p.stat_part + (((size_t)n * p.blocks + blockIdx.x) * 2) * p.CoutPad;
-      dst[c] = a1;
-      dst[p.CoutPad + c] = a2;
+      stats_acc_add(p.stat_acc + (size_t)n * STATS_ROWS * p.CoutPad, p.CoutPad, c, a1, a2);
     }
   }
 }
 
 struct StatSrc {
-  const double* part;
-  int tiles, Cs;
+  const long long* acc;
+  int Cs;
   float inv_count;
   const float* gamma;
   const float* beta;
 };
 
-__device__ __forceinline__ void block_stats_64(const StatSrc& s, int n, int c0, int nch, double* red ,
-                                               float* s_sc, float* s_sh) {
-  const int j = threadIdx.x & 63, q = threadIdx.x >> 6;
-  double a1 = 0.0, a2 = 0.0;
-  if (j < nch) stats_from_partials(s.part + (size_t)n * s.tiles * 2 * s.Cs, s.tiles, s.Cs, c0 + j, q, 4, a1, a2);
-  red[(q * 64 + j) * 2] = a1; red[(q * 64 + j) * 2 + 1] = a2;
-  __syncthreads();
-  if (q == 0 && j < nch) {
-    double t1 = 0.0, t2 = 0.0;
-#pragma unroll
-    for (int k = 0; k < 4; ++k) { t1 += red[(k * 64 + j) * 2]; t2 += red[(k * 64 + j) * 2 + 1]; }
+__device__ __forceinline__ void block_stats_64(const StatSrc& s, int n, int c0, int nch, float* s_sc, float* s_sh) {
+  const int j = threadIdx.x;
+  if (j < nch) {
+    double t1, t2;
+    stats_of_acc(s.acc + (size_t)n * STATS_ROWS * s.Cs, s.Cs, c0 + j, t1, t2);
     float sc, sh;
     scale_shift_of(t1, t2, s.inv_count, s.gamma ? s.gamma[c0 + j] : 1.f, s.beta ? s.beta[c0 + j] : 0.f, sc, sh);
     s_sc[j] = sc; s_sh[j] = sh;
@@ -347,8 +326,8 @@
   k.sc = make_float4(1.f, 1.f, 1.f, 1.f); k.sh = make_float4(0.f, 0.f, 0.f, 0.f);
   k.aff = false;
   const int l = (threadIdx.x & 15) * 4;
-  if (p.st.part) {
-    block_stats_64(p.st, n, slice * 64, min(64, p.Cin - slice * 64), red, s_sc, s_sh);
+  if (p.st.acc) {
+    block_stats_64(p.st, n, slice * 64, min(64, p.Cin - slice * 64), s_sc, s_sh);
     k.sc = make_float4(s_sc[l], s_sc[l + 1], s_sc[l + 2], s_sc[l + 3]);
     k.sh = make_float4(s_sh[l], s_sh[l + 1], s_sh[l + 2], s_sh[l + 3]);
     k.aff = true;
@@ -365,9 +344,9 @@
   if constexpr (MODE == WSRC_JOIN) {
     k.sc2 = make_float4(1.f, 1.f, 1.f, 1.f); k.sh2 = make_float4(0.f, 0.f, 0.f, 0.f);
     if (p.x2) {
-      if (p.st2.part) {
+      if (p.st2.acc) {
         __syncthreads();
-        block_stats_64(p.st2, n, slice * 64, min(64, p.Cin - slice * 64), red, s_sc, s_sh);
+        block_stats_64(p.st2, n, slice * 64, min(64, p.Cin - slice * 64), s_sc, s_sh);
         k.sc2 = make_float4(s_sc[l], s_sc[l + 1], s_sc[l + 2], s_sc[l + 3]);
         k.sh2 = make_float4(s_sh[l], s_sh[l + 1], s_sh[l + 2], s_sh[l + 3]);
       } else if (cok) {
@@ -474,11 +453,11 @@
   float* y; int yC, yoff, Cout, Hout, Wout;
   int act;
   const float* res; int resC;
-  double* stat_part;
+  long long* stat_acc;
   int nslices, ublocks;
 };
 
-__device__ __forceinline__ void wino_out_partials(double (*red)[256][4], const double s1[4], const double s2[4], double* stat_part,
+__device__ __forceinline__ void wino_out_partials(double (*red)[256][4], const double s1[4], const double s2[4], long long* stat_acc,
                                                   int n, int ublocks, int ub, int slice, int CoutPad) {
 #pragma unroll
   for (int e = 0; e < 4; ++e) { red[0][threadIdx.x][e] = s1[e]; red[1][threadIdx.x][e] = s2[e]; }
@@ -490,9 +469,7 @@
       double a1 = 0.0, a2 = 0.0;
 #pragma unroll
       for (int s = 0; s < 16; ++s) { a1 += red[0][s * 16 + g][e]; a2 += red[1][s * 16 + g][e]; }
-      double* dst = stat_part + (((size_t)n * ublocks + ub) * 2) * CoutPad;
-      dst[c] = a1;
-      dst[CoutPad + c] = a2;
+      stats_acc_add(stat_acc + (size_t)n * STATS_ROWS * CoutPad, CoutPad, c, a1, a2);
     }
   }
 }
@@ -551,7 +528,7 @@
       }
     }
   }
-  if (p.stat_part) wino_out_partials(red, s1, s2, p.stat_part, n, p.ublocks, ub, slice, p.CoutPad);
+  if (p.stat_acc) wino_out_partials(red, s1, s2, p.stat_acc, n, p.ublocks, ub, slice, p.CoutPad);
 }
 
 __device__ __constant__ float kWino4BT[6][6] = {
@@ -711,7 +688,7 @@
       }
     }
   }
-  if (p.stat_part) wino_out_partials(red, s1, s2, p.stat_part, n, p.ublocks, ub, slice, p.CoutPad);
+  if (p.stat_acc) wino_out_partials(red, s1, s2, p.stat_acc, n, p.ublocks, ub, slice, p.CoutPad);
 }
 #undef RIB_F4_SUB
 #undef RIB_F4_ADD
@@ -743,15 +720,15 @@
   const int set = v >= p.C ? 1 : 0;
   const int c = v - set * p.C;
   float4 sc, sh;
-  if (p.st.part) {
+  if (p.st.acc) {
     const int v0 = slice * 64, c0 = v0 >= p.C ? v0 - p.C : v0;
-    block_stats_64(p.st, n, c0, min(64, p.C - c0), red, s_sc, s_sh);
+    block_stats_64(p.st, n, c0, min(64, p.C - c0), s_sc, s_sh);
     const int l = (threadIdx.x & 15) * 4;
     sc = make_float4(s_sc[l], s_sc[l + 1], s_sc[l + 2], s_sc[l + 3]);
     sh = make_float4(s_sh[l], s_sh[l + 1], s_sh[l + 2], s_sh[l + 3]);
   }
   if (v4 >= v4n) return;
-  if (!p.st.part) {
+  if (!p.st.acc) {
     sc = *reinterpret_cast<const float4*>(p.m_scale + (size_t)n * p.m_ld + c);
     sh = *reinterpret_cast<const float4*>(p.m_shift + (size_t)n * p.m_ld + c);
   }
@@ -796,7 +773,7 @@
 struct PoolParams {
   const float* x; float* y;
   int H, W, C;
-  double* stat_part;
+  long long* stat_acc;
   int blocks;
 };
 
@@ -844,9 +821,7 @@
     const int g = c / 4, e = c % 4;
     double a1 = 0.0, a2 = 0.0;
     for (int s = 0; s < slots; ++s) { a1 += red[0][s * c4n + g][e]; a2 += red[1][s * c4n + g][e]; }
-    double* dst = p.stat_part + (((size_t)n * p.blocks + blockIdx.x) * 2) * p.C;
-    dst[c] = a1;
-    dst[p.C + c] = a2;
+    stats_acc_add(p.stat_acc + (size_t)n * STATS_ROWS * p.C, p.C, c, a1, a2);
   }
 }
 
@@ -870,15 +845,15 @@
   const int slice = blockIdx.x % p.nslices, pb = blockIdx.x / p.nslices;
   const int c4 = slice * 16 + (threadIdx.x & 15);
   const int nch = min(64, p.C - slice * 64);
-  if (p.st1.part) block_stats_64(p.st1, n, slice * 64, nch, red, s_sc[0], s_sh[0]);
-  if (p.ts && p.sts.part) block_stats_64(p.sts, n, slice * 64, nch, red, s_sc[1], s_sh[1]);
+  if (p.st1.acc) block_stats_64(p.st1, n, slice * 64, nch, s_sc[0], s_sh[0]);
+  if (p.ts && p.sts.acc) block_stats_64(p.sts, n, slice * 64, nch, s_sc[1], s_sh[1]);
   if (c4 >= c4n) return;
   const int l = (threadIdx.x & 15) * 4;
   float4 s, t, s2 = make_float4(0.f, 0.f, 0.f, 0.f), t2 = s2;
-  if (p.st1.part) { s = make_float4(s_sc[0][l], s_sc[0][l + 1], s_sc[0][l + 2], s_sc[0][l + 3]); t = make_float4(s_sh[0][l], s_sh[0][l + 1], s_sh[0][l + 2], s_sh[0][l + 3]); }
+  if (p.st1.acc) { s = make_float4(s_sc[0][l], s_sc[0][l + 1], s_sc[0][l + 2], s_sc[0][l + 3]); t = make_float4(s_sh[0][l], s_sh[0][l + 1], s_sh[0][l + 2], s_sh[0][l + 3]); }
   else { s = *reinterpret_cast<const float4*>(p.sc1 + (size_t)n * p.ld + c4 * 4); t = *reinterpret_cast<const float4*>(p.sh1 + (size_t)n * p.ld + c4 * 4); }
   if (p.ts) {
-    if (p.sts.part) { s2 = make_float4(s_sc[1][l], s_sc[1][l + 1], s_sc[1][l + 2], s_sc[1][l + 3]); t2 = make_float4(s_sh[1][l], s_sh[1][l + 1], s_sh[1][l + 2], s_sh[1][l + 3]); }
+    if (p.sts.acc) { s2 = make_float4(s_sc[1][l], s_sc[1][l + 1], s_sc[1][l + 2], s_sc[1][l + 3]); t2 = make_float4(s_sh[1][l], s_sh[1][l + 1], s_sh[1][l + 2], s_sh[1][l + 3]); }
     else { s2 = *reinterpret_cast<const float4*>(p.scs + (size_t)n * p.ld + c4 * 4); t2 = *reinterpret_cast<const float4*>(p.shs + (size_t)n * p.ld + c4 * 4); }
   }
   const float* second = p.ts ? p.ts : p.xres;
@@ -1114,7 +1089,8 @@
   const float* bias;
   float* y; int yC, yoff, Cout;
   int act;
-  double* stat_part; int CoutPad;
+  long long* stat_acc; int CoutPad;
+  long long* stat_zero; int stat_zero_n;
   int tilesX, tilesY;
 };
 
@@ -1137,6 +1113,10 @@
   const int tile = blockIdx.x;
   const int ty0 = (tile / p.tilesX) * TH, tx0 = (tile % p.tilesX) * TW;
   const int ctot = p.c0 + p.c1 + p.c2;
+  if (p.stat_zero) {
+    const int nth = gridDim.x * gridDim.y * 256;
+    for (int i = (blockIdx.y * gridDim.x + blockIdx.x) * 256 + tid; i < p.stat_zero_n; i += nth) p.stat_zero[i] = 0;
+  }
   const size_t HW = (size_t)p.H * p.W;
   {
     constexpr int TOT = CE * IH * IW, NIT = (TOT + 255) / 256;
@@ -1229,7 +1209,7 @@
           c1 += (double)v; c2 += (double)v * (double)v;
         }
       }
-      if (p.stat_part) {
+      if (p.stat_acc) {
         c1 += __shfl_xor(c1, 32); c2 += __shfl_xor(c2, 32);
         if (lh == 0) { red[wave][col][0] = c1; red[wave][col][1] = c2; }
       }
@@ -1270,13 +1250,13 @@
         s1 += (double)v; s2 += (double)v * (double)v;
       }
     }
-    if (p.stat_part) {
+    if (p.stat_acc) {
       s1 += __shfl_xor(s1, 16); s2 += __shfl_xor(s2, 16);
       s1 += __shfl_xor(s1, 32); s2 += __shfl_xor(s2, 32);
       if (lq == 0) { red[wave][col][0] = s1; red[wave][col][1] = s2; }
     }
   }
-  if (p.stat_part) {
+  if (p.stat_acc) {
     __syncthreads();
     for (int c = tid; c < p.CoutPad; c += 256) {
       double a1 = 0.0, a2 = 0.0;
@@ -1284,11 +1264,7 @@
 #pragma unroll
         for (int w = 0; w < 4; ++w) { a1 += red[w][c][0]; a2 += red[w][c][1]; }
       }
-      {
-        double* dst = p.stat_part + (((size_t)n * (p.tilesX * p.tilesY) + tile) * 2) * p.CoutPad;
-        dst[c] = a1;
-        dst[p.CoutPad + c] = a2;
-      }
+      stats_acc_add(p.stat_acc + (size_t)n * STATS_ROWS * p.CoutPad, p.CoutPad, c, a1, a2);
     }
   }
 }
diff --git a/render-in-between_amd/csrc/rib.hip b/render-in-between_amd/csrc/rib.hip
--- a/render-in-between_amd/csrc/rib.hip
+++ b/render-in-between_amd/csrc/rib.hip
@@ -401,9 +401,9 @@
   return best;
 }
 
-enum OpKind { OP_PACK, OP_IGEMM, OP_FINALIZE, OP_POOL, OP_INADD, OP_SPLITEPI, OP_MODULATE, OP_WINO_IN, OP_WINO_OUT, OP_LOWC, OP_GEMM };
-
-enum PtrSpace { PS_NULL = 0, PS_WS, PS_WEIGHT, PS_USER, PS_WINO };
+enum OpKind { OP_PACK, OP_IGEMM, OP_FINALIZE, OP_POOL, OP_INADD, OP_SPLITEPI, OP_MODULATE, OP_WINO_IN, OP_WINO_OUT, OP_LOWC, OP_GEMM, OP_ZERO };
+
+enum PtrSpace { PS_NULL = 0, PS_WS, PS_WEIGHT, PS_USER, PS_WINO, PS_STATS };
 enum UserSlot { U_LABEL = 0, U_FAKE, U_PREV, U_IMG, U_MASK, U_FUSE, U_COUNT };
 struct PRef {
   PtrSpace sp = PS_NULL;
@@ -423,17 +423,18 @@
   bool fuse_blend = false;
   IgemmParams ip;
   PRef x, pro_scale, pro_shift, w, bias, y, res, y_nchw, stat, xm, m_scale, m_shift, ys0, ys1, slab, x2, w2;
-  PRef m_part;
-  PRef st_part[2], st_gamma[2], st_beta[2];
+  PRef m_acc;
+  PRef st_acc[2], st_gamma[2], st_beta[2];
   SplitEpiParams sp; PRef s_slab, s_bias, s_y, s_res, s_stat;
   ModulateParams mp; PRef m_slab, m_bias, m_xm, m_sc, m_sh, m_ys0, m_ys1;
   dim3 grid;
   double flops = 0;
-  FinalizeParams fp; PRef f_part, f_gamma, f_beta, f_scale, f_shift;
+  FinalizeParams fp; PRef f_acc, f_gamma, f_beta, f_scale, f_shift;
+  PRef z_acc; int z_n = 0;
   PoolParams pp; PRef p_x, p_y, p_stat;
   InAddParams ap; PRef a_t1, a_sc1, a_sh1, a_ts, a_scs, a_shs, a_x, a_out;
   PackParams kp; PRef k_s0, k_s1, k_s2, k_dst;
-  LowcParams lc; PRef lc_s0, lc_s1, lc_s2, lc_w, lc_bias, lc_y, lc_stat; int lowc_ce = 0, lowc_ncol = 0, lowc_tw = 32;
+  LowcParams lc; PRef lc_s0, lc_s1, lc_s2, lc_w, lc_bias, lc_y, lc_stat, lc_zero; int lowc_ce = 0, lowc_ncol = 0, lowc_tw = 32;
   WinoInParams wi; PRef wi_x, wi_sc, wi_sh, wi_v, wi_slab, wi_sbias, wi_x2, wi_xres, wi_o, wi_sc2, wi_sh2; int wi_mode = 0;
   WinoOutParams wo; PRef wo_m, wo_bias, wo_y, wo_res, wo_stat;
   GemmDmaParams gp; PRef g_a, g_b, g_c;
@@ -444,7 +445,7 @@
 struct PendingStats {
   Op fin;
   bool pushed = false;
-  size_t part_off = 0; int tiles = 0, Cs = 0; float inv_count = 0.f;
+  PRef acc; int Cs = 0; float inv_count = 0.f;
   bool affine = false; size_t g_off = 0, be_off = 0;
 };
 
@@ -823,19 +824,19 @@
     if (n.pend && !n.pend->pushed) { n.pend->pushed = true; n.pend->fin.for_op = consumer; push(n.pend->fin); }
   }
   static bool has_partials(const Norm& n) { return n.pend && !n.pend->pushed; }
-  void finalize_or_defer(Op& f, Norm* out, bool now, size_t part_off, int tiles, int Cs, float inv_count, bool affine, size_t g_off, size_t be_off) {
-    if (now || !pol.consumer_stats || !defer_stats || mark_label || tiles > STATS_MAX_PARTIALS) { push(f); return; }
+  void finalize_or_defer(Op& f, Norm* out, bool now, int Cs, float inv_count, bool affine, size_t g_off, size_t be_off) {
+    if (now || !pol.consumer_stats || !defer_stats || mark_label) { push(f); return; }
     auto ps = std::make_shared<PendingStats>();
-    ps->fin = f; ps->part_off = part_off; ps->tiles = tiles; ps->Cs = Cs; ps->inv_count = inv_count;
+    ps->fin = f; ps->acc = f.f_acc; ps->Cs = Cs; ps->inv_count = inv_count;
     ps->affine = affine; ps->g_off = g_off; ps->be_off = be_off;
     out->pend = ps;
   }
   bool take_partials(const Norm& n, StatSrc& st, Op& op, int slot) {
-    if (!has_partials(n) || n.pend->tiles > STATS_MAX_PARTIALS) return false;
+    if (!has_partials(n)) return false;
     const PendingStats& ps = *n.pend;
     memset(&st, 0, sizeof st);
-    st.tiles = ps.tiles; st.Cs = ps.Cs; st.inv_count = ps.inv_count;
-    op.st_part[slot] = WS(ps.part_off);
+    st.Cs = ps.Cs; st.inv_count = ps.inv_count;
+    op.st_acc[slot] = ps.acc;
     if (ps.affine) { op.st_gamma[slot] = WT(ps.g_off); op.st_beta[slot] = WT(ps.be_off); }
     return true;
   }
@@ -854,6 +855,16 @@
     size_t o = ws; ws += align256(bytes);
     allocs.push_back(AllocRec{o, align256(bytes), o, INT_MAX, -1});
     return o;
+  }
+  size_t stats_bytes = 0;
+  bool stats_acc(PRef& r, int images, int Cs, int tiles, const std::string& who) {
+    if (tiles > STATS_MAX_TILES) {
+      error = fmt("%s: %d statistics partials per channel (at most %d keep the integer sums exact)", who.c_str(), tiles, (int)STATS_MAX_TILES);
+      return false;
+    }
+    r.sp = PS_STATS; r.off = stats_bytes;
+    stats_bytes += align256((size_t)images * STATS_ROWS * Cs * sizeof(long long));
+    return true;
   }
   Act act(int C, int H, int W) {
     Act a; a.C = C; a.Cp = h->padc(C); a.H = H; a.W = W;
@@ -1025,13 +1036,13 @@
       return true;
     }
     int tiles = p.tilesX * p.tilesY;
-    size_t part_off = 0;
+    PRef acc;
     op.grid = dim3(tiles, v->NF == 0 ? 1 : (c.coutp + v->BN() - 1) / v->BN(), nB * S);
     op.flops = 2.0 * c.cin * c.ks * c.ks * c.cout * (double)Hout * Wout * nB + aux_flops;
     P->flops[RIB_KC_IGEMM] += op.flops;
     if (a.pair && (S != 1 || v->NF == 0)) { error = opname + ": a paired launch cannot split K or use the 16-column path"; return false; }
     if (S == 1) {
-      if (a.want_stats) { part_off = alloc((size_t)nB * tiles * 2 * c.coutp * sizeof(double)); op.stat = WS(part_off); }
+      if (a.want_stats) { if (!stats_acc(acc, nB, c.coutp, tiles, opname)) return false; op.stat = acc; }
       push(op);
     } else {
       const size_t slab_off = alloc((size_t)S * B * Hout * Wout * c.coutp * sizeof(float));
@@ -1044,9 +1055,8 @@
       const int blocks = (Hout * Wout + ppb - 1) / ppb;
       e.sp.blocks = blocks;
       e.s_slab = WS(slab_off); e.s_bias = op.bias; e.s_y = op.y; e.s_res = op.res;
-      if (a.want_stats) { part_off = alloc((size_t)B * blocks * 2 * c.coutp * sizeof(double)); e.s_stat = WS(part_off); }
+      if (a.want_stats) { if (!stats_acc(acc, B, c.coutp, blocks, opname)) return false; e.s_stat = acc; }
       e.grid = dim3(blocks, B, 1);
-      tiles = blocks;
       op.y = PRef(); op.res = PRef();
       push(op);
       push(e);
@@ -1054,15 +1064,15 @@
     if (a.want_stats) {
       Op f; f.kind = OP_FINALIZE; f.kclass = RIB_KC_STATS; f.name = opname + ".stats";
       memset(&f.fp, 0, sizeof f.fp);
-      f.fp.tiles = tiles; f.fp.Cs = c.coutp; f.fp.C = h->padc(c.cout);
+      f.fp.Cs = c.coutp; f.fp.C = h->padc(c.cout);
       f.fp.ld = a.stats_out->ld; f.fp.off = (int)a.stats_choff;
       f.fp.inv_count = 1.0f / ((float)Hout * (float)Wout); f.fp.eps = 1e-5f;
-      f.f_part = WS(part_off);
+      f.f_acc = acc;
       if (a.affine) { f.f_gamma = WT(c.g_off); f.f_beta = WT(c.be_off); }
       f.f_scale = WS(a.stats_out->sc); f.f_shift = WS(a.stats_out->sh);
-      f.grid = dim3(c.coutp / 16, nB, 1);
+      f.grid = dim3((c.coutp + 63) / 64, nB, 1);
       if (a.pair) { f.fp.g_stride = a.affine ? (int)(a.pair->g_off - c.g_off) : 0; f.fp.pair_merge = a.pair_merge ? 1 : 0; f.fp.pair_off = a.pair_yoff; }
-      finalize_or_defer(f, a.stats_out, a.stats_choff != 0 || a.stats_now || a.pair != nullptr, part_off, tiles, c.coutp, f.fp.inv_count, a.affine, c.g_off, c.be_off);
+      finalize_or_defer(f, a.stats_out, a.stats_choff != 0 || a.stats_now || a.pair != nullptr, c.coutp, f.fp.inv_count, a.affine, c.g_off, c.be_off);
     }
     return true;
   }
@@ -1086,8 +1096,8 @@
     op.lc_s0 = US(a.in.usrc[0]); if (p.c1) op.lc_s1 = US(a.in.usrc[1]); if (p.c2) op.lc_s2 = US(a.in.usrc[2]);
     op.lc_w = WT(c.wl_off); op.lc_bias = WT(c.b_off); op.lc_y = WS(a.out.off);
     const int tiles = p.tilesX * p.tilesY;
-    size_t part_off = 0;
-    if (a.want_stats) { part_off = alloc((size_t)B * tiles * 2 * c.coutp * sizeof(double)); op.lc_stat = WS(part_off); }
+    PRef acc;
+    if (a.want_stats) { if (!stats_acc(acc, B, c.coutp, tiles, opname)) return false; op.lc_stat = acc; }
     op.grid = dim3(tiles, B, 1);
     op.flops = 2.0 * c.cin * 9.0 * c.cout * (double)H * W * B;
     P->flops[RIB_KC_IGEMM] += op.flops;
@@ -1095,14 +1105,14 @@
     if (a.want_stats) {
       Op f; f.kind = OP_FINALIZE; f.kclass = RIB_KC_STATS; f.name = opname + ".stats";
       memset(&f.fp, 0, sizeof f.fp);
-      f.fp.tiles = tiles; f.fp.Cs = c.coutp; f.fp.C = h->padc(c.cout);
+      f.fp.Cs = c.coutp; f.fp.C = h->padc(c.cout);
       f.fp.ld = a.stats_out->ld; f.fp.off = (int)a.stats_choff;
       f.fp.inv_count = 1.0f / ((float)H * (float)W); f.fp.eps = 1e-5f;
-      f.f_part = WS(part_off);
+      f.f_acc = acc;
       if (a.affine) { f.f_gamma = WT(c.g_off); f.f_beta = WT(c.be_off); }
       f.f_scale = WS(a.stats_out->sc); f.f_shift = WS(a.stats_out->sh);
-      f.grid = dim3(c.coutp / 16, B, 1);
-      finalize_or_defer(f, a.stats_out, a.stats_choff != 0 || a.stats_now, part_off, tiles, c.coutp, f.fp.inv_count, a.affine, c.g_off, c.be_off);
+      f.grid = dim3((c.coutp + 63) / 64, B, 1);
+      finalize_or_defer(f, a.stats_out, a.stats_choff != 0 || a.stats_now, c.coutp, f.fp.inv_count, a.affine, c.g_off, c.be_off);
     }
     return true;
   }
@@ -1146,7 +1156,7 @@
         op.wi_sc = WS(a.pro->sc + a.pro_choff * sizeof(float)); op.wi_sh = WS(a.pro->sh + a.pro_choff * sizeof(float));
       }
       const int nsl = (c.cinp + 63) / 64, units = ntiles * (wm + 2);
-      op.wi.nslices = nsl; op.wi.ublocks = std::max(1, std::min((units + 15) / 16, (op.wi.st.tiles > 0 ? 512 : 4096) / nsl));
+      op.wi.nslices = nsl; op.wi.ublocks = std::max(1, std::min((units + 15) / 16, (op.st_acc[0].sp != PS_NULL ? 512 : 4096) / nsl));
       op.grid = dim3(op.wi.ublocks * nsl, B, 1);
       push(op);
     }
@@ -1202,21 +1212,21 @@
       if (a.out.H != Hout || a.out.W != Wout) { error = fmt("%s: output size mismatch", opname.c_str()); return false; }
       op.wo_m = WS(m_off); op.wo_bias = WT(c.b_off); op.wo_y = WS(a.out.off);
       if (a.res) { op.wo_res = WS(a.res->off); op.wo.resC = a.res->Cp; }
-      size_t part_off = 0;
-      if (a.want_stats) { part_off = alloc((size_t)B * blocks * 2 * c.coutp * sizeof(double)); op.wo_stat = WS(part_off); }
+      PRef acc;
+      if (a.want_stats) { if (!stats_acc(acc, B, c.coutp, blocks, opname)) return false; op.wo_stat = acc; }
       op.grid = dim3(blocks * nsl, B, 1);
       push(op);
       if (a.want_stats) {
         Op f; f.kind = OP_FINALIZE; f.kclass = RIB_KC_STATS; f.name = opname + ".stats";
         memset(&f.fp, 0, sizeof f.fp);
-        f.fp.tiles = blocks; f.fp.Cs = c.coutp; f.fp.C = h->padc(c.cout);
+        f.fp.Cs = c.coutp; f.fp.C = h->padc(c.cout);
         f.fp.ld = a.stats_out->ld; f.fp.off = (int)a.stats_choff;
         f.fp.inv_count = 1.0f / ((float)Hout * (float)Wout); f.fp.eps = 1e-5f;
-        f.f_part = WS(part_off);
+        f.f_acc = acc;
         if (a.affine) { f.f_gamma = WT(c.g_off); f.f_beta = WT(c.be_off); }
         f.f_scale = WS(a.stats_out->sc); f.f_shift = WS(a.stats_out->sh);
-        f.grid = dim3(c.coutp / 16, B, 1);
-        finalize_or_defer(f, a.stats_out, a.stats_choff != 0 || a.stats_now, part_off, blocks, c.coutp, f.fp.inv_count, a.affine, c.g_off, c.be_off);
+        f.grid = dim3((c.coutp + 63) / 64, B, 1);
+        finalize_or_defer(f, a.stats_out, a.stats_choff != 0 || a.stats_now, c.coutp, f.fp.inv_count, a.affine, c.g_off, c.be_off);
       }
     }
     return true;
@@ -1359,7 +1369,7 @@
       }
       mo.m_ys0 = WS(ys0->off); if (sg.nsets == 2) mo.m_ys1 = WS(ys1->off);
       const int nsl = (sg.nsets * sg.Cp + 63) / 64;
-      mo.mp.nslices = nsl; mo.mp.pblocks = std::max(1, std::min((Hout * Wout + 15) / 16, (mo.mp.st.tiles > 0 ? 384 : 2048) / nsl));
+      mo.mp.nslices = nsl; mo.mp.pblocks = std::max(1, std::min((Hout * Wout + 15) / 16, (mo.st_acc[0].sp != PS_NULL ? 384 : 2048) / nsl));
       mo.grid = dim3(mo.mp.pblocks * nsl, B, 1);
       push(mo);
       return true;
@@ -1382,7 +1392,7 @@
     op.xm = WS(x.off);
     if (has_partials(nx) && !nx.pend->affine && sg.Cp <= nx.pend->Cs) {
       const PendingStats& ps = *nx.pend;
-      op.m_part = WS(ps.part_off); p.m_tiles = ps.tiles; p.m_Cs = ps.Cs; p.m_inv = ps.inv_count;
+      op.m_acc = ps.acc; p.m_Cs = ps.Cs; p.m_inv = ps.inv_count;
     } else {
       materialize(nx, key + ".spade");
       op.m_scale = WS(nx.sc); op.m_shift = WS(nx.sh);
@@ -1502,15 +1512,38 @@
     return true;
   }
 
-  template <typename F> static void for_each_pref(Op& op, F f) {
+  template <typename F> static void for_each_pref(Op& op, F f, PtrSpace sp = PS_WS) {
     PRef* all[] = {&op.x, &op.pro_scale, &op.pro_shift, &op.w, &op.bias, &op.y, &op.res, &op.y_nchw, &op.stat, &op.xm, &op.m_scale,
-                   &op.m_shift, &op.ys0, &op.ys1, &op.slab, &op.x2, &op.w2, &op.m_part,
+                   &op.m_shift, &op.ys0, &op.ys1, &op.slab, &op.x2, &op.w2, &op.m_acc,
                    &op.s_slab, &op.s_bias, &op.s_y, &op.s_res, &op.s_stat, &op.m_slab, &op.m_bias, &op.m_xm, &op.m_sc, &op.m_sh,
-                   &op.m_ys0, &op.m_ys1, &op.f_part, &op.f_gamma, &op.f_beta, &op.f_scale, &op.f_shift, &op.p_x, &op.p_y, &op.p_stat,
+                   &op.m_ys0, &op.m_ys1, &op.f_acc, &op.f_gamma, &op.f_beta, &op.f_scale, &op.f_shift, &op.p_x, &op.p_y, &op.p_stat,
                    &op.a_t1, &op.a_sc1, &op.a_sh1, &op.a_ts, &op.a_scs, &op.a_shs, &op.a_x, &op.a_out, &op.k_s0, &op.k_s1, &op.k_s2, &op.k_dst,
                    &op.wi_x, &op.wi_sc, &op.wi_sh, &op.wi_v, &op.wi_slab, &op.wi_x2, &op.wi_xres, &op.wi_o, &op.wi_sc2, &op.wi_sh2, &op.wo_m, &op.wo_bias, &op.wo_y, &op.wo_res, &op.wo_stat,
-                   &op.lc_s0, &op.lc_s1, &op.lc_s2, &op.lc_w, &op.lc_bias, &op.lc_y, &op.lc_stat, &op.st_part[0], &op.st_part[1], &op.g_a, &op.g_c};
-    for (PRef* r : all) if (r->sp == PS_WS) f(*r);
+                   &op.lc_s0, &op.lc_s1, &op.lc_s2, &op.lc_w, &op.lc_bias, &op.lc_y, &op.lc_stat, &op.st_acc[0], &op.st_acc[1], &op.g_a, &op.g_c,
+                   &op.lc_zero, &op.z_acc};
+    for (PRef* r : all) if (r->sp == sp) f(*r);
+  }
+  bool finish_stats_arena() {
+    if (!stats_bytes) return true;
+    Op* zop = nullptr;
+    for (Op& op : P->ops) {
+      if (op.kind == OP_LOWC && op.lc_stat.sp == PS_NULL && !op.label_only) { zop = &op; break; }
+      bool touches = false;
+      for_each_pref(op, [&](PRef&) { touches = true; }, PS_STATS);
+      if (touches) break;
+    }
+    const size_t base = alloc(stats_bytes);
+    allocs.back().first = -1; allocs.back().last = INT_MAX;
+    for (Op& op : P->ops) for_each_pref(op, [&](PRef& r) { r.sp = PS_WS; r.off += base; }, PS_STATS);
+    const int n = (int)(stats_bytes / sizeof(long long));
+    if (zop) {
+      zop->lc_zero = WS(base); zop->lc.stat_zero_n = n;
+    } else {
+      Op z; z.kind = OP_ZERO; z.kclass = RIB_KC_STATS; z.name = "stats.zero";
+      z.z_acc = WS(base); z.z_n = n; z.grid = dim3(std::min((n + 255) / 256, 64), 1, 1);
+      P->ops.insert(P->ops.begin(), z);
+    }
+    return true;
   }
   AllocRec* alloc_of(size_t voff) {
     size_t lo = 0, hi = allocs.size();
@@ -1598,7 +1631,7 @@
     ConvArgs a; a.cd = &df; a.in = L; a.out = x; a.want_stats = true; a.stats_out = &nx;
     if (!conv(a, "down_first")) return false;
     record_label_slots(x, nx, CAT, ncat);
-    return assign_physical();
+    return finish_stats_arena() && assign_physical();
   }
 
   struct Frame {
@@ -1711,20 +1744,21 @@
         Norm np = norm(pooled.Cp);
         const int slots = 256 / (out.Cp / 4), ppb = slots * 4;
         const int blocks = (pooled.H * pooled.W + ppb - 1) / ppb;
-        const size_t part = alloc((size_t)B * blocks * 2 * out.Cp * sizeof(double));
+        PRef part;
+        if (!stats_acc(part, B, out.Cp, blocks, "down_" + std::to_string(i) + ".pool")) return false;
         Op op; op.kind = OP_POOL; op.kclass = RIB_KC_POOL; op.name = "down_" + std::to_string(i) + ".pool";
         memset(&op.pp, 0, sizeof op.pp);
         op.pp.H = out.H; op.pp.W = out.W; op.pp.C = out.Cp; op.pp.blocks = blocks;
-        op.p_x = WS(out.off); op.p_y = WS(pooled.off); op.p_stat = WS(part);
+        op.p_x = WS(out.off); op.p_y = WS(pooled.off); op.p_stat = part;
         op.grid = dim3(blocks, B, 1);
         push(op);
         Op f; f.kind = OP_FINALIZE; f.kclass = RIB_KC_STATS; f.name = op.name + ".stats";
         memset(&f.fp, 0, sizeof f.fp);
-        f.fp.tiles = blocks; f.fp.Cs = out.Cp; f.fp.C = out.Cp; f.fp.ld = np.ld; f.fp.off = 0;
+        f.fp.Cs = out.Cp; f.fp.C = out.Cp; f.fp.ld = np.ld; f.fp.off = 0;
         f.fp.inv_count = 1.0f / ((float)pooled.H * (float)pooled.W); f.fp.eps = 1e-5f;
-        f.f_part = WS(part); f.f_scale = WS(np.sc); f.f_shift = WS(np.sh);
-        f.grid = dim3((out.Cp + 15) / 16, B, 1);
-        finalize_or_defer(f, &np, false, part, blocks, out.Cp, f.fp.inv_count, false, 0, 0);
+        f.f_acc = part; f.f_scale = WS(np.sc); f.f_shift = WS(np.sh);
+        f.grid = dim3((out.Cp + 63) / 64, B, 1);
+        finalize_or_defer(f, &np, false, out.Cp, f.fp.inv_count, false, 0, 0);
         x = pooled; nx = np;
       } else { x = out; nx = nout; }
     }
@@ -1810,7 +1844,7 @@
       } else op.a_x = WS(xin_stored.off);
       op.a_out = WS(o.off);
       const int nsl = (o.Cp + 63) / 64;
-      op.ap.nslices = nsl; op.ap.pblocks = std::max(1, std::min((Hm * Wm + 15) / 16, ((op.ap.st1.tiles > 0 || op.ap.sts.tiles > 0) ? 384 : 2048) / nsl));
+      op.ap.nslices = nsl; op.ap.pblocks = std::max(1, std::min((Hm * Wm + 15) / 16, ((op.st_acc[0].sp != PS_NULL || op.st_acc[1].sp != PS_NULL) ? 384 : 2048) / nsl));
       op.grid = dim3(op.ap.pblocks * nsl, B, 1);
       push(op);
       tap("mask.res_" + std::to_string(i), o);
@@ -1838,7 +1872,7 @@
 
   bool build() {
     Frame F;
-    return plan_boundary(F) && plan_embedder(F) && plan_mask_label_branch(F) && plan_trunk(F) && plan_mask_net(F) && assign_physical();
+    return plan_boundary(F) && plan_embedder(F) && plan_mask_label_branch(F) && plan_trunk(F) && plan_mask_net(F) && finish_stats_arena() && assign_physical();
   }
 };
 
@@ -1935,11 +1969,11 @@
         p.x = R.get<const float>(op.x); p.pro_scale = R.get<const float>(op.pro_scale); p.pro_shift = R.get<const float>(op.pro_shift);
         p.w = R.get<const float>(op.w); p.bias = R.get<const float>(op.bias);
         p.y = R.get<float>(op.y); p.res = R.get<const float>(op.res); p.y_nchw = R.get<float>(op.y_nchw);
-        p.stat_part = R.get<double>(op.stat); p.slab = R.get<float>(op.slab);
+        p.stat_acc = R.get<long long>(op.stat); p.slab = R.get<float>(op.slab);
         p.x2 = R.get<const float>(op.x2); p.w2 = R.get<const float>(op.w2);
         p.xm = R.get<const float>(op.xm); p.m_scale = R.get<const float>(op.m_scale); p.m_shift = R.get<const float>(op.m_shift);
         p.ys0 = R.get<float>(op.ys0); p.ys1 = R.get<float>(op.ys1);
-        p.m_part = R.get<const double>(op.m_part);
+        p.m_acc = R.get<const long long>(op.m_acc);
         p.zeros = R.blob + h->zero_off;
         if (op.small_co > 0 && op.head) {
           if (op.fuse_blend && R.user[U_FUSE]) {
@@ -1965,28 +1999,30 @@
       } break;
       case OP_FINALIZE: {
         FinalizeParams p = op.fp;
-        p.part = R.get<const double>(op.f_part); p.gamma = R.get<const float>(op.f_gamma); p.beta = R.get<const float>(op.f_beta);
+        p.acc = R.get<const long long>(op.f_acc); p.gamma = R.get<const float>(op.f_gamma); p.beta = R.get<const float>(op.f_beta);
         p.scale = R.get<float>(op.f_scale); p.shift = R.get<float>(op.f_shift);
-        if (p.tiles > 512) RIB_KLAUNCH(k_stats_finalize<4>, dim3((p.Cs + 3) / 4, op.grid.y, op.grid.z), dim3(1024), 0, st, p);
-        else RIB_KLAUNCH(k_stats_finalize<16>, op.grid, dim3(1024), 0, st, p);
+        RIB_KLAUNCH(k_stats_finalize, op.grid, dim3(64), 0, st, p);
       } break;
+      case OP_ZERO:
+        RIB_KLAUNCH(k_stats_zero, op.grid, dim3(256), 0, st, R.get<long long>(op.z_acc), op.z_n);
+        break;
       case OP_MODULATE: {
         ModulateParams p = op.mp;
         p.slab = R.get<const float>(op.m_slab); p.bias = R.get<const float>(op.m_bias); p.xm = R.get<const float>(op.m_xm);
         p.m_scale = R.get<const float>(op.m_sc); p.m_shift = R.get<const float>(op.m_sh);
-        p.st.part = R.get<const double>(op.st_part[0]); p.st.gamma = R.get<const float>(op.st_gamma[0]); p.st.beta = R.get<const float>(op.st_beta[0]);
+        p.st.acc = R.get<const long long>(op.st_acc[0]); p.st.gamma = R.get<const float>(op.st_gamma[0]); p.st.beta = R.get<const float>(op.st_beta[0]);
         p.ys0 = R.get<float>(op.m_ys0); p.ys1 = R.get<float>(op.m_ys1);
         RIB_LAUNCH_ST(bf16, k_spade_modulate, op.grid, dim3(256), 0, st, p);
       } break;
       case OP_SPLITEPI: {
         SplitEpiParams p = op.sp;
         p.slab = R.get<const float>(op.s_slab); p.bias = R.get<const float>(op.s_bias); p.y = R.get<float>(op.s_y);
-        p.res = R.get<const float>(op.s_res); p.stat_part = R.get<double>(op.s_stat);
+        p.res = R.get<const float>(op.s_res); p.stat_acc = R.get<long long>(op.s_stat);
         RIB_LAUNCH_ST(bf16, k_splitk_epilogue, op.grid, dim3(256), 0, st, p);
       } break;
       case OP_POOL: {
         PoolParams p = op.pp;
-        p.x = R.get<const float>(op.p_x); p.y = R.get<float>(op.p_y); p.stat_part = R.get<double>(op.p_stat);
+        p.x = R.get<const float>(op.p_x); p.y = R.get<float>(op.p_y); p.stat_acc = R.get<long long>(op.p_stat);
         RIB_LAUNCH_ST(bf16, k_avgpool, op.grid, dim3(256), 0, st, p);
       } break;
       case OP_INADD: {
@@ -1994,19 +2030,19 @@
         p.t1 = R.get<const float>(op.a_t1); p.sc1 = R.get<const float>(op.a_sc1); p.sh1 = R.get<const float>(op.a_sh1);
         p.ts = R.get<const float>(op.a_ts); p.scs = R.get<const float>(op.a_scs); p.shs = R.get<const float>(op.a_shs);
         p.xres = R.get<const float>(op.a_x); p.out = R.get<float>(op.a_out);
-        p.st1.part = R.get<const double>(op.st_part[0]); p.st1.gamma = R.get<const float>(op.st_gamma[0]); p.st1.beta = R.get<const float>(op.st_beta[0]);
-        p.sts.part = R.get<const double>(op.st_part[1]); p.sts.gamma = R.get<const float>(op.st_gamma[1]); p.sts.beta = R.get<const float>(op.st_beta[1]);
+        p.st1.acc = R.get<const long long>(op.st_acc[0]); p.st1.gamma = R.get<const float>(op.st_gamma[0]); p.st1.beta = R.get<const float>(op.st_beta[0]);
+        p.sts.acc = R.get<const long long>(op.st_acc[1]); p.sts.gamma = R.get<const float>(op.st_gamma[1]); p.sts.beta = R.get<const float>(op.st_beta[1]);
         RIB_LAUNCH_ST(bf16, k_in_add, op.grid, dim3(256), 0, st, p);
       } break;
       case OP_WINO_IN: {
         WinoInParams p = op.wi;
         p.x = R.get<const float>(op.wi_x); p.pro_scale = R.get<const float>(op.wi_sc); p.pro_shift = R.get<const float>(op.wi_sh);
         p.v = R.get<float>(op.wi_v);
-        p.st.part = R.get<const double>(op.st_part[0]); p.st.gamma = R.get<const float>(op.st_gamma[0]); p.st.beta = R.get<const float>(op.st_beta[0]);
+        p.st.acc = R.get<const long long>(op.st_acc[0]); p.st.gamma = R.get<const float>(op.st_gamma[0]); p.st.beta = R.get<const float>(op.st_beta[0]);
         p.slab = R.get<const float>(op.wi_slab); p.sbias = R.get<const float>(op.wi_sbias);
         p.x2 = R.get<const float>(op.wi_x2); p.xres = R.get<const float>(op.wi_xres); p.o = R.get<float>(op.wi_o);
         p.pro2_scale = R.get<const float>(op.wi_sc2); p.pro2_shift = R.get<const float>(op.wi_sh2);
-        p.st2.part = R.get<const double>(op.st_part[1]); p.st2.gamma = R.get<const float>(op.st_gamma[1]); p.st2.beta = R.get<const float>(op.st_beta[1]);
+        p.st2.acc = R.get<const long long>(op.st_acc[1]); p.st2.gamma = R.get<const float>(op.st_gamma[1]); p.st2.beta = R.get<const float>(op.st_beta[1]);
         if (op.wino_m == 4) {
           if (op.wi_mode == WSRC_SPADE) RIB_KLAUNCH(k_wino4_in<WSRC_SPADE>, op.grid, dim3(256), 0, st, p);
           else if (op.wi_mode == WSRC_JOIN) RIB_KLAUNCH(k_wino4_in<WSRC_JOIN>, op.grid, dim3(256), 0, st, p);
@@ -2020,7 +2056,7 @@
       case OP_WINO_OUT: {
         WinoOutParams p = op.wo;
         p.m = R.get<const float>(op.wo_m); p.bias = R.get<const float>(op.wo_bias); p.y = R.get<float>(op.wo_y);
-        p.res = R.get<const float>(op.wo_res); p.stat_part = R.get<double>(op.wo_stat);
+        p.res = R.get<const float>(op.wo_res); p.stat_acc = R.get<long long>(op.wo_stat);
         if (op.wino_m == 4) RIB_KLAUNCH(k_wino4_out, op.grid, dim3(256), 0, st, p);
         else RIB_KLAUNCH(k_wino_out, op.grid, dim3(256), 0, st, p);
       } break;
@@ -2028,7 +2064,7 @@
         LowcParams p = op.lc;
         p.s0 = R.get<const float>(op.lc_s0); p.s1 = R.get<const float>(op.lc_s1); p.s2 = R.get<const float>(op.lc_s2);
         p.w = R.get<const float>(op.lc_w); p.bias = R.get<const float>(op.lc_bias); p.y = R.get<float>(op.lc_y);
-        p.stat_part = R.get<double>(op.lc_stat);
+        p.stat_acc = R.get<long long>(op.lc_stat); p.stat_zero = R.get<long long>(op.lc_zero);
         launch_lowc(op.lowc_ce, op.lowc_ncol, op.lowc_tw, op.grid, st, p);
       } break;
       case OP_PACK: {
@@ -2857,7 +2893,8 @@
       const int T = op.wino_m + 2;
       return Bn * w.tilesY * w.tilesX * (double)T * T * w.CoutPad * 4.0 + Bn * w.Hout * w.Wout * (double)w.Cout * e * (w.res ? 2.0 : 1.0);
     }
-    case OP_FINALIZE: return Bn * op.fp.tiles * 2.0 * op.fp.Cs * 8.0;
+    case OP_FINALIZE: return Bn * op.fp.Cs * (STATS_ROWS * 8.0 + 8.0);
+    case OP_ZERO: return op.z_n * 8.0;
     default: return 0.0;
   }
 }
```

Result: slower. 375.2, median of 2 (-4.7%).
